# Ryan-Yanlong/DREAM-GNN

Hardware: AMD Instinct MI355X
Metric: GCMC+FGCN SpMM edges/sec and achieved HBM GB/s at 1/2/4/8 MI355X (higher is better)
Workload: dtype f32

## Files before the change

### dream_gnn_amd/_lib.py

```python
from __future__ import annotations

import ctypes
import os

import torch

_HERE = os.path.dirname(os.path.abspath(__file__))
LIB_PATH = os.path.join(_HERE, "libdgmi.so")
TORCH_LIB_PATH = os.path.join(_HERE, "libdgmi_torch.so")

ABI_VERSION = 20

_vp = ctypes.c_void_p
_i64 = ctypes.c_int64
_EPI = [ctypes.c_int32, ctypes.c_float, _vp, _i64, ctypes.c_float]


SIGNATURES = {
    "dgmi_abi_version": (ctypes.c_int, []),
    "dgmi_status_string": (ctypes.c_char_p, [ctypes.c_int]),
    "dgmi_device_ok": (ctypes.c_int, []),
    "dgmi_csr_from_coo_i32": (ctypes.c_int, [_vp, _vp, _i64, _i64, _i64, _vp, _vp, _vp, _vp,
                                             ctypes.POINTER(ctypes.c_size_t), _vp]),
    "dgmi_spmm_csr_f32": (ctypes.c_int, [_vp, _vp, _vp, _vp, _vp, ctypes.c_int32, _vp, _i64, _vp, _vp, _vp, _i64, _i64,
                                         _i64, _i64] + _EPI + [_vp]),
    "dgmi_gather_f32": (ctypes.c_int, [_vp, _vp, _i64, _vp, _vp]),
    "dgmi_gather_concat_f32": (ctypes.c_int, [_vp, _vp, _i64, _vp, _i64, _i64, _vp, _i64, _i64, _vp, _i64, _vp]),
    "dgmi_csr_sliced_from_coo_i32": (ctypes.c_int, [_vp, _vp, _i64, _i64, _i64, ctypes.c_int32, _vp, _vp, _vp, _vp,
                                                    ctypes.POINTER(ctypes.c_size_t), _vp]),
    "dgmi_csr_sliced_from_csr_i32": (ctypes.c_int, [_vp, _vp, _vp, _i64, _i64, _i64, ctypes.c_int32, _vp, _vp, _vp, _vp,
                                                    ctypes.POINTER(ctypes.c_size_t), _vp]),
    "dgmi_spmm_sliced_planes_bytes": (ctypes.c_size_t, [_i64, ctypes.c_int32, _i64]),
    "dgmi_spmm_sliced_f32": (ctypes.c_int, [_vp, _vp, _vp, _vp, _vp, ctypes.c_int32, _vp, _i64, _vp, _vp, _vp, _i64, _i64,
                                            _i64, _i64, ctypes.c_int32, ctypes.c_int32, ctypes.c_int32, _vp, ctypes.c_size_t] + _EPI
                             + [_vp]),
    "dgmi_knn_cosine_supported": (ctypes.c_int, [_i64, _i64, _i64]),
    "dgmi_knn_cosine_workspace_bytes": (ctypes.c_size_t, [_i64, _i64, ctypes.c_int32]),
    "dgmi_knn_cosine_topk_f32": (ctypes.c_int, [_vp, _i64, _i64, _i64, ctypes.c_int32, _vp, _vp, ctypes.c_size_t, _vp]),
    "dgmi_probe_row_gather_f32": (ctypes.c_int, [_vp, _i64, _i64, _i64, _i64, _i64, ctypes.c_int32, _vp, _vp]),
    "dgmi_epilogue_backward_f32": (ctypes.c_int, [_vp, _vp, _vp, _i64, ctypes.c_int32, ctypes.c_float, ctypes.c_float, _vp, _vp]),
    "dgmi_gather_add_f32": (ctypes.c_int, [_vp, _vp, _i64, _vp, _i64, _vp, _i64, _vp, _i64, _vp, _i64, ctypes.c_int32, _vp]),
    "dgmi_random_subset_workspace_bytes": (ctypes.c_size_t, []),
    "dgmi_random_subset_mask_f32": (ctypes.c_int, [_i64, _i64, ctypes.c_uint64, _vp, _vp, ctypes.c_size_t, _vp]),
    "dgmi_spmm_default_chunk": (ctypes.c_int32, [_i64, _i64]),
    "dgmi_spmm_plan_bytes": (ctypes.c_size_t, [_i64, _i64, ctypes.c_int32]),
    "dgmi_spmm_partials_bytes": (ctypes.c_size_t, [_i64, ctypes.c_int32, _i64]),
    "dgmi_spmm_plan_build": (ctypes.c_int, [_vp, _i64, _i64, ctypes.c_int32, _vp, ctypes.c_size_t, _vp,
                                            ctypes.POINTER(ctypes.c_size_t), _vp]),
    "dgmi_spmm_csr_planned_f32": (ctypes.c_int, [_vp, _vp, _vp, _vp, _vp, ctypes.c_int32, _vp, _i64, _vp, _vp, _vp, _i64,
                                                 _i64, _i64, _i64, _i64, ctypes.c_int32, _vp, _vp, ctypes.c_size_t] + _EPI
                                  + [_vp]),
    "dgmi_random_subset_select": (ctypes.c_int, [_i64, _i64, ctypes.c_uint64, ctypes.c_uint32, _vp, _vp, ctypes.c_size_t,
                                                 _vp]),
    "dgmi_random_subset_select_batch": (ctypes.c_int, [ctypes.c_int32, _vp, _vp, _vp, _vp, _vp, _vp, ctypes.c_size_t, _vp]),
    "dgmi_random_subset_select_batch_dseed": (ctypes.c_int, [ctypes.c_int32, _vp, _vp, _vp, _vp, _vp, _vp, ctypes.c_size_t, _vp]),
    "dgmi_keep_mask_f32": (ctypes.c_int, [_vp, ctypes.c_int32, _i64, _vp, _vp]),
    "dgmi_scale_rows_f32": (ctypes.c_int, [_vp, _i64, _vp, _i64, _i64, _vp, _i64, _vp]),
    "dgmi_weighted_colsum_f32": (ctypes.c_int, [_vp, _i64, _vp, _i64, _i64, _i64, ctypes.c_int32, _vp, _i64, _vp]),
    "dgmi_rank_add_f32": (ctypes.c_int, [_vp, _i64, _vp, _i64, _vp, _i64, _i64, _i64, ctypes.c_int32, _vp]),
    "dgmi_compact_layout_workspace_bytes": (ctypes.c_size_t, [_i64]),
    "dgmi_compact_layout_i32": (ctypes.c_int, [_vp, _i64, _vp, _vp, _vp, _i64, _vp, ctypes.c_int32, _vp, _vp, _vp, _vp,
                                               ctypes.c_size_t, _vp]),
    "dgmi_set_tuning": (ctypes.c_int, [ctypes.c_char_p, _i64]),
    "dgmi_row_multiplicity_f32": (ctypes.c_int, [_vp, _vp, _i64, _i64, ctypes.c_float, _vp, _vp, _vp, _vp]),
}


PAIR_SIGNATURES = {
    "dgmi_pair_topk_workspace_bytes": (ctypes.c_size_t, [_i64, _i64, ctypes.c_int32]),
    "dgmi_pair_mlp_topk_f32": (ctypes.c_int, [_vp, _i64, _i64, _vp, _i64, _i64, ctypes.c_int32, ctypes.c_int32, _vp, _vp, _vp,
                                              _vp, _vp, _vp, _i64, ctypes.c_int32, _vp, _vp, _vp, _vp, _vp, ctypes.c_size_t,
                                              _vp]),
}
PAIR_TOPK_MAX_K = 1024

RANK_SIGNATURES = {
    "dgmi_row_topk_workspace_bytes": (ctypes.c_size_t, [_i64, _i64, ctypes.c_int32]),
    "dgmi_pair_mlp_row_topk_f32": (ctypes.c_int, [_vp, _i64, _i64, _vp, _i64, _i64, ctypes.c_int32, ctypes.c_int32, _vp, _vp,
                                                  _vp, _vp, _vp, _vp, _i64, ctypes.c_int32, _vp, _vp, _vp, _vp, _vp,
                                                  ctypes.c_size_t, _vp]),
}
ROW_TOPK_MAX_K = 128

ABOVE_SIGNATURES = {
    "dgmi_pair_emit_workspace_bytes": (ctypes.c_size_t, [_i64, _i64]),
    "dgmi_pair_mlp_emit_f32": (ctypes.c_int, [_vp, _i64, _i64, _vp, _i64, _i64, ctypes.c_int32, ctypes.c_int32, _vp, _vp, _vp,
                                              _vp, _vp, _vp, _i64, ctypes.c_float, _i64, _vp, _vp, _vp, _vp, _vp, _vp,
                                              ctypes.c_size_t, _vp]),
    "dgmi_pair_records_sort_workspace_bytes": (ctypes.c_size_t, [_i64]),
    "dgmi_pair_records_sort_f32": (ctypes.c_int, [_vp, _vp, _vp, _i64, _vp, ctypes.c_size_t, _vp]),
}
PAIR_EMIT_MAX_RECORDS = 1 << 24

BF16_SIGNATURES = {
    "dgmi_rows_to_bf16": (ctypes.c_int, [_vp, _i64, _vp, _i64, _i64, _vp, _i64, _vp]),
    "dgmi_spmm_sliced_bf16": (ctypes.c_int, [_vp, _vp, _vp, _vp, _vp, ctypes.c_int32, _vp, _i64, _vp, _vp, _i64, _i64, _i64, _i64,
                                             ctypes.c_int32, ctypes.c_int32, ctypes.c_int32, _vp, ctypes.c_size_t] + _EPI + [_vp]),
}


GIVEN_SIGNATURES = {
    "dgmi_pair_rank_workspace_bytes": (ctypes.c_size_t, [_i64, _i64, _i64]),
    "dgmi_pair_mlp_score_list_f32": (ctypes.c_int, [_vp, _i64, _i64, _vp, _i64, _i64, ctypes.c_int32, ctypes.c_int32, _vp, _vp,
                                                    _vp, _vp, _vp, _vp, _i64, _vp, _vp, _vp]),
    "dgmi_pair_mlp_rank_list_f32": (ctypes.c_int, [_vp, _i64, _i64, _vp, _i64, _i64, ctypes.c_int32, ctypes.c_int32, _vp, _vp,
                                                   _vp, _vp, _vp, _vp, _i64, _vp, _vp, _i64, _vp, _vp, _vp, _vp, _vp,
                                                   ctypes.c_size_t, _vp]),
}

CURVE_SIGNATURES = {
    "dgmi_curve_areas_workspace_bytes": (ctypes.c_size_t, [_i64, _i64]),
    "dgmi_curve_areas_f32": (ctypes.c_int, [_vp, _vp, _vp, _i64, _i64, ctypes.c_float, _vp, _vp, _vp, _vp, ctypes.c_size_t,
                                            _vp]),
}
CURVE_MAX_SEGMENTS = 1 << 24

LAYOUT_SIGNATURES = {
    "dgmi_sliced_layout_slices": (ctypes.c_int32, [_i64, _i64, _i64, ctypes.c_int32]),
}

_TRAIN_OPERANDS = [_vp, _i64, _i64, _vp, _i64, _i64, ctypes.c_int32, ctypes.c_int32, _vp, _vp, _vp, _vp, _vp, _vp, _i64,
                   ctypes.c_float, _vp]
TRAIN_SIGNATURES = {
    "dgmi_pair_mlp_train_workspace_bytes": (ctypes.c_size_t, [_i64]),
    "dgmi_pair_mlp_train_forward_f32": (ctypes.c_int, _TRAIN_OPERANDS + [_vp, _vp, _vp]),
    "dgmi_pair_mlp_train_backward_f32": (ctypes.c_int, _TRAIN_OPERANDS + [_vp, _vp, _i64, _vp, _vp, _vp, _vp, _vp, _vp,
                                                                          ctypes.c_size_t, _vp]),
}

_ATTN_OPERANDS = [_vp, _i64, _vp, _i64, _i64, ctypes.c_int32, ctypes.c_int32, _vp, _vp, _vp, _vp]
ATTN_SIGNATURES = {
    "dgmi_attn_fuse_workspace_bytes": (ctypes.c_size_t, [_i64, ctypes.c_int32]),
    "dgmi_attn_fuse_forward_f32": (ctypes.c_int, _ATTN_OPERANDS + [_vp, _i64, _vp, _vp]),
    "dgmi_attn_fuse_backward_f32": (ctypes.c_int, _ATTN_OPERANDS + [_vp, _i64, _vp, _i64, _vp, _i64, _vp, _vp, _vp, _vp,
                                                                     ctypes.c_size_t, _vp]),
}


class DgmiError(RuntimeError):
    """A non-zero dgmi_status came back from the C ABI."""


def _load() -> ctypes.CDLL:
    if not os.path.exists(LIB_PATH):
        raise ImportError(
            "dream_gnn_amd: %s is missing. Build it with `python -c 'import __graft_entry__ as g; g.build()'` "
            "or `make -C dream_gnn_amd/csrc` (hipcc --offload-arch=gfx950). There is no CPU fallback." % LIB_PATH)
    lib = ctypes.CDLL(LIB_PATH)
    for name, (res, args) in (list(SIGNATURES.items()) + list(PAIR_SIGNATURES.items()) + list(RANK_SIGNATURES.items())
                              + list(ABOVE_SIGNATURES.items()) + list(BF16_SIGNATURES.items())
                              + list(GIVEN_SIGNATURES.items()) + list(CURVE_SIGNATURES.items())
                              + list(LAYOUT_SIGNATURES.items()) + list(TRAIN_SIGNATURES.items())
                              + list(ATTN_SIGNATURES.items())):
        fn = getattr(lib, name)
        fn.restype = res
        fn.argtypes = args
    got = lib.dgmi_abi_version()
    if got != ABI_VERSION:
        raise ImportError("libdgmi.so ABI version %d != expected %d; rebuild" % (got, ABI_VERSION))
    return lib


lib = _load()


def _load_torch_ops():
    if not os.path.exists(TORCH_LIB_PATH):
        raise ImportError(
            "dream_gnn_amd: %s is missing. Build it with `python -c 'import __graft_entry__ as g; g.build()'` or "
            "`make -C dream_gnn_amd/csrc`. There is no CPU fallback." % TORCH_LIB_PATH)
    torch.ops.load_library(TORCH_LIB_PATH)
    return torch.ops.dreamgnn_mi


torch_ops = _load_torch_ops()


def set_tuning(name: str, value: int) -> None:
    check(lib.dgmi_set_tuning(name.encode(), int(value)), "dgmi_set_tuning(%s)" % name)


def sliced_layout_slices(n_dst: int, n_src: int, F: int, id_mult: bool = False) -> int:
    return int(lib.dgmi_sliced_layout_slices(int(n_dst), int(n_src), int(F), 1 if id_mult else 0))


def check(status: int, what: str) -> None:
    if status != 0:
        raise DgmiError("%s failed: %s (status %d)" % (what, lib.dgmi_status_string(status).decode(), status))
```

### dream_gnn_amd/csrc/dgmi_api.hip

```cpp
#include <hip/hip_runtime.h>
#include <limits.h>
#include <stdlib.h>
#include <string.h>

#include "dgmi.h"
#include "dgmi_bf16.h"
#include "dgmi_keep.h"
#include "dgmi_layout.h"
#include "dgmi_kernels.h"
#include "dgmi_tuning.h"

namespace {

inline hipStream_t as_stream(dgmi_stream_t s) { return static_cast<hipStream_t>(s); }

inline int from_hip(hipError_t e) { return e == hipSuccess ? DGMI_OK : DGMI_ERR_LAUNCH; }

long long env_ll(const char* name, long long dflt) {
  const char* e = getenv(name);
  return e != nullptr && e[0] != '\0' ? atoll(e) : dflt;
}

}

namespace dgmi {

Tuning& tuning() {
  static Tuning t = [] {
    Tuning v;
    v.sliced_rows = (int)env_ll("DGMI_SLICED_ROWS", 0);
    v.sliced_touch_lead = (int)env_ll("DGMI_SLICED_PF", -1);
    v.sliced_lpr = (int)env_ll("DGMI_SLICED_LPR", 0);
    v.sliced_no_off32 = getenv("DGMI_NO_OFF32") != nullptr ? 1 : 0;
    v.sliced_chunk_rows = env_ll("DGMI_SLICED_CHUNK_ROWS", 0);
    v.sliced_taper_rows = env_ll("DGMI_SLICED_TAPER_ROWS", 0);
    v.sliced_owned = (int)env_ll("DGMI_SLICED_OWNED", -1);
    v.sliced_owned_grid = (int)env_ll("DGMI_SLICED_OWNED_GRID", 0);
    v.sliced_owned_wgs = (int)env_ll("DGMI_SLICED_OWNED_WGS", 0);
    v.sliced_owned_rows = (int)env_ll("DGMI_SLICED_OWNED_ROWS", 0);
    v.sliced_owned_lds_rows = env_ll("DGMI_SLICED_OWNED_LDS_ROWS", 0);
    v.sliced_owned_workers = (int)env_ll("DGMI_SLICED_OWNED_WORKERS", 0);
    v.sliced_owned_slices = (int)env_ll("DGMI_SLICED_OWNED_SLICES", 0);
    v.sliced_owned_lag = (int)env_ll("DGMI_SLICED_OWNED_LAG", -2);
    v.sliced_owned_spin_ticks = env_ll("DGMI_SLICED_OWNED_SPIN_TICKS", 0);
    v.select_window_min = env_ll("DGMI_SELECT_WINDOW_MIN", 0);
    v.select_narrow_window = env_ll("DGMI_SELECT_NARROW_WINDOW", 0) != 0 ? 1 : 0;
    v.sort_plain_tiles = env_ll("DGMI_SORT_PLAIN_TILES", 0) != 0 ? 1 : 0;
    v.knn_screen_first = env_ll("DGMI_KNN_SCREEN_V1", 0) != 0 ? 1 : 0;
    v.knn_pool_chunks = env_ll("DGMI_KNN_POOL_CHUNKS", 0);
    return v;
  }();
  return t;
}

}

extern "C" {

DGMI_API int dgmi_set_tuning(const char* name, int64_t value) {
  if (name == nullptr) return DGMI_ERR_INVALID_ARG;
  dgmi::Tuning& t = dgmi::tuning();
  if (strcmp(name, "sliced_rows") == 0) t.sliced_rows = (int)value;
  else if (strcmp(name, "sliced_touch_lead") == 0) t.sliced_touch_lead = (int)value;
  else if (strcmp(name, "sliced_lpr") == 0) t.sliced_lpr = (int)value;
  else if (strcmp(name, "sliced_no_off32") == 0) t.sliced_no_off32 = value != 0;
  else if (strcmp(name, "sliced_chunk_rows") == 0) t.sliced_chunk_rows = value;
  else if (strcmp(name, "sliced_taper_rows") == 0) t.sliced_taper_rows = value;
  else if (strcmp(name, "sliced_owned") == 0) t.sliced_owned = (int)value;
  else if (strcmp(name, "sliced_owned_grid") == 0) t.sliced_owned_grid = (int)value;
  else if (strcmp(name, "sliced_owned_wgs") == 0) t.sliced_owned_wgs = (int)value;
  else if (strcmp(name, "sliced_owned_rows") == 0) t.sliced_owned_rows = (int)value;
  else if (strcmp(name, "sliced_owned_lds_rows") == 0) t.sliced_owned_lds_rows = value;
  else if (strcmp(name, "sliced_owned_workers") == 0) t.sliced_owned_workers = (int)value;
  else if (strcmp(name, "sliced_owned_slices") == 0) t.sliced_owned_slices = (int)value;
  else if (strcmp(name, "sliced_owned_lag") == 0) t.sliced_owned_lag = (int)value;
  else if (strcmp(name, "sliced_owned_spin_ticks") == 0) t.sliced_owned_spin_ticks = value;
  else if (strcmp(name, "select_window_min") == 0) t.select_window_min = value;
  else if (strcmp(name, "select_narrow_window") == 0) t.select_narrow_window = value != 0;
  else if (strcmp(name, "sort_plain_tiles") == 0) t.sort_plain_tiles = value != 0;
  else if (strcmp(name, "knn_screen_first") == 0) t.knn_screen_first = value != 0;
  else if (strcmp(name, "knn_pool_chunks") == 0) t.knn_pool_chunks = value;
  else return DGMI_ERR_INVALID_ARG;
  return DGMI_OK;
}

DGMI_API int dgmi_abi_version(void) { return DGMI_ABI_VERSION; }

DGMI_API const char* dgmi_status_string(int status) {
  switch (status) {
    case DGMI_OK: return "ok";
    case DGMI_ERR_INVALID_ARG: return "invalid argument (null pointer, negative size or ld < F)";
    case DGMI_ERR_TOO_LARGE: return "size does not fit the int32 id space";
    case DGMI_ERR_WORKSPACE: return "workspace missing or too small";
    case DGMI_ERR_LAUNCH: return "HIP launch failed";
    case DGMI_ERR_NO_DEVICE: return "no gfx950 device visible";
    default: return "unknown dgmi status";
  }
}

DGMI_API int dgmi_device_ok(void) {
  int n = 0;
  if (hipGetDeviceCount(&n) != hipSuccess || n <= 0) return 0;
  int dev = 0;
  if (hipGetDevice(&dev) != hipSuccess) return 0;
  hipDeviceProp_t prop;
  if (hipGetDeviceProperties(&prop, dev) != hipSuccess) return 0;
  return strncmp(prop.gcnArchName, "gfx950", 6) == 0 ? 1 : 0;
}

DGMI_API int dgmi_csr_from_coo_i32(const int32_t* row, const int32_t* col, int64_t E, int64_t n_rows,
                          int64_t n_cols, int32_t* indptr, int32_t* indices, int32_t* eid, void* workspace,
                          size_t* workspace_bytes, dgmi_stream_t stream) {
  if (E < 0 || n_rows < 0 || workspace_bytes == nullptr) return DGMI_ERR_INVALID_ARG;
  if (E > INT32_MAX || n_rows >= INT32_MAX || n_cols >= INT32_MAX) return DGMI_ERR_TOO_LARGE;
  if (workspace != nullptr) {
    if (indptr == nullptr) return DGMI_ERR_INVALID_ARG;
    if (E > 0 && (row == nullptr || col == nullptr || indices == nullptr || eid == nullptr))
      return DGMI_ERR_INVALID_ARG;
  }
  size_t need = 0;
  hipError_t err = dgmi::csr_from_coo_i32(row, col, E, n_rows, n_cols, indptr, indices, eid, nullptr,
                                          &need, as_stream(stream));
  if (err != hipSuccess) return DGMI_ERR_LAUNCH;
  if (workspace == nullptr) {
    *workspace_bytes = need;
    return DGMI_OK;
  }
  if (*workspace_bytes < need) return DGMI_ERR_WORKSPACE;
  return from_hip(dgmi::csr_from_coo_i32(row, col, E, n_rows, n_cols, indptr, indices, eid, workspace,
                                         workspace_bytes, as_stream(stream)));
}

static bool epilogue_ok(int32_t act, const float* out_mask, int64_t ld_mask, int64_t F) {
  return (act == 0 || act == 1) && (out_mask == nullptr || ld_mask >= F);
}

static bool keep_args_ok(const int32_t* eid, const uint32_t* keep, int32_t n_keep) {
  if (n_keep < 0 || n_keep > dgmi::kMaxKeepSegs) return false;
  return n_keep == 0 || (eid != nullptr && keep != nullptr);
}

DGMI_API int dgmi_spmm_csr_f32(const int32_t* indptr, const int32_t* indices, const float* vals,
                      const int32_t* eid, const uint32_t* keep, int32_t n_keep,
                      const float* X, int64_t ldx, const float* src_scale,
                      const float* dst_scale, float* Y, int64_t ldy, int64_t n_dst,
                      int64_t n_src, int64_t F, int32_t act, float act_slope, const float* out_mask,
                      int64_t ld_mask, float out_mask_scale, dgmi_stream_t stream) {
  if (n_dst < 0 || n_src < 0 || F < 0 || !keep_args_ok(eid, keep, n_keep) || !epilogue_ok(act, out_mask, ld_mask, F))
    return DGMI_ERR_INVALID_ARG;
  if (n_dst >= INT32_MAX || n_src >= INT32_MAX || F > INT32_MAX) return DGMI_ERR_TOO_LARGE;
  if (n_dst == 0 || F == 0) return DGMI_OK;
  if (indptr == nullptr || Y == nullptr) return DGMI_ERR_INVALID_ARG;
  if (ldx < F || ldy < F) return DGMI_ERR_INVALID_ARG;
  if (X == nullptr && n_src > 0) return DGMI_ERR_INVALID_ARG;
  if (static_cast<const void*>(X) == static_cast<const void*>(Y)) return DGMI_ERR_INVALID_ARG;
  dgmi::SpmmArgs a{indptr, indices, vals, X, ldx, src_scale, dst_scale, Y, ldy, n_dst, n_src, F,
                   nullptr, 0, 0, nullptr, 0, eid, keep, n_keep, {act, act_slope, out_mask, ld_mask, out_mask_scale}};
  return from_hip(dgmi::spmm_csr_f32(a, as_stream(stream)));
}

DGMI_API int32_t dgmi_spmm_default_chunk(int64_t n_rows, int64_t nnz) {
  (void)n_rows;
  int64_t c = (nnz / 4096 + 63) / 64 * 64;
  if (c < 64) c = 64;
  if (c > 512) c = 512;
  return (int32_t)c;
}

static bool chunk_ok(int32_t chunk) { return chunk >= 16 && chunk <= 65536; }

DGMI_API size_t dgmi_spmm_plan_bytes(int64_t n_rows, int64_t nnz, int32_t chunk) {
  if (n_rows < 0 || nnz < 0 || !chunk_ok(chunk)) return 0;
  return dgmi::plan_bytes(n_rows, nnz, chunk);
}

DGMI_API size_t dgmi_spmm_partials_bytes(int64_t nnz, int32_t chunk, int64_t F) {
  if (nnz < 0 || F < 0 || !chunk_ok(chunk)) return 0;
  const size_t ldp = (size_t)((F + 3) / 4 * 4);
  const size_t b = (size_t)dgmi::plan_slots_cap(nnz, chunk) * ldp * sizeof(float);
  return b < 16 ? 16 : b;
}

DGMI_API int dgmi_spmm_plan_build(const int32_t* indptr, int64_t n_rows, int64_t nnz, int32_t chunk,
                                  void* plan, size_t plan_bytes, void* workspace,
                                  size_t* workspace_bytes, dgmi_stream_t stream) {
  if (n_rows < 0 || nnz < 0 || !chunk_ok(chunk) || workspace_bytes == nullptr)
    return DGMI_ERR_INVALID_ARG;
  if (n_rows >= INT32_MAX || nnz > INT32_MAX) return DGMI_ERR_TOO_LARGE;
  size_t need = 0;
  if (dgmi::spmm_plan_build(indptr, n_rows, nnz, chunk, nullptr, nullptr, &need, as_stream(stream)) !=
      hipSuccess)
    return DGMI_ERR_LAUNCH;
  if (workspace == nullptr) {
    *workspace_bytes = need;
    return DGMI_OK;
  }
  if (plan == nullptr || (indptr == nullptr && n_rows > 0)) return DGMI_ERR_INVALID_ARG;
  if (*workspace_bytes < need || plan_bytes < dgmi::plan_bytes(n_rows, nnz, chunk))
    return DGMI_ERR_WORKSPACE;
  return from_hip(dgmi::spmm_plan_build(indptr, n_rows, nnz, chunk, static_cast<int32_t*>(plan),
                                        workspace, workspace_bytes, as_stream(stream)));
}

DGMI_API int dgmi_spmm_csr_planned_f32(const int32_t* indptr, const int32_t* indices,
                                       const float* vals, const int32_t* eid, const uint32_t* keep,
                                       int32_t n_keep, const float* X, int64_t ldx,
                                       const float* src_scale, const float* dst_scale, float* Y,
                                       int64_t ldy, int64_t n_dst, int64_t n_src, int64_t F,
                                       int64_t nnz, int32_t chunk, const void* plan, void* partials,
                                       size_t partials_bytes, int32_t act, float act_slope,
                                       const float* out_mask, int64_t ld_mask, float out_mask_scale,
                                       dgmi_stream_t stream) {
  if (n_dst < 0 || n_src < 0 || F < 0 || nnz < 0 || !chunk_ok(chunk) || !keep_args_ok(eid, keep, n_keep) ||
      !epilogue_ok(act, out_mask, ld_mask, F))
    return DGMI_ERR_INVALID_ARG;
  if (n_dst >= INT32_MAX || n_src >= INT32_MAX || F > INT32_MAX || nnz > INT32_MAX)
    return DGMI_ERR_TOO_LARGE;
  if (n_dst == 0 || F == 0) return DGMI_OK;
  if (indptr == nullptr || Y == nullptr || plan == nullptr || partials == nullptr)
    return DGMI_ERR_INVALID_ARG;
  if (ldx < F || ldy < F) return DGMI_ERR_INVALID_ARG;
  if (X == nullptr && n_src > 0) return DGMI_ERR_INVALID_ARG;
  if (static_cast<const void*>(X) == static_cast<const void*>(Y)) return DGMI_ERR_INVALID_ARG;
  if (partials_bytes < dgmi_spmm_partials_bytes(nnz, chunk, F)) return DGMI_ERR_WORKSPACE;
  dgmi::SpmmArgs a{indptr, indices, vals, X, ldx, src_scale, dst_scale, Y, ldy, n_dst, n_src, F,
                   static_cast<const int32_t*>(plan), nnz, chunk, static_cast<float*>(partials),
                   (F + 3) / 4 * 4, eid, keep, n_keep, {act, act_slope, out_mask, ld_mask, out_mask_scale}};
  return from_hip(dgmi::spmm_csr_f32(a, as_stream(stream)));
}

static int64_t slice_width_for(int64_t n_cols, int32_t n_slices) {
  const int64_t w = (n_cols + n_slices - 1) / n_slices;
  return w > 0 ? w : 1;
}

static int id_bits(int64_t n) {
  int b = 1;
  while (b < 32 && ((int64_t)1 << b) < n) ++b;
  return b;
}

DGMI_API int dgmi_csr_sliced_from_coo_i32(const int32_t* row, const int32_t* col, int64_t E, int64_t n_rows,
                                          int64_t n_cols, int32_t n_slices, int32_t* segptr,
                                          int32_t* indices, int32_t* eid, void* workspace,
                                          size_t* workspace_bytes, dgmi_stream_t stream) {
  if (E < 0 || n_rows < 0 || n_cols < 0 || n_slices < 1 || n_slices > 64 || workspace_bytes == nullptr)
    return DGMI_ERR_INVALID_ARG;
  if (E > INT32_MAX || n_cols >= INT32_MAX || n_rows * (int64_t)n_slices >= INT32_MAX) return DGMI_ERR_TOO_LARGE;
  if (workspace != nullptr) {
    if (segptr == nullptr) return DGMI_ERR_INVALID_ARG;
    if (E > 0 && (row == nullptr || col == nullptr || indices == nullptr || eid == nullptr))
      return DGMI_ERR_INVALID_ARG;
  }
  const int64_t width = slice_width_for(n_cols, n_slices);
  size_t need = 0;
  if (dgmi::csr_sliced_from_coo_i32(row, col, E, n_rows, n_cols, n_slices, width, segptr, indices, eid, nullptr,
                                    &need, as_stream(stream)) != hipSuccess)
    return DGMI_ERR_LAUNCH;
  if (workspace == nullptr) {
    *workspace_bytes = need;
    return DGMI_OK;
  }
  if (*workspace_bytes < need) return DGMI_ERR_WORKSPACE;
  return from_hip(dgmi::csr_sliced_from_coo_i32(row, col, E, n_rows, n_cols, n_slices, width, segptr, indices,
                                                eid, workspace, workspace_bytes, as_stream(stream)));
}

DGMI_API int dgmi_csr_sliced_from_csr_i32(const int32_t* indptr, const int32_t* indices, const int32_t* eid, int64_t E,
                                          int64_t n_rows, int64_t n_cols, int32_t n_slices, int32_t* segptr,
                                          int32_t* s_indices, int32_t* s_eid, void* workspace, size_t* workspace_bytes,
                                          dgmi_stream_t stream) {
  if (E < 0 || n_rows < 0 || n_cols < 0 || n_slices < 1 || n_slices > 64 || workspace_bytes == nullptr)
    return DGMI_ERR_INVALID_ARG;
  if (E > INT32_MAX || n_cols >= INT32_MAX || n_rows * (int64_t)n_slices >= INT32_MAX) return DGMI_ERR_TOO_LARGE;
  if (id_bits(n_rows) + id_bits(n_slices) > 31) return DGMI_ERR_TOO_LARGE;
  if (workspace != nullptr) {
    if (segptr == nullptr) return DGMI_ERR_INVALID_ARG;
    if (E > 0 && (indptr == nullptr || indices == nullptr || eid == nullptr || s_indices == nullptr || s_eid == nullptr))
      return DGMI_ERR_INVALID_ARG;
  }
  const int64_t width = slice_width_for(n_cols, n_slices);
  size_t need = 0;
  if (dgmi::csr_sliced_from_csr_i32(indptr, indices, eid, E, n_rows, n_cols, n_slices, width, segptr, s_indices, s_eid,
                                    nullptr, &need, as_stream(stream)) != hipSuccess)
    return DGMI_ERR_LAUNCH;
  if (workspace == nullptr) {
    *workspace_bytes = need;
    return DGMI_OK;
  }
  if (*workspace_bytes < need) return DGMI_ERR_WORKSPACE;
  return from_hip(dgmi::csr_sliced_from_csr_i32(indptr, indices, eid, E, n_rows, n_cols, n_slices, width, segptr, s_indices,
                                                s_eid, workspace, workspace_bytes, as_stream(stream)));
}

static int64_t sliced_chunk_rows(int64_t n_dst, int32_t n_slices, int64_t F) {
  const int64_t row_bytes = (int64_t)n_slices * ((F + 3) / 4 * 4) * (int64_t)sizeof(float);
  int64_t rows = ((int64_t)4096 << 20) / (row_bytes > 0 ? row_bytes : 1);
  rows = rows / 1024 * 1024;
  if (rows < 1024) rows = 1024;
  if (dgmi::tuning().sliced_chunk_rows > 0) rows = dgmi::tuning().sliced_chunk_rows;
  return rows < n_dst ? rows : n_dst;
}

DGMI_API size_t dgmi_spmm_sliced_planes_bytes(int64_t n_dst, int32_t n_slices, int64_t F) {
  if (n_dst < 0 || n_slices < 1 || F < 0) return 0;
  const size_t b = (size_t)sliced_chunk_rows(n_dst, n_slices, F) * (size_t)n_slices *
                   (size_t)((F + 3) / 4 * 4) * sizeof(float);
  return b < 16 ? 16 : b;
}

static int spmm_sliced(const int32_t* segptr, const int32_t* indices, const float* vals, const int32_t* eid, const uint32_t* keep,
                       int32_t n_keep, const void* X, int x_bytes, int64_t ldx, const float* src_scale, const float* dst_scale,
                       float* Y, int64_t ldy, int64_t n_dst, int64_t n_src, int64_t F, int32_t n_slices, int32_t column_passes,
                       int32_t id_multiplicity, void* planes, size_t planes_bytes, int32_t act, float act_slope,
                       const float* out_mask, int64_t ld_mask, float out_mask_scale, dgmi_stream_t stream) {
  const int cols = 16 / x_bytes;
  if (n_dst < 0 || n_src < 0 || F < 0 || n_slices < 1 || n_slices > 64 || !keep_args_ok(eid, keep, n_keep) ||
      !epilogue_ok(act, out_mask, ld_mask, F) || column_passes < 0 || column_passes > 1 || id_multiplicity < 0 ||
      id_multiplicity > 1)
    return DGMI_ERR_INVALID_ARG;
  if (id_multiplicity == 1 && (vals != nullptr || n_src > (int64_t)dgmi::kMultIdMask + 1)) return DGMI_ERR_INVALID_ARG;
  if (out_mask != nullptr && (ld_mask % 4 != 0 || (reinterpret_cast<uintptr_t>(out_mask) & 15))) return DGMI_ERR_INVALID_ARG;
  if (n_dst >= INT32_MAX || n_src >= INT32_MAX || F > INT32_MAX) return DGMI_ERR_TOO_LARGE;
  if (n_dst == 0 || F == 0) return DGMI_OK;
  if (segptr == nullptr || Y == nullptr || planes == nullptr) return DGMI_ERR_INVALID_ARG;
  if (X == nullptr && n_src > 0) return DGMI_ERR_INVALID_ARG;
  if (ldx < F || ldy < F || F % cols != 0 || ldx % cols != 0 || ldy % 4 != 0) return DGMI_ERR_INVALID_ARG;
  if ((reinterpret_cast<uintptr_t>(X) & 15) || (reinterpret_cast<uintptr_t>(Y) & 15) ||
      (reinterpret_cast<uintptr_t>(planes) & 15))
    return DGMI_ERR_INVALID_ARG;
  if (X == static_cast<const void*>(Y)) return DGMI_ERR_INVALID_ARG;
  if (planes_bytes < dgmi_spmm_sliced_planes_bytes(n_dst, n_slices, F)) return DGMI_ERR_WORKSPACE;
  dgmi::SlicedArgs a{segptr, indices, vals, X, x_bytes, ldx, src_scale, dst_scale, Y, ldy, n_dst, n_src, F, n_slices,
                     static_cast<float*>(planes), F, sliced_chunk_rows(n_dst, n_slices, F), eid, keep, n_keep,
                     {act, act_slope, out_mask, ld_mask, out_mask_scale}, column_passes == 1, id_multiplicity == 1};
  return from_hip(dgmi::spmm_sliced(a, as_stream(stream)));
}

DGMI_API int dgmi_spmm_sliced_f32(const int32_t* segptr, const int32_t* indices, const float* vals,
                                  const int32_t* eid, const uint32_t* keep, int32_t n_keep,
                                  const float* X, int64_t ldx, const float* src_scale,
                                  const float* dst_scale, float* Y, int64_t ldy, int64_t n_dst,
                                  int64_t n_src, int64_t F, int32_t n_slices, int32_t column_passes,
                                  int32_t id_multiplicity, void* planes,
                                  size_t planes_bytes, int32_t act, float act_slope, const float* out_mask,
                                  int64_t ld_mask, float out_mask_scale, dgmi_stream_t stream) {
  return spmm_sliced(segptr, indices, vals, eid, keep, n_keep, X, 4, ldx, src_scale, dst_scale, Y, ldy, n_dst, n_src, F,
                     n_slices, column_passes, id_multiplicity, planes, planes_bytes, act, act_slope, out_mask, ld_mask,
                     out_mask_scale, stream);
}

DGMI_API int dgmi_rows_to_bf16(const float* X, int64_t ldx, const float* scale, int64_t n, int64_t F, uint16_t* out, int64_t ldo,
                               dgmi_stream_t stream) {
  if (n < 0 || F < 0 || F % 8 != 0 || ldx < F || ldo < F || ldx % 4 != 0 || ldo % 8 != 0) return DGMI_ERR_INVALID_ARG;
  if (F > INT32_MAX) return DGMI_ERR_TOO_LARGE;
  if (n == 0 || F == 0) return DGMI_OK;
  if (X == nullptr || out == nullptr) return DGMI_ERR_INVALID_ARG;
  if ((reinterpret_cast<uintptr_t>(X) & 15) || (reinterpret_cast<uintptr_t>(out) & 15)) return DGMI_ERR_INVALID_ARG;
  if (static_cast<const void*>(X) == static_cast<const void*>(out)) return DGMI_ERR_INVALID_ARG;
  return from_hip(dgmi::rows_to_bf16(X, ldx, scale, n, F, out, ldo, as_stream(stream)));
}

DGMI_API int dgmi_spmm_sliced_bf16(const int32_t* segptr, const int32_t* indices, const float* vals, const int32_t* eid,
                                   const uint32_t* keep, int32_t n_keep, const uint16_t* X, int64_t ldx,
                                   const float* dst_scale, float* Y, int64_t ldy, int64_t n_dst, int64_t n_src, int64_t F,
                                   int32_t n_slices, int32_t column_passes, int32_t id_multiplicity, void* planes,
                                   size_t planes_bytes, int32_t act, float act_slope, const float* out_mask,
                                   int64_t ld_mask, float out_mask_scale, dgmi_stream_t stream) {
  return spmm_sliced(segptr, indices, vals, eid, keep, n_keep, X, 2, ldx, nullptr, dst_scale, Y, ldy, n_dst, n_src, F,
                     n_slices, column_passes, id_multiplicity, planes, planes_bytes, act, act_slope, out_mask, ld_mask,
                     out_mask_scale, stream);
}

DGMI_API int32_t dgmi_sliced_layout_slices(int64_t n_dst, int64_t n_src, int64_t F, int32_t id_multiplicity) {
  return dgmi::sliced_layout_slices(n_dst, n_src, F, id_multiplicity == 1);
}

DGMI_API int dgmi_gather_concat_f32(const int32_t* src, const int32_t* dst, int64_t E, const float* A,
                                    int64_t lda, int64_t Fa, const float* B, int64_t ldb, int64_t Fb,
                                    float* out, int64_t ldo, dgmi_stream_t stream) {
  if (E < 0 || Fa < 0 || Fb < 0) return DGMI_ERR_INVALID_ARG;
  if (E > INT32_MAX || Fa + Fb > INT32_MAX) return DGMI_ERR_TOO_LARGE;
  if (E == 0 || Fa + Fb == 0) return DGMI_OK;
  if (src == nullptr || dst == nullptr || out == nullptr) return DGMI_ERR_INVALID_ARG;
  if ((Fa > 0 && A == nullptr) || (Fb > 0 && B == nullptr)) return DGMI_ERR_INVALID_ARG;
  if (lda < Fa || ldb < Fb || ldo < Fa + Fb) return DGMI_ERR_INVALID_ARG;
  return from_hip(dgmi::gather_concat_f32(src, dst, E, A, lda, Fa, B, ldb, Fb, out, ldo, as_stream(stream)));
}

DGMI_API int dgmi_gather_add_f32(const int32_t* src, const int32_t* dst, int64_t E, const float* A,
                                 int64_t lda, const float* B, int64_t ldb, const float* bias, int64_t F,
                                 float* out, int64_t ldo, int32_t act, dgmi_stream_t stream) {
  if (E < 0 || F < 0 || (act != 0 && act != 1)) return DGMI_ERR_INVALID_ARG;
  if (E > INT32_MAX || F > INT32_MAX) return DGMI_ERR_TOO_LARGE;
  if (E == 0 || F == 0) return DGMI_OK;
  if (src == nullptr || dst == nullptr || A == nullptr || B == nullptr || out == nullptr)
    return DGMI_ERR_INVALID_ARG;
  if (lda < F || ldb < F || ldo < F) return DGMI_ERR_INVALID_ARG;
  return from_hip(dgmi::gather_add_f32(src, dst, E, A, lda, B, ldb, bias, F, out, ldo, act, as_stream(stream)));
}

DGMI_API int dgmi_epilogue_backward_f32(const float* dY, const float* Y, const float* mask, int64_t n, int32_t act,
                                        float act_slope, float mask_scale, float* out, dgmi_stream_t stream) {
  if (n < 0 || act < 0 || act > 2 || (act == 2 && mask != nullptr)) return DGMI_ERR_INVALID_ARG;
  if (n == 0) return DGMI_OK;
  if (dY == nullptr || out == nullptr || (act != 0 && Y == nullptr)) return DGMI_ERR_INVALID_ARG;
  return from_hip(dgmi::epilogue_backward_f32(dY, Y, mask, n, act, act_slope, mask_scale, out, as_stream(stream)));
}

DGMI_API int dgmi_scale_rows_f32(const float* X, int64_t ldx, const float* scale, int64_t n, int64_t F, float* out, int64_t ldo,
                                 dgmi_stream_t stream) {
  if (n < 0 || F < 0 || ldx < F || ldo < F) return DGMI_ERR_INVALID_ARG;
  if (F > INT32_MAX) return DGMI_ERR_TOO_LARGE;
  if (n == 0 || F == 0) return DGMI_OK;
  if (X == nullptr || scale == nullptr || out == nullptr) return DGMI_ERR_INVALID_ARG;
  return from_hip(dgmi::scale_rows_f32(X, ldx, scale, n, F, out, ldo, as_stream(stream)));
}

DGMI_API int dgmi_weighted_colsum_f32(const float* A, int64_t lda, const float* coef, int64_t ldc, int64_t n, int64_t W,
                                      int32_t B, float* out, int64_t ldo, dgmi_stream_t stream) {
  if (n < 0 || W < 0 || B < 0 || B > 64 || lda < W || ldo < W || ldc < n) return DGMI_ERR_INVALID_ARG;
  if (W > INT32_MAX) return DGMI_ERR_TOO_LARGE;
  if (W == 0 || B == 0) return DGMI_OK;
  if (out == nullptr || coef == nullptr || (A == nullptr && n > 0)) return DGMI_ERR_INVALID_ARG;
  return from_hip(dgmi::weighted_colsum_f32(A, lda, coef, ldc, n, W, B, out, ldo, as_stream(stream)));
}

DGMI_API int dgmi_rank_add_f32(float* G, int64_t ldg, const float* coef, int64_t ldc, const float* gs, int64_t lds, int64_t n,
                               int64_t W, int32_t B, dgmi_stream_t stream) {
  if (n < 0 || W < 0 || B < 0 || B > 64 || ldg < W || lds < W || ldc < n) return DGMI_ERR_INVALID_ARG;
  if (W > INT32_MAX) return DGMI_ERR_TOO_LARGE;
  if (n == 0 || W == 0 || B == 0) return DGMI_OK;
  if (G == nullptr || coef == nullptr || gs == nullptr) return DGMI_ERR_INVALID_ARG;
  return from_hip(dgmi::rank_add_f32(G, ldg, coef, ldc, gs, lds, n, W, B, as_stream(stream)));
}

DGMI_API size_t dgmi_random_subset_workspace_bytes(void) { return dgmi::random_subset_workspace_bytes(); }

DGMI_API int dgmi_random_subset_mask_f32(int64_t E, int64_t keep, uint64_t seed, float* mask, void* workspace,
                                         size_t workspace_bytes, dgmi_stream_t stream) {
  if (E < 0 || keep < 0 || keep > E) return DGMI_ERR_INVALID_ARG;
  if (E > INT32_MAX) return DGMI_ERR_TOO_LARGE;
  if (E == 0) return DGMI_OK;
  if (mask == nullptr || workspace == nullptr) return DGMI_ERR_INVALID_ARG;
  if (workspace_bytes < dgmi::random_subset_workspace_bytes()) return DGMI_ERR_WORKSPACE;
  return from_hip(dgmi::random_subset_mask_f32(E, keep, seed, mask, workspace, as_stream(stream)));
}

DGMI_API int dgmi_random_subset_select(int64_t E, int64_t keep, uint64_t seed, uint32_t e_offset, uint32_t* desc,
                                      void* workspace, size_t workspace_bytes, dgmi_stream_t stream) {
  if (E < 0 || keep < 0 || keep > E || desc == nullptr) return DGMI_ERR_INVALID_ARG;
  if (E > INT32_MAX || (uint64_t)e_offset + (uint64_t)E > (uint64_t)INT32_MAX) return DGMI_ERR_TOO_LARGE;
  if (workspace == nullptr) return DGMI_ERR_INVALID_ARG;
  if (workspace_bytes < dgmi::random_subset_workspace_bytes()) return DGMI_ERR_WORKSPACE;
  return from_hip(dgmi::random_subset_select(E, keep, seed, e_offset, desc, workspace, as_stream(stream)));
}

DGMI_API int dgmi_random_subset_select_batch(int32_t n, const int64_t* E, const int64_t* keep, const uint64_t* seed,
                                            const uint32_t* e_offset, uint32_t* descs, void* workspace,
                                            size_t workspace_bytes, dgmi_stream_t stream) {
  if (n < 0 || n > dgmi::kMaxKeepSegs) return DGMI_ERR_INVALID_ARG;
  if (n == 0) return DGMI_OK;
  if (E == nullptr || keep == nullptr || seed == nullptr || descs == nullptr || workspace == nullptr)
    return DGMI_ERR_INVALID_ARG;
  for (int i = 0; i < n; ++i) {
    if (E[i] < 0 || keep[i] < 0 || keep[i] > E[i]) return DGMI_ERR_INVALID_ARG;
    if (E[i] > INT32_MAX || (uint64_t)(e_offset ? e_offset[i] : 0u) + (uint64_t)E[i] > (uint64_t)INT32_MAX)
      return DGMI_ERR_TOO_LARGE;
  }
  if (workspace_bytes < dgmi::random_subset_workspace_bytes()) return DGMI_ERR_WORKSPACE;
  return from_hip(dgmi::random_subset_select_batch(n, E, keep, seed, e_offset, descs, workspace, as_stream(stream)));
}

DGMI_API int dgmi_random_subset_select_batch_dseed(int32_t n, const int64_t* E, const int64_t* keep, const uint64_t* seed_dev,
                                                  const uint32_t* e_offset, uint32_t* descs, void* workspace,
                                                  size_t workspace_bytes, dgmi_stream_t stream) {
  if (n < 0 || n > dgmi::kMaxKeepSegs) return DGMI_ERR_INVALID_ARG;
  if (n == 0) return DGMI_OK;
  if (E == nullptr || keep == nullptr || seed_dev == nullptr || descs == nullptr || workspace == nullptr)
    return DGMI_ERR_INVALID_ARG;
  if (reinterpret_cast<uintptr_t>(seed_dev) & 7) return DGMI_ERR_INVALID_ARG;
  for (int i = 0; i < n; ++i) {
    if (E[i] < 0 || keep[i] < 0 || keep[i] > E[i]) return DGMI_ERR_INVALID_ARG;
    if (E[i] > INT32_MAX || (uint64_t)(e_offset ? e_offset[i] : 0u) + (uint64_t)E[i] > (uint64_t)INT32_MAX)
      return DGMI_ERR_TOO_LARGE;
  }
  if (workspace_bytes < dgmi::random_subset_workspace_bytes()) return DGMI_ERR_WORKSPACE;
  return from_hip(dgmi::random_subset_select_batch(n, E, keep, nullptr, e_offset, descs, workspace, as_stream(stream), seed_dev));
}

DGMI_API int dgmi_keep_mask_f32(const uint32_t* keep, int32_t n_keep, int64_t E, float* mask, dgmi_stream_t stream) {
  if (E < 0 || n_keep < 0 || n_keep > dgmi::kMaxKeepSegs || (n_keep > 0 && keep == nullptr)) return DGMI_ERR_INVALID_ARG;
  if (E > INT32_MAX) return DGMI_ERR_TOO_LARGE;
  if (E == 0) return DGMI_OK;
  if (mask == nullptr) return DGMI_ERR_INVALID_ARG;
  return from_hip(dgmi::keep_mask_f32(keep, n_keep, E, mask, as_stream(stream)));
}

DGMI_API int dgmi_row_multiplicity_f32(const int32_t* indptr, const float* vals, int64_t n_rows, int64_t nnz, float rel_tol,
                                       float* row_scale, int32_t* mult, int32_t* fail, dgmi_stream_t stream) {
  if (n_rows < 0 || nnz < 0 || !(rel_tol >= 0.f) || fail == nullptr) return DGMI_ERR_INVALID_ARG;
  if (n_rows >= INT32_MAX || nnz > INT32_MAX) return DGMI_ERR_TOO_LARGE;
  if (n_rows > 0 && (indptr == nullptr || row_scale == nullptr)) return DGMI_ERR_INVALID_ARG;
  if (nnz > 0 && (vals == nullptr || mult == nullptr)) return DGMI_ERR_INVALID_ARG;
  return from_hip(dgmi::row_multiplicity_f32(indptr, vals, n_rows, rel_tol, row_scale, mult, fail, as_stream(stream)));
}

DGMI_API size_t dgmi_compact_layout_workspace_bytes(int64_t nnz) {
  return nnz < 0 ? 0 : dgmi::compact_workspace_bytes(nnz);
}

DGMI_API int dgmi_compact_layout_i32(const int32_t* ptr, int64_t n_ptr, const int32_t* indices, const float* vals,
                                     const int32_t* eid, int64_t nnz, const uint32_t* keep, int32_t n_keep, int32_t* ptr_out,
                                     int32_t* indices_out, float* vals_out, void* workspace, size_t workspace_bytes,
                                     dgmi_stream_t stream) {
  if (n_ptr < 0 || nnz < 0 || n_keep < 1 || n_keep > dgmi::kMaxKeepSegs || keep == nullptr)
    return DGMI_ERR_INVALID_ARG;
  if (nnz > INT32_MAX || n_ptr > INT32_MAX) return DGMI_ERR_TOO_LARGE;
  if (n_ptr == 0) return DGMI_OK;
  if (ptr == nullptr || ptr_out == nullptr) return DGMI_ERR_INVALID_ARG;
  if (nnz > 0 && (indices == nullptr || eid == nullptr || indices_out == nullptr || workspace == nullptr)) return DGMI_ERR_INVALID_ARG;
  if ((vals == nullptr) != (vals_out == nullptr)) return DGMI_ERR_INVALID_ARG;
  if (nnz > 0 && workspace_bytes < dgmi::compact_workspace_bytes(nnz)) return DGMI_ERR_WORKSPACE;
  if (nnz > 0 && (reinterpret_cast<uintptr_t>(workspace) & 7)) return DGMI_ERR_INVALID_ARG;
  return from_hip(dgmi::compact_layout_i32(ptr, n_ptr, indices, vals, eid, nnz, keep, n_keep, ptr_out, indices_out, vals_out,
                                           workspace, as_stream(stream)));
}

DGMI_API int dgmi_gather_f32(const float* in, const int32_t* perm, int64_t n, float* out,
                    dgmi_stream_t stream) {
  if (n < 0) return DGMI_ERR_INVALID_ARG;
  if (n == 0) return DGMI_OK;
  if (in == nullptr || perm == nullptr || out == nullptr) return DGMI_ERR_INVALID_ARG;
  return from_hip(dgmi::gather_f32(in, perm, n, out, as_stream(stream)));
}

DGMI_API int dgmi_knn_cosine_supported(int64_t N, int64_t D, int64_t k) { return dgmi::knn_supported(N, D, k) ? 1 : 0; }

DGMI_API size_t dgmi_knn_cosine_workspace_bytes(int64_t N, int64_t D, int32_t k) {
  return dgmi::knn_supported(N, D, k) ? dgmi::knn_workspace_bytes(N, D, k) : 0;
}

DGMI_API int dgmi_knn_cosine_topk_f32(const float* Xn, int64_t ld, int64_t N, int64_t D, int32_t k, int32_t* nbr,
                                      void* workspace, size_t workspace_bytes, dgmi_stream_t stream) {
  if (N < 0 || D < 0 || k < 0 || ld < D) return DGMI_ERR_INVALID_ARG;
  if (N > INT32_MAX) return DGMI_ERR_TOO_LARGE;
  if (N == 0 || k == 0) return DGMI_OK;
  if (Xn == nullptr || nbr == nullptr || ld % 4 != 0 || (reinterpret_cast<uintptr_t>(Xn) & 15)) return DGMI_ERR_INVALID_ARG;
  if (!dgmi::knn_supported(N, D, k)) return DGMI_ERR_INVALID_ARG;
  const size_t need = dgmi::knn_workspace_bytes(N, D, k);
  if (need > 0 && (workspace == nullptr || workspace_bytes < need)) return DGMI_ERR_WORKSPACE;
  return from_hip(dgmi::knn_cosine_topk_f32(Xn, ld, N, D, k, nbr, workspace, as_stream(stream)));
}

DGMI_API int dgmi_probe_row_gather_f32(const float* table, int64_t n_rows, int64_t F, int64_t groups,
                                       int64_t per_group, int64_t window, int32_t per_xcd, float* out,
                                       dgmi_stream_t stream) {
  if (table == nullptr || out == nullptr || n_rows < 1 || groups < 1 || per_group < 1) return DGMI_ERR_INVALID_ARG;
  if (F < 4 || F % 4 != 0 || F > 256 || window < 1 || window > n_rows) return DGMI_ERR_INVALID_ARG;
  if (window > UINT32_MAX || groups > INT32_MAX) return DGMI_ERR_TOO_LARGE;
  if (per_xcd && window * 8 > n_rows) return DGMI_ERR_INVALID_ARG;
  if ((reinterpret_cast<uintptr_t>(table) & 15) || (reinterpret_cast<uintptr_t>(out) & 15)) return DGMI_ERR_INVALID_ARG;
  return from_hip(dgmi::probe_row_gather(table, n_rows, F, groups, per_group, window, per_xcd, out, as_stream(stream)));
}

}
```

### dream_gnn_amd/csrc/dgmi_kernels.h

```cpp
#pragma once
#include <hip/hip_runtime.h>
#include <stddef.h>
#include <stdint.h>

namespace dgmi {

constexpr int kPlanHeaderWords = 16;
constexpr int kPlanNumItems = 0;
constexpr int kPlanNumLong = 1;
constexpr int kPlanNumSlots = 2;
constexpr int kPlanChunk = 3;

inline int64_t plan_items_cap(int64_t n_rows, int64_t nnz, int64_t chunk) {
  return n_rows + nnz / chunk;
}
inline int64_t plan_long_cap(int64_t nnz, int64_t chunk) { return nnz / (chunk + 1); }
inline int64_t plan_slots_cap(int64_t nnz, int64_t chunk) {
  return nnz / chunk + plan_long_cap(nnz, chunk);
}
inline size_t plan_bytes(int64_t n_rows, int64_t nnz, int64_t chunk) {
  return sizeof(int32_t) *
         (size_t)(kPlanHeaderWords + 4 * (plan_items_cap(n_rows, nnz, chunk) + plan_long_cap(nnz, chunk)));
}

inline int pick_lpr(int64_t F, int cols = 4, int widest = 64) {
  const int64_t fc = (F + cols - 1) / cols;
  int best = 8;
  double best_util = 0.0;
  for (int lpr = widest; lpr >= 8; lpr /= 2) {
    const int64_t tiles = (fc + lpr - 1) / lpr;
    const double util = (double)fc / (double)(tiles * lpr);
    if (util >= 0.85) return lpr;
    if (util > best_util + 1e-9) {
      best_util = util;
      best = lpr;
    }
  }
  return best;
}

struct Epilogue {
  int act;
  float slope;
  const float* mask;
  int64_t ldm;
  float mask_scale;
};

struct SpmmArgs {
  const int32_t* indptr;
  const int32_t* indices;
  const float* vals;
  const float* X;
  int64_t ldx;
  const float* src_scale;
  const float* dst_scale;
  float* Y;
  int64_t ldy;
  int64_t n_dst;
  int64_t n_src;
  int64_t F;
  const int32_t* plan;
  int64_t nnz;
  int64_t chunk;
  float* partials;
  int64_t ldp;
  const int32_t* eid;
  const void* keep;
  int n_keep;
  Epilogue ep;
};

hipError_t spmm_csr_f32(const SpmmArgs& a, hipStream_t s);

hipError_t spmm_plan_build(const int32_t* indptr, int64_t n_rows, int64_t nnz, int64_t chunk,
                           int32_t* plan, void* workspace, size_t* workspace_bytes, hipStream_t s);

hipError_t csr_from_coo_i32(const int32_t* row, const int32_t* col, int64_t E,
                            int64_t n_rows, int64_t n_cols, int32_t* indptr, int32_t* indices,
                            int32_t* eid, void* workspace, size_t* workspace_bytes,
                            hipStream_t s);

struct SortPassPlan {
  int shift[8], bits[8];
};
int radix_sort_passes(int shift0, int bits, SortPassPlan* plan);
size_t radix_sort_workspace_bytes(int64_t E, int bits);
hipError_t radix_sort_records(const int32_t* key, const int32_t* eid_in, const int32_t* col, int64_t E, int shift0, int bits,
                              int32_t n_rows, int32_t n_cols, int32_t* keys_out, int32_t* eid_out, int32_t* col_out, int32_t* flag,
                              void* workspace, hipStream_t s);

hipError_t csr_sliced_from_coo_i32(const int32_t* row, const int32_t* col, int64_t E, int64_t n_rows,
                                   int64_t n_cols, int64_t n_slices, int64_t slice_width,
                                   int32_t* segptr, int32_t* indices, int32_t* eid, void* workspace,
                                   size_t* workspace_bytes, hipStream_t s);

hipError_t csr_sliced_from_csr_i32(const int32_t* indptr, const int32_t* indices, const int32_t* eid, int64_t E,
                                   int64_t n_rows, int64_t n_cols, int64_t n_slices, int64_t slice_width, int32_t* segptr,
                                   int32_t* s_indices, int32_t* s_eid, void* workspace, size_t* workspace_bytes,
                                   hipStream_t s);

constexpr int kMultShift = 28;
constexpr int kMultMax = 7;
constexpr uint32_t kMultIdMask = 0x0fffffffu;

struct SlicedArgs {
  const int32_t* segptr;
  const int32_t* indices;
  const float* vals;
  const void* X;
  int x_bytes;
  int64_t ldx;
  const float* src_scale;
  const float* dst_scale;
  float* Y;
  int64_t ldy;
  int64_t n_dst, n_src, F;
  int64_t n_slices;
  float* planes;
  int64_t ldp;
  int64_t chunk_rows;
  const int32_t* eid;
  const void* keep;
  int n_keep;
  Epilogue ep;
  bool full_width;
  bool id_mult;
};

hipError_t row_multiplicity_f32(const int32_t* indptr, const float* vals, int64_t n_rows, float rel_tol, float* row_scale,
                                int32_t* mult, int32_t* fail, hipStream_t s);
hipError_t spmm_sliced(const SlicedArgs& a, hipStream_t s);
int sliced_layout_slices(int64_t n_dst, int64_t n_src, int64_t F, bool id_mult);

hipError_t rows_to_bf16(const float* X, int64_t ldx, const float* scale, int64_t n, int64_t F, uint16_t* out, int64_t ldo,
                        hipStream_t s);

hipError_t gather_concat_f32(const int32_t* src, const int32_t* dst, int64_t E, const float* A,
                             int64_t lda, int64_t Fa, const float* B, int64_t ldb, int64_t Fb,
                             float* out, int64_t ldo, hipStream_t s);

hipError_t gather_add_f32(const int32_t* src, const int32_t* dst, int64_t E, const float* A, int64_t lda,
                          const float* B, int64_t ldb, const float* bias, int64_t F, float* out,
                          int64_t ldo, int act, hipStream_t s);

hipError_t epilogue_backward_f32(const float* dY, const float* Y, const float* mask, int64_t n, int act, float slope,
                                 float mask_scale, float* out, hipStream_t s);

hipError_t weighted_colsum_f32(const float* A, int64_t lda, const float* coef, int64_t ldc, int64_t n, int64_t W, int B,
                               float* out, int64_t ldo, hipStream_t s);
hipError_t rank_add_f32(float* G, int64_t ldg, const float* coef, int64_t ldc, const float* gs, int64_t lds, int64_t n,
                        int64_t W, int B, hipStream_t s);

hipError_t scale_rows_f32(const float* X, int64_t ldx, const float* scale, int64_t n, int64_t F, float* out, int64_t ldo,
                          hipStream_t s);

size_t random_subset_workspace_bytes();
hipError_t random_subset_select(int64_t E, int64_t keep, uint64_t seed, uint32_t e_offset, void* seg_out,
                                void* workspace, hipStream_t s);
hipError_t random_subset_select_batch(int n, const int64_t* E, const int64_t* keep, const uint64_t* seed,
                                      const uint32_t* e_offset, void* descs, void* workspace, hipStream_t s,
                                      const uint64_t* seed_dev = nullptr);
hipError_t keep_mask_f32(const void* table, int n_seg, int64_t E, float* mask, hipStream_t s);
hipError_t random_subset_mask_f32(int64_t E, int64_t keep, uint64_t seed, float* mask, void* workspace,
                                  hipStream_t s);

hipError_t gather_f32(const float* in, const int32_t* perm, int64_t n, float* out,
                      hipStream_t s);

size_t compact_workspace_bytes(int64_t nnz);
hipError_t compact_layout_i32(const int32_t* ptr, int64_t n_ptr, const int32_t* indices, const float* vals, const int32_t* eid,
                              int64_t nnz, const void* keep, int n_keep, int32_t* ptr_out, int32_t* indices_out, float* vals_out,
                              void* workspace, hipStream_t s);

bool knn_supported(int64_t N, int64_t D, int64_t k);
size_t knn_workspace_bytes(int64_t N, int64_t D, int k);
constexpr int kKnnTileMaxK = 16;
constexpr int kKnnScreenMaxK = 64;
int64_t knn_screen_min_rows();
bool knn_screen_supported(int64_t N, int64_t D, int64_t k);
size_t knn_screen_workspace_bytes(int64_t N, int64_t D, int k);
hipError_t knn_cosine_topk_screened(const float* Xn, int64_t ld, int64_t N, int64_t D, int k, int32_t* nbr, void* workspace,
                                    hipStream_t s);
hipError_t knn_cosine_topk_exact_tiles(const float* Xn, int64_t ld, int64_t N, int64_t D, int k, int32_t* nbr,
                                       const int32_t* flags, hipStream_t s);
hipError_t knn_cosine_topk_f32(const float* Xn, int64_t ld, int64_t N, int64_t D, int k, int32_t* nbr, void* workspace,
                               hipStream_t s);

hipError_t probe_row_gather(const float* table, int64_t n_rows, int64_t F, int64_t groups, int64_t per_group,
                            int64_t window, int per_xcd, float* out, hipStream_t s);

}
```

### dream_gnn_amd/csrc/dgmi_owned.hip

```cpp
#include <hip/hip_runtime.h>
#include <limits.h>
#include <stdint.h>

#include <map>
#include <mutex>
#include <type_traits>
#include <utility>

#include "dgmi_owned_common.h"
#include "dgmi_owned_kernel.h"
#include "dgmi_sliced_common.h"

namespace dgmi {
namespace {

constexpr int64_t kOwnedSpinTicks = 3000;
constexpr int64_t kOwnedMinRows = 32768;
constexpr int kOwnedLag = -1;
constexpr int kOwnedWideSlices = 16;
constexpr int kOwnedAssumedCus = 256;

template <int LPR, int VALS, bool OFF32, int WAVES>
__global__ __launch_bounds__(kWave* WAVES, WAVES == kOwnedWaves ? 4 : 6) void spmm_owned_kernel(
    const int32_t* __restrict__ segptr, const int32_t* __restrict__ indices, const float* __restrict__ X, int64_t ldx,
    const float* __restrict__ dst_scale, float* __restrict__ Y, int64_t ldy, int64_t n_dst, int F, OwnedPlan pl,
    unsigned* __restrict__ arrive, int lag, int64_t spin_ticks, int workers, Epilogue ep) {
  owned_body<OwnedRowF32, LPR, VALS, OFF32, WAVES, true>(segptr, indices, X, ldx, dst_scale, Y, ldy, n_dst, F, pl, arrive, lag,
                                                         spin_ticks, workers, ep);
}

template <int LPR, int VALS, bool OFF32>
__global__ __launch_bounds__(kWave* kOwnedWaves, 4) void spmm_owned_bf16_kernel(
    const int32_t* __restrict__ segptr, const int32_t* __restrict__ indices, const uint16_t* __restrict__ X, int64_t ldx,
    const float* __restrict__ dst_scale, float* __restrict__ Y, int64_t ldy, int64_t n_dst, int F, OwnedPlan pl,
    unsigned* __restrict__ arrive, int lag, int64_t spin_ticks, int workers, Epilogue ep) {
  owned_body<OwnedRowBf16, LPR, VALS, OFF32, kOwnedWaves, false>(segptr, indices, X, ldx, dst_scale, Y, ldy, n_dst, F, pl, arrive,
                                                                 lag, spin_ticks, workers, ep);
}

template <typename Row, int LPR, int VALS, bool OFF32, int WAVES>
constexpr auto owned_kernel() {
  if constexpr (std::is_same<Row, OwnedRowBf16>::value)
    return &spmm_owned_bf16_kernel<LPR, VALS, OFF32>;
  else
    return &spmm_owned_kernel<LPR, VALS, OFF32, WAVES>;
}

int device_cus() {
  static const int cus = [] {
    int dev = 0, n = 0;
    if (hipGetDevice(&dev) != hipSuccess || hipDeviceGetAttribute(&n, hipDeviceAttributeMultiprocessorCount, dev) != hipSuccess)
      return 0;
    return n;
  }();
  return cus;
}

int owned_class_form(const OwnedPlan& pl, bool id_mult, int64_t table_bytes, int x_bytes) {
  const auto mib = [&](int64_t lo, int64_t hi) { return table_bytes >= (lo << 20) && table_bytes <= (hi << 20); };
  if (x_bytes == 2) {
    if (pl.slices != kOwnedSlices || pl.col_rounds != 1) return 0;
    if (pl.row_rounds == 1 && !id_mult && mib(16, 32)) return 1;
    if (pl.row_rounds == 2 && !id_mult && mib(8, 16)) return 1;
    if (pl.row_rounds == 2 && id_mult && mib(16, 32)) return 1;
    if (pl.row_rounds == 1 && id_mult && mib(8, 16)) return 1;
    return 0;
  }
  if (x_bytes != 4) return 0;
  if (pl.slices == kOwnedSlices) {
    if (pl.col_rounds == 1 && pl.row_rounds == 2 && !id_mult && mib(16, 32)) return 1;
    if (pl.col_rounds == 2 && pl.row_rounds == 1 && id_mult && mib(48, 64)) return 1;
    if (pl.col_rounds == 1 && pl.row_rounds == 1 && id_mult && mib(16, 32)) return 1;
  }
  if (pl.slices == kOwnedWideSlices && pl.col_rounds == 1 && pl.row_rounds == 1 && !id_mult && mib(48, 64)) return 1;
  return 0;
}

int owned_class_phase_tasks(const OwnedPlan& pl, bool id_mult, int64_t table_bytes, int x_bytes) {
  if (x_bytes != 4) return kOwnedPhaseTasks;
  const auto mib = [&](int64_t lo, int64_t hi) { return table_bytes >= (lo << 20) && table_bytes <= (hi << 20); };
  if (pl.slices != kOwnedSlices) return kOwnedPhaseTasks;
  if (pl.col_rounds == 2 && pl.row_rounds == 1 && id_mult && mib(48, 64)) return kOwnedPhaseTasksMult;
  if (pl.col_rounds == 1 && pl.row_rounds == 1 && id_mult && mib(16, 32)) return kOwnedPhaseTasksMult;
  return kOwnedPhaseTasks;
}

bool owned_coresident(const void* kern, int threads, size_t lds, int wgs) {
  static std::mutex mu;
  static std::map<std::pair<const void*, size_t>, int> known;
  std::lock_guard<std::mutex> lock(mu);
  auto it = known.find({kern, lds});
  if (it == known.end()) {
    int n = 0;
    if (hipOccupancyMaxActiveBlocksPerMultiprocessor(&n, kern, threads, lds) != hipSuccess) {
      (void)hipGetLastError();
      n = 0;
    }
    it = known.emplace(std::make_pair(kern, lds), n).first;
  }
  return it->second >= wgs;
}

template <typename Row, int LPR, int WAVES>
hipError_t launch_owned(const SlicedArgs& a, const OwnedPlan& pl, int64_t grid, bool off32, int lag, int64_t spin_ticks,
                        hipStream_t s, bool* resident) {
  constexpr int kWgsPerCu = WAVES == kOwnedWaves ? 1 : 2;
  unsigned* arrive = reinterpret_cast<unsigned*>(a.planes);
  const int workers = tuning().sliced_owned_workers > 0 && tuning().sliced_owned_workers < WAVES - 1 ? tuning().sliced_owned_workers : 0;
  *resident = true;
#define DGMI_OWNED(V, O)                                                                                                  \
  do {                                                                                                                    \
    if constexpr (kWgsPerCu > 1 && LPR == 8 && V == 2) {                                                                  \
      *resident = false;                                                                                                  \
      return hipSuccess;                                                                                                  \
    } else {                                                                                                              \
    auto kern = owned_kernel<Row, LPR, V, O, WAVES>();                                                                    \
    static const hipError_t attr = hipFuncSetAttribute(reinterpret_cast<const void*>(kern),                               \
                                                       hipFuncAttributeMaxDynamicSharedMemorySize, (160 << 10) / kWgsPerCu); \
    if (attr != hipSuccess) return attr;                                                                                  \
    if (kWgsPerCu > 1 && !owned_coresident(reinterpret_cast<const void*>(kern), kWave * WAVES, pl.lds_bytes, kWgsPerCu)) { \
      *resident = false;                                                                                                  \
      return hipSuccess;                                                                                                  \
    }                                                                                                                     \
    if (lag >= 0) {                                                            \
      const hipError_t err = hipMemsetAsync(arrive, 0, sizeof(unsigned) * 8 * (size_t)pl.phases, s);                      \
      if (err != hipSuccess) return err;                                                                                  \
    }                                                                                                                     \
    hipLaunchKernelGGL(kern, dim3((unsigned)grid), dim3(kWave* WAVES), pl.lds_bytes, s, a.segptr, a.indices,              \
                       static_cast<const typename Row::Elem*>(a.X), a.ldx, a.dst_scale, a.Y, a.ldy, a.n_dst, (int)a.F, pl, \
                       arrive, lag, spin_ticks, workers, a.ep);                                                           \
    }                                                                                                                     \
  } while (0)
  if (a.id_mult) {
    if (off32) DGMI_OWNED(2, true); else DGMI_OWNED(2, false);
  } else {
    if (off32) DGMI_OWNED(0, true); else DGMI_OWNED(0, false);
  }
#undef DGMI_OWNED
  return hipGetLastError();
}

template <typename Row, int WAVES>
hipError_t launch_owned_width(const SlicedArgs& a, const OwnedPlan& pl, int lpr, int64_t grid, bool off32, int lag,
                              int64_t spin_ticks, hipStream_t s, bool* resident) {
  switch (lpr) {
    case 8: return launch_owned<Row, 8, WAVES>(a, pl, grid, off32, lag, spin_ticks, s, resident);
    case 16: return launch_owned<Row, 16, WAVES>(a, pl, grid, off32, lag, spin_ticks, s, resident);
    case 32: return launch_owned<Row, 32, WAVES>(a, pl, grid, off32, lag, spin_ticks, s, resident);
    case 64:
      if constexpr (Row::kMaxLpr >= 64)
        return launch_owned<Row, 64, WAVES>(a, pl, grid, off32, lag, spin_ticks, s, resident);
      else
        return hipErrorInvalidValue;
    default: return hipErrorInvalidValue;
  }
}

}

hipError_t spmm_owned_try(const SlicedArgs& a, hipStream_t s, bool* taken) {
  *taken = false;
  const Tuning& tune = tuning();
  if (tune.sliced_owned == 0) return hipSuccess;
  if ((a.x_bytes != 4 && a.x_bytes != 2) || a.vals != nullptr || a.src_scale != nullptr || a.n_keep != 0 || a.n_slices < 1 || a.n_slices > kOwnedMaxSlices ||
      tune.sliced_chunk_rows > 0 || a.chunk_rows < a.n_dst || a.n_dst == 0 || a.F == 0)
    return hipSuccess;
  if (a.x_bytes == 2 && tune.sliced_owned_slices > 0) return hipSuccess;
  const int64_t grid = tune.sliced_owned_grid > 0 ? tune.sliced_owned_grid : device_cus();
  if (grid < 1) return hipSuccess;
  const int lpr = sliced_lpr(a.F, a.n_src, a.n_slices, a.n_dst, a.full_width, a.n_keep, a.x_bytes, tune.sliced_lpr);
  const int slices = (int)a.n_slices;
  const int cols = 16 / a.x_bytes;
  const int64_t table_bytes = a.n_src * a.ldx * (int64_t)a.x_bytes;
  OwnedPlan pl = owned_plan(a.n_dst, a.F, lpr, grid, tune.sliced_owned_rows, tune.sliced_owned_lds_rows, 1, kOwnedPhaseTasks, slices, cols);
  const int phase_tasks = a.n_dst < kOwnedMinRows ? kOwnedPhaseTasks : owned_class_phase_tasks(pl, a.id_mult, table_bytes, a.x_bytes);
  if (pl.ok && phase_tasks != kOwnedPhaseTasks)
    pl = owned_plan(a.n_dst, a.F, lpr, grid, tune.sliced_owned_rows, tune.sliced_owned_lds_rows, 1, phase_tasks, slices, cols);
  if (!pl.ok || pl.lds_bytes > (size_t)(160 << 10)) return hipSuccess;
  const int rule = a.n_dst < kOwnedMinRows ? 0 : owned_class_form(pl, a.id_mult, table_bytes, a.x_bytes);
  if (tune.sliced_owned != 1 && rule == 0) return hipSuccess;
  const bool off32 = !tune.sliced_no_off32 && (a.n_src * a.ldx + a.F) * a.x_bytes < ((int64_t)1 << 32);
  bool resident = true;
  if (a.x_bytes == 2) {
    *taken = true;
    return launch_owned_width<OwnedRowBf16, kOwnedWaves>(a, pl, lpr, grid, off32, -1, 0, s, &resident);
  }
  const auto arrive_fits = [&](const OwnedPlan& p) {
    return sizeof(unsigned) * 8 * (size_t)p.phases <= sizeof(float) * (size_t)a.n_slices * (size_t)a.n_dst * (size_t)a.ldp;
  };
  if (!arrive_fits(pl)) return hipSuccess;
  const int form = tune.sliced_owned_wgs == 1 || tune.sliced_owned_wgs == 2 ? tune.sliced_owned_wgs : (rule == 2 ? 2 : 1);
  const int64_t spin = tune.sliced_owned_spin_ticks > 0 ? tune.sliced_owned_spin_ticks : kOwnedSpinTicks;
  const int lag = tune.sliced_owned_lag >= -1 ? tune.sliced_owned_lag : kOwnedLag;
  *taken = true;
  if (form == 2) {
    const int64_t grid2 = tune.sliced_owned_grid > 0 ? grid : 2 * grid;
    const OwnedPlan pl2 = owned_plan(a.n_dst, a.F, lpr, grid2, tune.sliced_owned_rows, tune.sliced_owned_lds_rows, 2, kOwnedPhaseTasks, slices);
    if (pl2.ok && pl2.lds_bytes <= (size_t)(80 << 10) && arrive_fits(pl2)) {
      const hipError_t err = launch_owned_width<OwnedRowF32, kOwnedPairWaves>(a, pl2, lpr, grid2, off32, lag, spin, s, &resident);
      if (err != hipSuccess || resident) return err;
    }
  }
  return launch_owned_width<OwnedRowF32, kOwnedWaves>(a, pl, lpr, grid, off32, lag, spin, s, &resident);
}

int sliced_layout_slices(int64_t n_dst, int64_t n_src, int64_t F, bool id_mult) {
  const Tuning& tune = tuning();
  if (n_dst < 1 || n_src < 1 || F < 1 || F % 4 != 0 || tune.sliced_owned == 0 || tune.sliced_chunk_rows > 0) return kOwnedSlices;
  const int forced = tune.sliced_owned_slices;
  const int slices = forced > 0 ? (forced < kOwnedMaxSlices ? forced : kOwnedMaxSlices) : kOwnedWideSlices;
  if (slices == kOwnedSlices) return kOwnedSlices;
  if (n_dst * slices >= INT32_MAX || n_dst * slices * F * (int64_t)sizeof(float) > ((int64_t)4096 << 20)) return kOwnedSlices;
  const int64_t grid = tune.sliced_owned_grid > 0 ? tune.sliced_owned_grid : (device_cus() > 0 ? device_cus() : kOwnedAssumedCus);
  const int lpr = sliced_lpr(F, n_src, slices, n_dst, false, 0, 4, tune.sliced_lpr);
  const OwnedPlan pl = owned_plan(n_dst, F, lpr, grid, tune.sliced_owned_rows, tune.sliced_owned_lds_rows, 1, kOwnedPhaseTasks, slices);
  if (!pl.ok || pl.lds_bytes > (size_t)(160 << 10)) return kOwnedSlices;
  if (forced > 0) return slices;
  if (n_dst < kOwnedMinRows) return kOwnedSlices;
  return owned_class_form(pl, id_mult, n_src * F * (int64_t)sizeof(float), 4) == 1 ? slices : kOwnedSlices;
}

}
```

### dream_gnn_amd/csrc/dgmi_owned_kernel.h

```cpp
#pragma once
#include <hip/hip_runtime.h>
#include <stdint.h>

#include "dgmi_owned_common.h"
#include "dgmi_sliced_common.h"

namespace dgmi {
namespace {

constexpr int kOwnedTouchChunk = 4;
constexpr int kOwnedTouchLead = 8;

struct OwnedRowF32 : RowF32 {
  static constexpr int kLaneSlots = 1;
  static constexpr bool kCarry = true;
  static constexpr bool kPeel = true;

  template <int LPR>
  static __device__ __forceinline__ void commit(float4* slot, bool first, const Acc& acc) {
    if (first) {
      *slot = acc;
      return;
    }
    float4 t = *slot;
    t.x += acc.x;
    t.y += acc.y;
    t.z += acc.z;
    t.w += acc.w;
    *slot = t;
  }

  template <int LPR>
  static __device__ __forceinline__ Acc sum(const float4* slot) {
    return *slot;
  }

  static __device__ __forceinline__ void scale(Acc& t, float d) {
    t.x *= d;
    t.y *= d;
    t.z *= d;
    t.w *= d;
  }

  static __device__ __forceinline__ void write(const Acc& t, float* y, const Epilogue& ep, int64_t row, int col) {
    *reinterpret_cast<float4*>(y) = epilogue4(ep, t, row, col);
  }
};

struct OwnedRowBf16 : RowBf16 {
  static constexpr int kLaneSlots = 2;
  static constexpr bool kCarry = false;
  static constexpr bool kPeel = false;

  template <int LPR>
  static __device__ __forceinline__ Acc sum(const float4* slot) {
    return pairs(slot[0], slot[LPR]);
  }

  template <int LPR>
  static __device__ __forceinline__ void commit(float4* slot, bool first, const Acc& acc) {
    Acc t = acc;
    if (!first) {
      const Acc s = sum<LPR>(slot);
#pragma unroll
      for (int k = 0; k < 4; ++k) t.p[k] = s.p[k] + acc.p[k];
    }
    slot[0] = half(t, 0);
    slot[LPR] = half(t, 1);
  }

  static __device__ __forceinline__ void scale(Acc& t, float d) {
#pragma unroll
    for (int k = 0; k < 4; ++k) t.p[k] *= d;
  }

  static __device__ __forceinline__ void write(const Acc& t, float* y, const Epilogue& ep, int64_t row, int col) {
    OwnedRowF32::write(half(t, 0), y, ep, row, col);
    OwnedRowF32::write(half(t, 1), y + 4, ep, row, col + 4);
  }
};

template <typename Row, int LPR, int VALS, bool OFF32, int WAVES, bool GATE>
__device__ __forceinline__ void owned_body(const int32_t* __restrict__ segptr, const int32_t* __restrict__ indices,
                                           const typename Row::Elem* __restrict__ X, int64_t ldx,
                                           const float* __restrict__ dst_scale, float* __restrict__ Y, int64_t ldy,
                                           int64_t n_dst, int F, OwnedPlan pl, unsigned* __restrict__ arrive, int lag,
                                           int64_t spin_ticks, int workers, Epilogue ep) {
  typedef typename Row::Elem Elem;
  typedef typename Row::Acc Acc;
  constexpr bool MULT = VALS == 2;
  constexpr int kIdMask = MULT ? (int)kMultIdMask : 0x7fffffff;
  constexpr int kRowSlots = Row::kLaneSlots * LPR;
  constexpr bool CARRY = WAVES == kOwnedWaves && MULT && Row::kCarry;
  extern __shared__ float4 lds_rows[];
  const int lane = threadIdx.x & (kWave - 1);
  const int wave = threadIdx.x >> 6;
  const int grp = lane / LPR, glane = lane % LPR, gbase = grp * LPR;
  const int64_t wg = blockIdx.x;
  const int T = owned_wg_tasks(pl, wg);
  if (T == 0) return;
  int* done = reinterpret_cast<int*>(lds_rows + (size_t)pl.round_rows * kRowSlots);
  int* phase_cnt = done + pl.tasks;
  int* counter = phase_cnt + pl.phases;
  int* open = counter + 1;
  for (int i = threadIdx.x; i < pl.tasks + pl.phases + 2; i += blockDim.x) done[i] = 0;
  __syncthreads();
  const int total = pl.phases * T;
  const int label = (int)(blockIdx.x & 7u);

  if (wave == WAVES - 1) {
    const unsigned n_label = (unsigned)((pl.active - label + 7) >> 3);
    const unsigned* my_arrive = GATE ? arrive + (size_t)label * pl.phases : nullptr;
    const int chunks_per_phase = (T + kOwnedTouchChunk - 1) / kOwnedTouchChunk, chunks = pl.phases * chunks_per_phase;
    const int last_gate = GATE && lag >= 0 ? pl.phases - 1 : 0;
    int keepalive = 0, touched = 0, opened = 0;
    bool waiting = false;
    uint64_t wait_start = 0;
    while (touched < chunks || opened < last_gate) {
      bool idle = true;
      const int next = __hip_atomic_load(counter, __ATOMIC_RELAXED, __HIP_MEMORY_SCOPE_WORKGROUP);
      if (touched < chunks) {
        const int P = touched / chunks_per_phase, t0 = (touched - P * chunks_per_phase) * kOwnedTouchChunk;
        if (P * T + t0 <= next + kOwnedTouchLead) {
          ++touched;
          idle = false;
          const OwnedPhase ph = owned_phase(pl, P);
          const int64_t in_round = owned_round_rows(pl, wg, ph.row_round);
          const int64_t lds_first = (int64_t)t0 * pl.G * pl.R;
          int64_t lds_last = lds_first + (int64_t)kOwnedTouchChunk * pl.G * pl.R;
          if (lds_last > in_round) lds_last = in_round;
          if (lds_first < lds_last) {
            const int32_t* sp_s = segptr + (int64_t)ph.slice * n_dst;
            const int64_t r_first = owned_task(pl, wg, ph.row_round, t0, 0).row0, r_last = r_first + (lds_last - lds_first);
            const int64_t rp = lane == 0 ? r_first : (lane == 1 ? r_last : r_first + (int64_t)(lane - 1) * 32);
            int v = 0;
            if (rp <= r_last) v = sp_s[rp];
            keepalive ^= v;
            const int e0 = __builtin_amdgcn_readlane(v, 0), e1 = __builtin_amdgcn_readlane(v, 1);
            for (int64_t p = (int64_t)e0 + (int64_t)lane * 32; p < e1; p += (int64_t)kWave * 32) keepalive ^= indices[p];
            asm volatile("" ::"v"(keepalive));
          }
        }
      }
      if (GATE && opened < last_gate) {
        const int P = opened + 1, need = P - 1 - lag;
        bool ok = need < 0 || __hip_atomic_load(&my_arrive[need], __ATOMIC_RELAXED, __HIP_MEMORY_SCOPE_AGENT) >= n_label;
        if (!ok && next >= P * T) {
          const uint64_t now = __builtin_amdgcn_s_memrealtime();
          if (!waiting) {
            waiting = true;
            wait_start = now;
          } else if (now - wait_start >= (uint64_t)spin_ticks) {
            ok = true;
          }
        }
        if (ok) {
          opened = P;
          waiting = false;
          idle = false;
          __hip_atomic_store(open, P, __ATOMIC_RELAXED, __HIP_MEMORY_SCOPE_WORKGROUP);
        }
      }
      if (idle) __builtin_amdgcn_s_sleep(2);
    }
    return;
  }

  if (workers > 0 && wave >= workers) return;
  auto grab = [&]() {
    int k = 0;
    if (lane == 0) k = __hip_atomic_fetch_add(counter, 1, __ATOMIC_RELAXED, __HIP_MEMORY_SCOPE_WORKGROUP);
    return __builtin_amdgcn_readfirstlane(k);
  };
  auto boundaries = [&](const OwnedWork& t) {
    return segptr[t.rows == 0 ? 0 : (int64_t)t.slice * n_dst + t.row_base + (t.lds_row + (glane < t.rows ? glane : t.rows))];
  };
  auto scales = [&](const OwnedWork& t) {
    if (!CARRY || dst_scale == nullptr || t.slice != pl.slices - 1 || t.rows == 0) return 0.f;
    return dst_scale[t.row_base + (t.lds_row + (glane < t.rows ? glane : t.rows - 1))];
  };
  int nxt_idx = 0, nxt_idx1 = 0, rel_b = 0;
  float my_ds = 0.f, nxt_ds = 0.f;
  static_assert(kOwnedWindowFirstBatches == 2, "nxt_idx and nxt_idx1");
  auto hand_over = [&](int b, const OwnedWork& nxt, int& beg, int& end) {
    beg = __shfl(b, gbase, kWave);
    rel_b = b - beg;
    end = beg + __shfl(rel_b, gbase + nxt.rows, kWave);
    if (beg < end) {
      nxt_idx = indices[beg + owned_carry_slot_edge(glane % kOwnedWindow, end - beg)];
      nxt_idx1 = indices[beg + owned_window_id_edge(owned_carry_start_batch(), glane, end - beg)];
    }
    my_ds = nxt_ds;
    nxt_ds = scales(nxt);
  };

  constexpr int W = kOwnedWindow;
  static_assert(W <= 8 && kMultShift == 28 && LPR % W == 0, "at most eight 4-bit multiplicity fields, shifted down from bit 28");
  typename Row::Reg v[W];
  int idx[W];
  int nidx[W];
  uint32_t mults = 0, mults_in = 0, nmults = 0;
  bool carried = false;
  auto read_batch = [&](int batch_idx, int (&out)[W], uint32_t& fields) {
#pragma unroll
    for (int u = 0; u < W; ++u) {
      int id = __shfl(batch_idx, gbase + u, kWave);
      if (MULT) {
        fields = (fields >> 4) | ((uint32_t)id & ((uint32_t)kMultMax << kMultShift));
        id &= kIdMask;
      }
      out[u] = id;
    }
    if (MULT) asm volatile("" : "+v"(fields));
  };
  auto read_ids = [&](int batch_idx) { read_batch(batch_idx, idx, mults_in); };

  const uint32_t row_bytes = (uint32_t)ldx * (uint32_t)sizeof(Elem);
  int k = grab();
  OwnedWork w = owned_decode(pl, wg, T, k, grp);
  int e_begin = 0, e_end = 0;
  hand_over(boundaries(w), w, e_begin, e_end);
  int my_rel = rel_b;
  while (k < total) {
    const int L = e_end - e_begin;
    int col = (w.col_round * LPR + glane) * Row::kCols;
    const bool col_ok = col < F;
    if (!col_ok) col = 0;
    const Elem* Xc = X + col;
    const uint32_t col_bytes = (uint32_t)col * (uint32_t)sizeof(Elem);
    if (L > 0 && !carried) {
      read_ids(nxt_idx);
#pragma unroll
      for (int u = 0; u < W; ++u) v[u] = Row::template load<OFF32>(X, Xc, idx[u], ldx, row_bytes, col_bytes);
      mults = mults_in;
    }
    const int k_next = grab();
    const OwnedWork w_next = owned_decode(pl, wg, T, k_next, grp);
    const int next_b = boundaries(w_next);
    int n_begin = 0, n_end = 0;
    if (GATE && lag >= 0)
      while (__hip_atomic_load(open, __ATOMIC_RELAXED, __HIP_MEMORY_SCOPE_WORKGROUP) < w.phase) __builtin_amdgcn_s_sleep(1);
    while (__hip_atomic_load(&done[w.task], __ATOMIC_ACQUIRE, __HIP_MEMORY_SCOPE_WORKGROUP) < w.phase) __builtin_amdgcn_s_sleep(1);
    const int first_ids = nxt_idx1;
    static_assert(owned_carry_start_batch() == 1, "nxt_idx1");
    if (CARRY) hand_over(next_b, w_next, n_begin, n_end);

    const int nr = w.rows;
    float4* slot = lds_rows + (size_t)w.lds_row * kRowSlots + glane;
    auto commit = [&](int r, const Acc& acc) { Row::template commit<LPR>(slot + r * kRowSlots, w.slice == 0, acc); };
    auto write_rows = [&]() {
      if (w.slice != pl.slices - 1) return;
      for (int r = 0; r < nr; ++r) {
        float d = 0.f;
        if (CARRY) d = __shfl(my_ds, gbase + r, kWave);
        if (!col_ok) continue;
        Acc t = Row::template sum<LPR>(slot + r * kRowSlots);
        const int64_t row = w.row_base + (w.lds_row + r);
        if (dst_scale != nullptr) {
          if (!CARRY) d = dst_scale[row];
          Row::scale(t, d);
        }
        Row::write(t, Y + row * ldy + col, ep, row, col);
      }
    };

    bool carry = false;
    int r = 0;
    Acc acc = Row::zero();
    if (L > 0) {
      int row_end = e_begin + __shfl(my_rel, gbase + 1, kWave);
      auto add = [&](int u) {
        float m = 1.f;
        if (MULT) {
          m = (float)(((mults >> (32 - 4 * W)) & (uint32_t)kMultMax) + 1u);
          mults >>= 4;
        }
        Row::template add<MULT>(acc, m, v[u]);
      };
      auto rows_before = [&](int p) {
        while (p >= row_end) {
          commit(r, acc);
          acc = Row::zero();
          ++r;
          row_end = e_begin + __shfl(my_rel, gbase + r + 1, kWave);
        }
      };
      int ids = first_ids;
      __builtin_amdgcn_sched_barrier(0);
      int p0 = e_begin;
      carry = CARRY && owned_carry(L, n_end - n_begin);
      auto group = [&](int g) {
        read_ids(ids);
        ids = indices[e_begin + owned_window_id_edge(owned_window_request_batch(g), glane, L)];
        __builtin_amdgcn_sched_barrier(0);
#pragma unroll
        for (int u = 0; u < W; ++u) {
          rows_before(p0 + u);
          add(u);
          v[u] = Row::template load<OFF32>(X, Xc, idx[u], ldx, row_bytes, col_bytes);
          __builtin_amdgcn_sched_barrier(0);
        }
        mults = mults_in;
      };
      static_assert(Row::kPeel || !CARRY, "the hand-over reads the next task's batch between the peeled groups");
      static_assert(owned_carry_read_group(2 * W + 1) == 0 && owned_carry_read_group(2 * W) == -1, "behind group 0 of three or more");
      int g = 0;
      if (!Row::kPeel) {
      } else if (owned_carry_read_group(L) == 0) {
        group(0);
        p0 += W;
        if (carry) read_batch(nxt_idx, nidx, nmults);
        group(1);
        p0 += W;
        g = 2;
      } else {
        if (p0 + W < e_end) {
          group(0);
          p0 += W;
          g = 1;
        }
        if (carry) read_batch(nxt_idx, nidx, nmults);
      }
      for (; p0 + W < e_end; ++g, p0 += W) group(g);
      const Elem* Xn = X;
      uint32_t ncol_bytes = 0;
      if (carry) {
        int ncol = (w_next.col_round * LPR + glane) * Row::kCols;
        if (ncol >= F) ncol = 0;
        Xn = X + ncol;
        ncol_bytes = (uint32_t)ncol * (uint32_t)sizeof(Elem);
      }
      __builtin_amdgcn_sched_barrier(0);
      if (carry) {
#pragma unroll
        for (int u = 0; u < W; ++u) {
          if (p0 + u < e_end) {
            rows_before(p0 + u);
            add(u);
          }
          v[u] = Row::template load<OFF32>(X, Xn, nidx[u], ldx, row_bytes, ncol_bytes);
          __builtin_amdgcn_sched_barrier(0);
        }
        mults = nmults;
      } else {
#pragma unroll
        for (int u = 0; u < W; ++u) {
          if (p0 + u < e_end) {
            rows_before(p0 + u);
            add(u);
          }
        }
      }
    }
    if (nr > 0) {
      for (; r < nr; ++r) {
        commit(r, acc);
        acc = Row::zero();
      }
      write_rows();
    }
    const OwnedWork w_then = CARRY ? w_next : owned_decode(pl, wg, T, k_next, grp);
    if (!CARRY) hand_over(next_b, w_then, n_begin, n_end);
    __builtin_amdgcn_wave_barrier();
    if (lane == 0) {
      __hip_atomic_store(&done[w.task], w.phase + 1, __ATOMIC_RELEASE, __HIP_MEMORY_SCOPE_WORKGROUP);
      if (GATE && lag >= 0) {
        const int finished = __hip_atomic_fetch_add(&phase_cnt[w.phase], 1, __ATOMIC_RELAXED, __HIP_MEMORY_SCOPE_WORKGROUP);
        if (finished == T - 1)
          __hip_atomic_fetch_add(&arrive[(size_t)label * pl.phases + w.phase], 1u, __ATOMIC_RELAXED, __HIP_MEMORY_SCOPE_AGENT);
      }
    }
    k = k_next;
    w = w_then;
    my_rel = rel_b;
    e_begin = n_begin;
    e_end = n_end;
    carried = carry;
  }
}

}
}
```

### dream_gnn_amd/csrc/dgmi_sliced.hip

```cpp
#include <hip/hip_runtime.h>
#include <stdint.h>

#include "dgmi_sliced_kernel.h"

namespace dgmi {
namespace {

template <int LPR, int VALS, bool HAS_SS, bool KEEP, bool OFF32>
__global__ __launch_bounds__(kWave* kWavesPerBlock) void spmm_sliced_vec4_kernel(
    const int32_t* __restrict__ segptr, const int32_t* __restrict__ indices,
    const float* __restrict__ vals, const float* __restrict__ X, int64_t ldx,
    const float* __restrict__ src_scale, float* __restrict__ planes, int64_t ldp, int64_t n_dst,
    int64_t row_begin, int64_t row_end, int F, int n_slices, const int32_t* __restrict__ eid,
    const KeepSeg* __restrict__ keep, int n_keep, int touch_lead, SlicedRuns runs, int touch_group) {
  sliced_body<SlicedRowF32, LPR, VALS, HAS_SS, KEEP, OFF32>(segptr, indices, vals, X, ldx, src_scale, planes, ldp, n_dst, row_begin,
                                                            row_end, F, n_slices, eid, keep, n_keep, touch_lead, runs, touch_group);
}

template <int LPR, int VALS, bool KEEP, bool OFF32>
__global__ __launch_bounds__(kWave* kWavesPerBlock, (VALS != 0 && (KEEP || LPR == 8)) ? 4 : 5) void spmm_sliced_bf16_kernel(
    const int32_t* __restrict__ segptr, const int32_t* __restrict__ indices, const float* __restrict__ vals,
    const uint16_t* __restrict__ X, int64_t ldx, float* __restrict__ planes, int64_t ldp, int64_t n_dst, int64_t row_begin,
    int64_t row_end, int F, int n_slices, const int32_t* __restrict__ eid, const KeepSeg* __restrict__ keep, int n_keep,
    int touch_lead, SlicedRuns runs, int touch_group) {
  sliced_body<SlicedRowBf16, LPR, VALS, false, KEEP, OFF32>(segptr, indices, vals, X, ldx, nullptr, planes, ldp, n_dst, row_begin,
                                                            row_end, F, n_slices, eid, keep, n_keep, touch_lead, runs, touch_group);
}

template <bool HAS_DS, int S>
__global__ __launch_bounds__(256) void reduce_planes_kernel(const float* __restrict__ planes, int64_t ldp,
                                                            int64_t rows, int F4, int n_slices,
                                                            const float* __restrict__ dst_scale,
                                                            float* __restrict__ Y, int64_t ldy, Epilogue ep) {
  const int64_t total = rows * F4;
  const int64_t stride = (int64_t)gridDim.x * 256;
  const int64_t plane_stride = rows * ldp;
  const bool dense = (ldp == 4 * (int64_t)F4) && (ldy == ldp);
  for (int64_t t = (int64_t)blockIdx.x * 256 + threadIdx.x; t < total; t += stride) {
    int64_t row, poff, yoff;
    if (dense) {
      row = t / F4;
      poff = yoff = 4 * t;
    } else {
      row = t / F4;
      const int c = (int)(t - row * F4) * 4;
      poff = row * ldp + c;
      yoff = row * ldy + c;
    }
    const float* p = planes + poff;
    float4 acc;
    if (S > 0) {
      float4 v[S > 0 ? S : 1];
#pragma unroll
      for (int s = 0; s < S; ++s) {
        const v4f t = __builtin_nontemporal_load(reinterpret_cast<const v4f*>(p + s * plane_stride));
        v[s] = make_float4(t.x, t.y, t.z, t.w);
      }
      acc = v[0];
#pragma unroll
      for (int s = 1; s < S; ++s) {
        acc.x += v[s].x;
        acc.y += v[s].y;
        acc.z += v[s].z;
        acc.w += v[s].w;
      }
    } else {
      acc = *reinterpret_cast<const float4*>(p);
      for (int s = 1; s < n_slices; ++s) {
        const float4 v = *reinterpret_cast<const float4*>(p + s * plane_stride);
        acc.x += v.x;
        acc.y += v.y;
        acc.z += v.z;
        acc.w += v.w;
      }
    }
    if (HAS_DS) {
      const float d = dst_scale[row];
      acc.x *= d;
      acc.y *= d;
      acc.z *= d;
      acc.w *= d;
    }
    *reinterpret_cast<float4*>(Y + yoff) = epilogue4(ep, acc, row, (int)(yoff - row * ldy));
  }
}

hipError_t reduce_planes(const float* planes, int64_t ldp, int64_t rows, int64_t F, int64_t n_slices, const float* ds, float* y,
                         int64_t ldy, const Epilogue& ep, hipStream_t s) {
  const int F4 = (int)(F / 4);
  int64_t blocks = (rows * F4 + 255) / 256;
  if (blocks > 8192) blocks = 8192;
#define DGMI_REDUCE(D, S)                                                                                        \
  hipLaunchKernelGGL((reduce_planes_kernel<D, S>), dim3((unsigned)blocks), dim3(256), 0, s, planes, ldp, rows, F4, \
                     (int)n_slices, ds, y, ldy, ep)
  if (n_slices == 8) {
    if (ds) DGMI_REDUCE(true, 8); else DGMI_REDUCE(false, 8);
  } else {
    if (ds) DGMI_REDUCE(true, 0); else DGMI_REDUCE(false, 0);
  }
#undef DGMI_REDUCE
  return hipGetLastError();
}

template <typename Row, int LPR, int VALS, bool HAS_SS, bool KEEP, bool OFF32>
void launch_form(const SlicedArgs& a, const SlicedGeometry& g, int64_t row_begin, int64_t row_end, hipStream_t s) {
  const dim3 block(kWave * kWavesPerBlock);
  const auto* X = static_cast<const typename Row::Elem*>(a.X);
  const auto* keep = static_cast<const KeepSeg*>(a.keep);
  if constexpr (!Row::kSrcScale) {
    if constexpr (!HAS_SS)
      hipLaunchKernelGGL((spmm_sliced_bf16_kernel<LPR, VALS, KEEP, OFF32>), g.grid, block, 0, s, a.segptr, a.indices, a.vals, X,
                         a.ldx, a.planes, a.ldp, a.n_dst, row_begin, row_end, (int)a.F, (int)a.n_slices, a.eid, keep, a.n_keep,
                         g.touch_lead, g.runs, g.touch_group);
  } else {
    hipLaunchKernelGGL((spmm_sliced_vec4_kernel<LPR, VALS, HAS_SS, KEEP, OFF32>), g.grid, block, 0, s, a.segptr, a.indices,
                       a.vals, X, a.ldx, a.src_scale, a.planes, a.ldp, a.n_dst, row_begin, row_end, (int)a.F, (int)a.n_slices,
                       a.eid, keep, a.n_keep, g.touch_lead, g.runs, g.touch_group);
  }
}

template <typename Row, int LPR>
hipError_t launch_sliced(const SlicedArgs& a, int64_t row_begin, int64_t row_end, hipStream_t s) {
  typedef void (*Form)(const SlicedArgs&, const SlicedGeometry&, int64_t, int64_t, hipStream_t);
#define DGMI_FORMS(V, S) \
  {{launch_form<Row, LPR, V, S, false, false>, launch_form<Row, LPR, V, S, false, true>}, \
   {launch_form<Row, LPR, V, S, true, false>, launch_form<Row, LPR, V, S, true, true>}}
  static constexpr Form table[3][2][2][2] = {{DGMI_FORMS(0, false), DGMI_FORMS(0, true)},
                                             {DGMI_FORMS(1, false), DGMI_FORMS(1, true)},
                                             {DGMI_FORMS(2, false), DGMI_FORMS(2, true)}};
#undef DGMI_FORMS
  const SlicedGeometry g = sliced_geometry(row_begin, row_end, a.F, a.n_src, a.ldx, a.n_slices, LPR, a.x_bytes);
  table[a.vals ? 1 : (a.id_mult ? 2 : 0)][a.src_scale != nullptr][a.n_keep > 0][g.off32](a, g, row_begin, row_end, s);
  return hipGetLastError();
}

template <typename Row>
hipError_t launch_gather(const SlicedArgs& a, int lpr, int64_t r0, int64_t r1, hipStream_t s) {
  switch (lpr) {
    case 8: return launch_sliced<Row, 8>(a, r0, r1, s);
    case 16: return launch_sliced<Row, 16>(a, r0, r1, s);
    case 32: return launch_sliced<Row, 32>(a, r0, r1, s);
    default:
      if constexpr (Row::kMaxLpr >= 64)
        return launch_sliced<Row, 64>(a, r0, r1, s);
      else
        return launch_sliced<Row, 32>(a, r0, r1, s);
  }
}

template <typename Row>
hipError_t spmm_sliced_chunks(const SlicedArgs& a, hipStream_t s) {
  if (a.n_dst == 0 || a.F == 0) return hipSuccess;
  const int64_t chunk = a.chunk_rows > 0 ? a.chunk_rows : a.n_dst;
  for (int64_t r0 = 0; r0 < a.n_dst; r0 += chunk) {
    const int64_t r1 = r0 + chunk < a.n_dst ? r0 + chunk : a.n_dst;
    const int lpr = sliced_lpr(a.F, a.n_src, a.n_slices, a.n_dst, a.full_width, a.n_keep, a.x_bytes, tuning().sliced_lpr);
    hipError_t err = launch_gather<Row>(a, lpr, r0, r1, s);
    if (err != hipSuccess) return err;
    Epilogue ep = a.ep;
    if (ep.mask != nullptr) ep.mask += r0 * ep.ldm;
    err = reduce_planes(a.planes, a.ldp, r1 - r0, a.F, a.n_slices, a.dst_scale ? a.dst_scale + r0 : nullptr, a.Y + r0 * a.ldy,
                        a.ldy, ep, s);
    if (err != hipSuccess) return err;
  }
  return hipSuccess;
}

}

hipError_t spmm_sliced(const SlicedArgs& a, hipStream_t s) {
  if (a.x_bytes != 4 && a.x_bytes != 2) return hipErrorInvalidValue;
  if (a.x_bytes == 2 && a.src_scale != nullptr) return hipErrorInvalidValue;
  bool owned = false;
  const hipError_t err = spmm_owned_try(a, s, &owned);
  if (err != hipSuccess || owned) return err;
  return a.x_bytes == 4 ? spmm_sliced_chunks<SlicedRowF32>(a, s) : spmm_sliced_chunks<SlicedRowBf16>(a, s);
}

}
```

### dream_gnn_amd/csrc/dgmi_tuning.h

```cpp
#pragma once
#include <stdint.h>

namespace dgmi {

struct Tuning {
  int sliced_rows = 0;
  int sliced_touch_lead = -1;
  int sliced_lpr = 0;
  int sliced_no_off32 = 0;
  int64_t sliced_chunk_rows = 0;
  int64_t sliced_taper_rows = 0;
  int sliced_owned = -1;
  int sliced_owned_grid = 0;
  int sliced_owned_wgs = 0;
  int sliced_owned_rows = 0;
  int64_t sliced_owned_lds_rows = 0;
  int sliced_owned_workers = 0;
  int sliced_owned_slices = 0;
  int sliced_owned_lag = -2;
  int64_t sliced_owned_spin_ticks = 0;
  int64_t select_window_min = 0;
  int select_narrow_window = 0;
  int sort_plain_tiles = 0;
  int knn_screen_first = 0;
  int64_t knn_pool_chunks = 0;
};

Tuning& tuning();

}
```

### dream_gnn_amd/ops.py

```python
from __future__ import annotations

import contextlib
import ctypes
import operator
import os
import threading
from typing import Optional, Tuple

import torch

from . import _lib

_L = _lib.lib
_T = _lib.torch_ops
_NULLCTX = contextlib.nullcontext()
_NO_EPI = (0, 0.0, None, 1.0)

_GATHER_DTYPES = (torch.float32, torch.bfloat16)
_gather_default = threading.local()


def _check_gather_dtype(dtype):
    if dtype is not None and dtype not in _GATHER_DTYPES:
        raise ValueError("gather_dtype must be None, torch.float32 or torch.bfloat16, got %r" % (dtype,))
    return dtype


def _resolve_gather_dtype(dtype):
    if _check_gather_dtype(dtype) is not None:
        return dtype
    return getattr(_gather_default, "dtype", None) or torch.float32


@contextlib.contextmanager
def gather_precision(dtype):
    _check_gather_dtype(dtype)
    prev = getattr(_gather_default, "dtype", None)
    _gather_default.dtype = dtype
    try:
        yield
    finally:
        _gather_default.dtype = prev


def rows_to_bf16(X: torch.Tensor, scale: Optional[torch.Tensor] = None) -> torch.Tensor:
    _require_device(X, scale)
    return _T.rows_to_bf16(X, None if scale is None else scale.reshape(-1).contiguous())


def _ptr(t: Optional[torch.Tensor]):
    return None if t is None else t.data_ptr()


def _stream(device) -> int:
    return torch._C._cuda_getCurrentRawStream(device.index)


def _guard(device):
    if torch.cuda.current_device() == device.index:
        return _NULLCTX
    return torch.cuda.device(device)


def _require_device(*tensors):
    dev = None
    for t in tensors:
        if t is None:
            continue
        if not t.is_cuda:
            raise RuntimeError(
                "dream_gnn_amd ops run on the MI355X only: got a %s tensor. There is no CPU path "
                "(the CPU restatement under oracle/ is test infrastructure)." % t.device)
        if dev is None:
            dev = t.device
        elif t.device != dev:
            raise RuntimeError("tensors on different devices: %s vs %s" % (dev, t.device))
    return dev


def csr_from_coo(row: torch.Tensor, col: torch.Tensor, n_rows: int, n_cols: int = 0,
                 check_range: bool = False, return_flag: bool = False):
    _require_device(row, col)
    indptr, indices, eid, flag = _T.csr_from_coo(row, col, n_rows, n_cols)
    if check_range and int(flag.item()) != 0:
        raise RuntimeError("csr_from_coo: an id is outside [0, %d) x [0, %s)"
                           % (n_rows, n_cols if n_cols > 0 else "unchecked"))
    if return_flag:
        return indptr, indices, eid, flag
    return indptr, indices, eid


def gather_f32(values: torch.Tensor, perm: torch.Tensor) -> torch.Tensor:
    _require_device(values, perm)
    return _T.gather_f32(values, perm)


class SpmmPlan:

    def __init__(self, indptr: torch.Tensor, nnz: int, chunk: Optional[int] = None):
        dev = _require_device(indptr)
        self.n_rows = int(indptr.shape[0] - 1)
        self.nnz = int(nnz)
        self.chunk = int(chunk) if chunk else int(_L.dgmi_spmm_default_chunk(self.n_rows, self.nnz))
        if int(_L.dgmi_spmm_plan_bytes(self.n_rows, self.nnz, self.chunk)) == 0:
            raise RuntimeError("invalid plan parameters (chunk=%d)" % self.chunk)
        self.buf = _T.plan_build(indptr, self.nnz, self.chunk)
        self._pbytes = {}

    def partials_bytes(self, F: int) -> int:
        b = self._pbytes.get(F)
        if b is None:
            b = self._pbytes[F] = int(_L.dgmi_spmm_partials_bytes(self.nnz, self.chunk, int(F)))
        return b

    def header(self):
        return tuple(int(v) for v in self.buf[:64].view(torch.int32).tolist())


def build_plan(indptr: torch.Tensor, nnz: int, chunk: Optional[int] = None) -> SpmmPlan:
    return SpmmPlan(indptr, nnz, chunk)


def _launch_spmm(dev, indptr, indices, vals, X, src_scale, dst_scale, out, plan, n_dst, n_src, F, ldx,
                 eid=None, keep=None, epi=None):
    args = (indptr, indices, vals, eid if keep is not None else None, keep, X, src_scale, dst_scale,
            None if plan is None else plan.buf, 0 if plan is None else plan.chunk)
    epi = epi or _NO_EPI
    if out is None:
        return _T.spmm_csr_raw(*args, *epi)
    _T.spmm_csr_out(*args, out, *epi)
    return out


def _prep_scale(s, n, name):
    if s is None:
        return None
    if s.dim() != 1:
        s = s.reshape(-1)
    if s.dtype != torch.float32 or s.shape[0] != n or not s.is_contiguous():
        if s.dtype != torch.float32:
            raise RuntimeError("%s must be float32" % name)
        if s.shape[0] != n:
            raise RuntimeError("%s has %d entries, expected %d" % (name, s.shape[0], n))
        s = s.contiguous()
    return s


def spmm_csr_raw(indptr, indices, vals, X, src_scale=None, dst_scale=None, out=None,
                 plan: Optional[SpmmPlan] = None, eid=None, keep=None) -> torch.Tensor:
    dev = _require_device(indptr, indices, vals, X, src_scale, dst_scale, out, eid, keep)
    if keep is not None:
        keep = _prep_keep(keep)
    n_dst = indptr.shape[0] - 1
    if plan is not None and (plan.n_rows != n_dst or plan.nnz != indices.shape[0]):
        raise RuntimeError("plan was built for another CSR")
    src_scale = None if src_scale is None else src_scale.reshape(-1)
    dst_scale = None if dst_scale is None else dst_scale.reshape(-1)
    return _launch_spmm(dev, indptr, indices, vals, X, src_scale, dst_scale, out, plan, n_dst, X.shape[0],
                        X.shape[1] if X.dim() == 2 else 0, 0, eid, keep)


def _prep_keep(keep):
    if keep.dtype != torch.int32 or keep.dim() not in (1, 2) or keep.shape[-1] != 8:
        raise RuntimeError("keep must be int32 with 8 words per description, got %s %s" % (keep.dtype, tuple(keep.shape)))
    keep = keep.reshape(-1, 8)
    if keep.shape[0] > 8:
        raise RuntimeError("at most 8 subset descriptions per product")
    return keep if keep.is_contiguous() else keep.contiguous()


def _sliced_ok(X, out) -> bool:
    if X.dtype != torch.float32 or X.stride(1) != 1 or X.stride(0) % 4 != 0 or X.data_ptr() % 16 != 0:
        return False
    return out is None or (out.is_contiguous() and out.data_ptr() % 16 == 0)


def _sliced_bf16_ok(X, out) -> bool:
    if X.dtype == torch.float32:
        return _sliced_ok(X, out)
    if X.dtype != torch.bfloat16 or X.stride(1) != 1 or X.stride(0) % 8 != 0 or X.data_ptr() % 16 != 0:
        return False
    return out is None or (out.is_contiguous() and out.data_ptr() % 16 == 0)


class SlicedCSR:

    N_SLICES = 8

    def __init__(self, dst, src, n_dst, n_src, vals=None, n_slices: int = N_SLICES):
        _require_device(dst, src, vals)
        self.n_dst, self.n_src, self.n_slices = int(n_dst), int(n_src), int(n_slices)
        self.segptr, self.indices, self.eid, self.range_flag = _T.csr_sliced_from_coo(dst, src, self.n_dst, self.n_src,
                                                                                    self.n_slices)
        self.vals = None if vals is None else gather_f32(vals, self.eid)
        self.id_mult = False

    @classmethod
    def from_csr(cls, indptr, indices, eid, n_dst, n_src, n_slices: int = N_SLICES):
        self = cls.__new__(cls)
        self.n_dst, self.n_src, self.n_slices = int(n_dst), int(n_src), int(n_slices)
        self.segptr, self.indices, self.eid, self.range_flag = _T.csr_sliced_from_csr(indptr, indices, eid, self.n_src,
                                                                                    self.n_slices)
        self.vals = None
        self.id_mult = False
        return self

    def compacted(self, keep, vals=None, indices=None, id_mult=False) -> "SlicedCSR":
        c = SlicedCSR.__new__(SlicedCSR)
        c.n_dst, c.n_src, c.n_slices = self.n_dst, self.n_src, self.n_slices
        c.segptr, c.indices, v = _T.compact_layout(self.segptr, self.indices if indices is None else indices, vals, self.eid,
                                                   _prep_keep(keep))
        c.vals = None if vals is None else v
        c.id_mult = bool(id_mult)
        c.eid, c.range_flag = None, self.range_flag
        return c

    _DEFAULT = object()

    def _prescale_pays(self, table_bytes: int, one_pass: bool) -> bool:
        return self._prescale_rule(table_bytes, one_pass, self.n_dst, self.n_slices, int(self.indices.shape[0]))

    @staticmethod
    def _prescale_rule(table_bytes: int, one_pass: bool, n_dst: int, n_slices: int, nnz: int) -> bool:
        if table_bytes < PRESCALE_MIN_TABLE_BYTES:
            return False
        passes = 1 if one_pass or n_dst < 32768 or table_bytes // n_slices <= (4 << 20) else 2
        return table_bytes <= 6 * nnz * passes

    def spmm(self, X, src_scale=None, dst_scale=None, out=None, vals=_DEFAULT, keep=None, epi=None, full_width=False,
             indices=None, id_mult=None, gather_dtype=None):
        vals = self.vals if vals is SlicedCSR._DEFAULT else vals
        _check_gather_dtype(gather_dtype)
        if X.dtype == torch.bfloat16 and src_scale is not None:
            raise RuntimeError("a bfloat16 X cannot take a src_scale: the scale is applied in float32 BEFORE the one rounding "
                               "to bf16 — pass the float32 table (with gather_dtype=torch.bfloat16) or rows_to_bf16(X, src_scale)")
        if not X.is_cuda or X.device != self.segptr.device:
            _require_device(self.segptr, X)
        if X.dim() == 2 and X.shape[0] != self.n_src:
            raise RuntimeError("X has %d rows, the graph has %d source nodes" % (X.shape[0], self.n_src))
        if X.dtype == torch.bfloat16 or gather_dtype == torch.bfloat16:
            if X.dim() != 2 or X.shape[1] % 8 != 0:
                raise RuntimeError("the bf16 gather needs a 2-D table with a multiple of 8 columns, got %s" % (tuple(X.shape),))
            if X.dtype != torch.bfloat16:
                if X.dtype != torch.float32:
                    raise RuntimeError("X must be float32 or bfloat16, got %s" % X.dtype)
                X = _T.rows_to_bf16(X, None if src_scale is None else src_scale.reshape(-1).contiguous())
            id_mult = self.id_mult if id_mult is None else bool(id_mult)
            args = (self.segptr, self.indices if indices is None else indices, vals, self.eid if keep is not None else None,
                    None if keep is None else _prep_keep(keep), X, None if dst_scale is None else dst_scale.reshape(-1),
                    self.n_dst, self.n_slices)
            epi = epi or _NO_EPI
            if out is None:
                return _T.spmm_sliced_bf16_raw(*args, *epi, 1 if full_width else 0, int(id_mult))
            _T.spmm_sliced_bf16_out(*args, out, *epi, 1 if full_width else 0, int(id_mult))
            return out
        if src_scale is not None and X.dim() == 2 and self._prescale_pays(X.shape[0] * X.shape[1] * 4, keep is not None or full_width):
            X = _T.scale_rows(X, src_scale.reshape(-1).contiguous())
            src_scale = None
        id_mult = self.id_mult if id_mult is None else bool(id_mult)
        args = (self.segptr, self.indices if indices is None else indices, vals, self.eid if keep is not None else None,
                None if keep is None else _prep_keep(keep), X, None if src_scale is None else src_scale.reshape(-1),
                None if dst_scale is None else dst_scale.reshape(-1), self.n_dst, self.n_slices)
        epi = epi or _NO_EPI
        passes = 1 if full_width else 0
        if out is None:
            return _T.spmm_sliced_raw(*args, *epi, passes, int(id_mult))
        _T.spmm_sliced_out(*args, out, *epi, passes, int(id_mult))
        return out


FORCE_KERNEL = {"planned": "planned", "sliced": "sliced"}.get(os.environ.get("DGMI_FORCE_KERNEL", ""))
SLICED_MIN_TABLE_BYTES = 6_000_000
SLICED_TIERS = ((48, 420_000_000), (96, 800_000_000), (192, 1_500_000_000))
SLICED_LOW_DEGREE = (32, 20_000_000, 80_000_000)
SPLIT_MIN_TABLE_BYTES = 4_000_000
PRESCALE_MIN_TABLE_BYTES = 8_000_000
COMPACT_DROPPED = os.environ.get("DGMI_COMPACT_DROPPED", "1") != "0"
MULT_FORM = os.environ.get("DGMI_MULT_FORM", "1") != "0"
MULT_REL_TOL = 2.4e-7
MULT_SHIFT, MULT_MAX_IDS = 28, 1 << 28
COLUMN_PASS_MIN_ROWS, LONG_ROW_MIN_DEGREE = 32768, 384
SPLIT_MIN_DEGREE, SPLIT_DENSE_DEGREE = 8, 300
SPLIT_MAX_TABLE_BYTES, SPLIT_MAX_TABLE_BYTES_DENSE = 350_000_000, 900_000_000


def _table_cap(tiers, degree: float) -> int:
    cap = 0
    for d, c in tiers:
        if degree >= d:
            cap = c
    return cap


class _Direction:

    __slots__ = ("transposed", "suffix", "csr_key", "sliced_key", "split_key", "gathered_name", "out_name",
                 "n_rows", "n_cols", "cols_coo", "indptr", "indices", "eid", "plan", "max_deg", "regular", "sliced", "split")

    def __init__(self, suffix, n_rows, n_cols, cols_coo, regular, gathered_name, out_name):
        self.transposed, self.suffix = bool(suffix), suffix
        self.csr_key, self.sliced_key, self.split_key = "csr" + suffix, "sliced" + suffix, "split" + suffix
        self.gathered_name, self.out_name = gathered_name, out_name
        self.n_rows, self.n_cols, self.cols_coo = n_rows, n_cols, cols_coo
        self.indptr = self.indices = self.eid = self.plan = None
        self.max_deg = None
        self.regular = regular
        self.sliced = self.split = None


class _Structure:

    __slots__ = ("n_dst", "n_src", "dst", "src", "nnz", "planned", "validated", "wide", "fwd", "bwd")


for _side, _sfx, _fields in (("fwd", "", ("indptr", "indices", "eid", "plan", "max_deg", "regular", "sliced", "split")),
                             ("bwd", "_t", ("max_deg", "regular", "sliced", "split"))):
    for _f in _fields:
        setattr(_Structure, _f + _sfx, property(operator.attrgetter(_side + "." + _f)))


SPLIT_ROW_EDGES = 256


SPLIT_LIGHT_ROW_EDGES = 24


class _SplitSliced:

    def __init__(self, indptr, eid, cols_coo, n_rows, n_cols):
        dev = indptr.device
        nnz = int(eid.shape[0])
        deg = (indptr[1:] - indptr[:-1]).long()
        light = deg < SPLIT_LIGHT_ROW_EDGES
        n_light = int(light.sum())
        self.has_light = 4 * n_light >= n_rows and n_light < n_rows
        if not self.has_light:
            light = torch.zeros_like(light)
        nv = torch.where(light, torch.zeros_like(deg), torch.clamp((deg + SPLIT_ROW_EDGES - 1) // SPLIT_ROW_EDGES, min=1))
        vptr = torch.zeros(n_rows + 1, dtype=torch.int64, device=dev)
        vptr[1:] = torch.cumsum(nv, 0)
        self.n_virtual = int(vptr[-1])
        rows_p = torch.repeat_interleave(torch.arange(n_rows, device=dev), deg, output_size=nnz)
        rank = torch.arange(nnz, device=dev) - indptr.long()[rows_p]
        vrow_p = (vptr[rows_p] + rank // SPLIT_ROW_EDGES).to(torch.int32)
        cols_p = cols_coo[eid.long()]
        self.n_rows, self.n_cols = n_rows, n_cols
        if not self.has_light:
            vrow_coo = torch.empty(nnz, dtype=torch.int32, device=dev)
            vrow_coo[eid.long()] = vrow_p
            self.sliced = SlicedCSR(vrow_coo, cols_coo, self.n_virtual, n_cols)
            self.c_indptr = vptr.to(torch.int32)
            self.c_indices = torch.arange(self.n_virtual, dtype=torch.int32, device=dev)
            self.c_eid = self.c_light_eid = self.c_order = None
        else:
            heavy_p = ~light[rows_p]
            self.sliced = SlicedCSR(vrow_p[heavy_p].contiguous(), cols_p[heavy_p].contiguous(), self.n_virtual, n_cols)
            self.sliced.eid = eid[heavy_p][self.sliced.eid.long()].contiguous()
            light_p = ~heavy_p
            ent_row = torch.cat([torch.repeat_interleave(torch.arange(n_rows, device=dev), nv, output_size=self.n_virtual), rows_p[light_p]])
            ent_idx = torch.cat([torch.arange(self.n_virtual, dtype=torch.int32, device=dev), cols_p[light_p] + self.n_virtual])
            order = torch.sort(ent_row, stable=True).indices
            self.c_order = order
            self.c_indices = ent_idx[order].contiguous()
            cptr = torch.zeros(n_rows + 1, dtype=torch.int64, device=dev)
            cptr[1:] = torch.cumsum(torch.where(light, deg, nv), 0)
            self.c_indptr = cptr.to(torch.int32)
            self.c_light_eid = eid[light_p]
            never = torch.full((self.n_virtual,), 0x7FFFFFFF, dtype=torch.int32, device=dev)
            self.c_eid = torch.cat([never, self.c_light_eid])[order].contiguous()
        self.c_plan = build_plan(self.c_indptr, int(self.c_indices.shape[0]))

    def combine_values(self, coo_vals):
        if coo_vals is None or not self.has_light:
            return None
        ones = torch.ones(self.n_virtual, dtype=torch.float32, device=coo_vals.device)
        return torch.cat([ones, coo_vals[self.c_light_eid.long()]])[self.c_order].contiguous()

    def spmm(self, X, src_scale, dst_scale, out, vals, keep=None, epi=None, compacted=None, c_vals=None):
        F = X.shape[1]
        if self.has_light:
            buf = torch.empty((self.n_virtual + self.n_cols, F), dtype=torch.float32, device=X.device)
            xs, yv = buf[self.n_virtual:], buf[:self.n_virtual]
            if src_scale is not None:
                torch.mul(X, src_scale.reshape(-1, 1), out=xs)
            else:
                xs.copy_(X)
            if compacted is not None:
                compacted.spmm(xs, None, None, yv)
            else:
                self.sliced.spmm(xs, None, None, yv, vals=vals, keep=keep)
            table, n_table, c_keep = buf, self.n_virtual + self.n_cols, keep
        else:
            if compacted is not None:
                yv = compacted.spmm(X, src_scale, None, None)
            else:
                yv = self.sliced.spmm(X, src_scale, None, None, vals=vals, keep=keep)
            table, n_table, c_keep = yv, self.n_virtual, None
        if out is None:
            out = torch.empty((self.n_rows, F), dtype=torch.float32, device=X.device)
        return _launch_spmm(X.device, self.c_indptr, self.c_indices, c_vals, table, None, dst_scale, out, self.c_plan,
                            self.n_rows, n_table, F, F, eid=self.c_eid, keep=c_keep, epi=epi)


class CSRGraph:

    def __init__(self, dst: torch.Tensor, src: torch.Tensor, n_dst: int, n_src: int,
                 vals: Optional[torch.Tensor] = None, check_range: bool = True, planned: bool = True,
                 regular: Optional[bool] = None, regular_t: Optional[bool] = None):
        _require_device(dst, src, vals)
        S = self._S = _Structure()
        S.n_dst, S.n_src = int(n_dst), int(n_src)
        S.dst = dst.to(torch.int32).contiguous()
        S.src = src.to(torch.int32).contiguous()
        if vals is not None and vals.shape[0] != S.dst.shape[0]:
            raise RuntimeError("vals/edge-list length mismatch")
        S.planned = planned
        S.wide = {}
        S.validated = bool(check_range)
        D = S.fwd = _Direction("", S.n_dst, S.n_src, S.src, bool(regular) if regular is not None else None, "src_scale", "dst_scale")
        S.bwd = _Direction("_t", S.n_src, S.n_dst, S.dst, regular_t, "dst_scale", "src_scale")
        D.indptr, D.indices, D.eid, flag = csr_from_coo(S.dst, S.src, S.n_dst, S.n_src, return_flag=True)
        S.nnz = int(D.indices.shape[0])
        self._set_values(None if vals is None else vals.to(torch.float32).contiguous())
        if check_range:
            self._validate(flag)
        D.plan = build_plan(D.indptr, S.nnz) if planned else None

    def _set_values(self, coo_vals, keep=None):
        self._coo_vals = coo_vals
        self._v = {}
        self._c = {}
        self._keep = keep
        self._mask = None
        self._vals_before_mask = None

    def with_values(self, coo_vals: Optional[torch.Tensor]) -> "CSRGraph":
        if coo_vals is not None and coo_vals.shape[0] != self.nnz:
            raise RuntimeError("expected %d edge values, got %d" % (self.nnz, coo_vals.shape[0]))
        view = object.__new__(CSRGraph)
        view._S = self._S
        view._set_values(None if coo_vals is None else coo_vals.to(torch.float32).contiguous(), self._keep)
        return view

    def masked(self, keep: torch.Tensor) -> "CSRGraph":
        keep = keep.to(torch.float32)
        view = self.with_values(keep if self._coo_vals is None else self._coo_vals * keep)
        view._keep = self._keep
        view._mask = keep if self._mask is None else self._mask * keep
        view._vals_before_mask = self._vals_before_mask if self._mask is not None else self._coo_vals
        view._v["mult"] = False
        return view

    def dropped(self, desc: torch.Tensor) -> "CSRGraph":
        desc = _prep_keep(desc)
        view = object.__new__(CSRGraph)
        view._S = self._S
        view._coo_vals, view._v = self._coo_vals, self._v
        view._c = {}
        view._mask, view._vals_before_mask = self._mask, self._vals_before_mask
        view._keep = desc if self._keep is None else torch.cat([self._keep, desc])
        if view._keep.shape[0] > 8:
            raise RuntimeError("at most 8 subset descriptions per graph view")
        return view

    def keep_mask(self) -> Optional[torch.Tensor]:
        return None if self._keep is None else keep_mask(self._keep, self.nnz)

    def survivors(self) -> Optional[torch.Tensor]:
        m = self.keep_mask()
        if self._mask is not None:
            m = self._mask if m is None else m * self._mask
        return m

    def undropped(self) -> "CSRGraph":
        view = object.__new__(CSRGraph)
        view._S = self._S
        vals = self._coo_vals
        if self._mask is not None:
            vals = self._vals_before_mask
        view._set_values(vals)
        return view

    def _compacted(self, name: str, sliced: "SlicedCSR", mult=None) -> Optional["SlicedCSR"]:
        if self._keep is None or not COMPACT_DROPPED:
            return None
        c = self._c.get(name)
        if c is None:
            if mult is not None:
                c = sliced.compacted(self._keep, None, indices=mult[2], id_mult=True)
            else:
                c = sliced.compacted(self._keep, self._vals_for(name, sliced.eid))
            self._c[name] = c
        return c

    def _mult_form(self):
        if self._coo_vals is None or not MULT_FORM or self._S.n_src > MULT_MAX_IDS or self._S.n_dst > MULT_MAX_IDS:
            return None
        m = self._v.get("mult")
        if m is None:
            if self._capturing():
                return None
            m = False
            for kind, D in (("row", self._S.fwd), ("col", self._S.bwd)):
                D = self._built(D)
                scale, code, fail = _T.row_multiplicity(D.indptr, self._vals_for(D.csr_key, D.eid), MULT_REL_TOL)
                if int(fail.item()) == 0:
                    code_coo = torch.empty_like(code)
                    code_coo[D.eid.long()] = code
                    m = (kind, scale, code_coo)
                    break
            self._v["mult"] = m
        return m or None

    def _mult_ids(self, name: str, sliced: "SlicedCSR"):
        mf = self._mult_form()
        if mf is None:
            return None
        ids = self._v.get(name + "/ids")
        if ids is None:
            ids = self._v[name + "/ids"] = sliced.indices | (mf[2][sliced.eid.long()] << MULT_SHIFT)
        return mf[0], mf[1], ids

    @staticmethod
    def _fold(scale, other):
        return scale if other is None else scale * other.reshape(-1)

    def _combine_vals(self, name: str, split: "_SplitSliced"):
        if self._coo_vals is None or not split.has_light:
            return None
        v = self._v.get(name + "/combine")
        if v is None:
            v = self._v[name + "/combine"] = split.combine_values(self._coo_vals)
        return v

    def _vals_for(self, layout: str, eid: torch.Tensor):
        if self._coo_vals is None:
            return None
        v = self._v.get(layout)
        if v is None:
            v = self._v[layout] = gather_f32(self._coo_vals, eid)
        return v

    n_dst = property(lambda self: self._S.n_dst)
    n_src = property(lambda self: self._S.n_src)
    indptr = property(lambda self: self._S.indptr)
    indices = property(lambda self: self._S.indices)
    eid = property(lambda self: self._S.eid)
    plan = property(lambda self: self._S.plan)
    regular = property(lambda self: self._S.regular)
    regular_t = property(lambda self: self._S.regular_t)
    _sliced = property(lambda self: self._S.sliced)
    _sliced_t = property(lambda self: self._S.sliced_t)

    @property
    def vals(self):
        return self._vals_for("csr", self._S.fwd.eid)

    @property
    def nnz(self) -> int:
        return self._S.nnz

    @property
    def device(self):
        return self._S.fwd.indptr.device

    @staticmethod
    def _is_regular(max_deg: int, nnz: int, n_rows: int) -> bool:
        return max_deg <= max(1024, 32 * (nnz // max(n_rows, 1)))

    def _validate(self, flag: torch.Tensor):
        S, D = self._S, self._S.fwd
        if self.nnz == 0:
            D.regular = True
            return
        bad, max_deg = torch.stack([flag.reshape(()), (D.indptr[1:] - D.indptr[:-1]).max()]).tolist()
        if bad:
            dlo, dhi, slo, shi = (int(v) for v in torch.stack([S.dst.min(), S.dst.max(), S.src.min(), S.src.max()]).tolist())
            if dlo < 0 or dhi >= S.n_dst:
                raise RuntimeError("destination id out of range [0, %d): min %d max %d" % (S.n_dst, dlo, dhi))
            raise RuntimeError("source id out of range [0, %d): min %d max %d" % (S.n_src, slo, shi))
        D.max_deg = int(max_deg)
        D.regular = self._is_regular(int(max_deg), self.nnz, S.n_dst)

    @staticmethod
    def _capturing() -> bool:
        return torch.cuda.is_available() and torch.cuda.is_current_stream_capturing()

    def _decide_regular(self, X, D: _Direction):
        small = X.dim() != 2 or D.n_cols * X.shape[1] * 4 < min(SLICED_MIN_TABLE_BYTES, SPLIT_MIN_TABLE_BYTES)
        if (small and not self._S.validated) or not X.is_cuda or self._capturing():
            return
        indptr = self._built(D).indptr
        D.max_deg = int((indptr[1:] - indptr[:-1]).max()) if self.nnz else 0
        D.regular = self._is_regular(D.max_deg, self.nnz, D.n_rows)

    def _use_sliced(self, F: int, n_rows: int, n_cols: int, regular: bool) -> bool:
        if FORCE_KERNEL is not None:
            return FORCE_KERNEL == "sliced" and F % 4 == 0 and n_rows * SlicedCSR.N_SLICES < 2 ** 31 - 1
        table = n_cols * F * 4
        if not (bool(regular) and F % 4 == 0 and n_rows * SlicedCSR.N_SLICES < 2 ** 31 - 1) or table < SLICED_MIN_TABLE_BYTES:
            return False
        degree = self.nnz / max(n_rows, 1)
        if table <= _table_cap(SLICED_TIERS, degree):
            return True
        lo_deg, lo, hi = SLICED_LOW_DEGREE
        return degree >= lo_deg and lo <= table <= hi

    def _use_split(self, F: int, n_rows: int, n_cols: int, regular) -> bool:
        if FORCE_KERNEL is not None or regular is not False or not self._S.validated:
            return False
        table = n_cols * F * 4
        n_virtual_bound = n_rows + self.nnz // SPLIT_ROW_EDGES
        if F % 4 != 0 or n_virtual_bound * SlicedCSR.N_SLICES >= 2 ** 31 - 1 or table < SPLIT_MIN_TABLE_BYTES:
            return False
        degree = self.nnz / max(n_rows, 1)
        if degree < SPLIT_MIN_DEGREE:
            return False
        return table <= (SPLIT_MAX_TABLE_BYTES_DENSE if degree >= SPLIT_DENSE_DEGREE else SPLIT_MAX_TABLE_BYTES)

    def _few_long_rows(self, F: int, n_rows: int, n_cols: int) -> bool:
        if FORCE_KERNEL is not None or not self._S.validated or n_rows >= COLUMN_PASS_MIN_ROWS:
            return False
        slice_bytes = (n_cols + SlicedCSR.N_SLICES - 1) // SlicedCSR.N_SLICES * F * 4
        return self.nnz >= LONG_ROW_MIN_DEGREE * max(n_rows, 1) and slice_bytes > (4 << 20)

    @staticmethod
    def _plan_if_needed(plan, max_deg):
        if plan is not None and max_deg is not None and max_deg <= plan.chunk:
            return None
        return plan

    def _built(self, D: _Direction) -> _Direction:
        if D.indptr is None:
            S = self._S
            D.indptr, D.indices, D.eid = csr_from_coo(S.src, S.dst, S.n_src)
            D.plan = build_plan(D.indptr, S.nnz) if S.planned else None
        return D

    def _t_struct(self):
        T = self._built(self._S.bwd)
        return T.indptr, T.indices, T.eid, T.plan

    def transposed(self):
        T = self._built(self._S.bwd)
        return T.indptr, T.indices, self._vals_for(T.csr_key, T.eid), T.plan

    def _run(self, D: _Direction, X, col_scale, row_scale, out, epi):
        dev = D.indptr.device
        if not X.is_cuda or X.device != dev:
            _require_device(D.indptr, X)
        if X.dim() == 2 and X.shape[0] != D.n_cols:
            raise RuntimeError("X has %d rows, the graph has %d source nodes" % (X.shape[0], D.n_cols))
        return _launch_spmm(dev, D.indptr, D.indices, self._vals_for(D.csr_key, D.eid), X,
                            None if col_scale is None else col_scale.reshape(-1),
                            None if row_scale is None else row_scale.reshape(-1), out, self._plan_if_needed(D.plan, D.max_deg),
                            D.n_rows, D.n_cols, 0, 0, D.eid if self._keep is not None else None, self._keep, epi)

    def _bf16_gather_reason(self, F: int, D: _Direction) -> Optional[str]:
        if F % 8 != 0:
            return "F = %d is not a multiple of 8 (a lane loads 8 bf16 columns)" % F
        if (bool(D.regular) and self._few_long_rows(F, D.n_rows, D.n_cols)) or not self._use_sliced(F, D.n_rows, D.n_cols, D.regular):
            return ("a %d x %d product at F = %d does not take the plain XCD-local form (it runs the planned, wave-per-row "
                    "or split kernels, which gather float32 only)" % (D.n_rows, D.n_cols, F))
        return None

    def takes_bf16_gather(self, F: int, transposed: bool = False) -> bool:
        D = self._S.bwd if transposed else self._S.fwd
        if D.regular is None:
            self._decide_regular(torch.empty((0, int(F)), dtype=torch.float32, device=self.device), D)
        return self._bf16_gather_reason(int(F), D) is None

    def _bf16_request(self, X, out, gather_dtype, D: _Direction) -> bool:
        if X.dtype != torch.bfloat16 and _resolve_gather_dtype(gather_dtype) != torch.bfloat16:
            return False
        if X.dim() != 2:
            reason = "X is not 2-D"
        else:
            reason = self._bf16_gather_reason(X.shape[1], D)
            if reason is None and not _sliced_bf16_ok(X, out):
                reason = "the rows of X (or out) are not contiguous and 16-byte aligned"
        if reason is not None and X.dtype == torch.bfloat16:
            raise RuntimeError("a bfloat16 X is only taken by the XCD-local bf16 gather, and %s: pass the float32 table" % reason)
        return reason is None

    def _plain_layout(self, D: _Direction, F: int, gathered_scale):
        n = SlicedCSR.N_SLICES
        mf = self._mult_form()
        if (self._coo_vals is None or mf is not None) and (self._keep is None or COMPACT_DROPPED):
            n = _lib.sliced_layout_slices(D.n_rows, D.n_cols, F, mf is not None)
            scaled = gathered_scale is not None or (mf is not None and (mf[0] == "row") == D.transposed)
            if n != SlicedCSR.N_SLICES and scaled and not SlicedCSR._prescale_rule(D.n_cols * F * 4, False, D.n_rows, n, self.nnz):
                n = SlicedCSR.N_SLICES
        return self._layout_of(D, n)

    def _layout_of(self, D, n_slices: int = SlicedCSR.N_SLICES):
        if D.__class__ is not _Direction:
            D = self._S.bwd if D else self._S.fwd
        first = D.sliced
        if first is not None and first.n_slices == n_slices:
            return D.sliced_key, first
        layout = None if first is None else self._S.wide.get((D.transposed, n_slices))
        if layout is None:
            self._built(D)
            layout = SlicedCSR.from_csr(D.indptr, D.indices, D.eid, D.n_rows, D.n_cols, n_slices)
            if first is not None:
                self._S.wide[(D.transposed, n_slices)] = layout
            else:
                D.sliced = layout
        return (D.sliced_key if first is None else "%s/%d" % (D.sliced_key, n_slices)), layout

    def _product(self, D: _Direction, X, gathered_scale, out_scale, out, epi, gather_dtype):
        if D.regular is None:
            self._decide_regular(X, D)
        two_d = X.dim() == 2
        F = X.shape[1] if two_d else 0
        bf16 = self._bf16_request(X, out, gather_dtype, D)
        long_rows = not bf16 and two_d and bool(D.regular) and self._few_long_rows(F, D.n_rows, D.n_cols)
        if bf16 or (two_d and not long_rows and self._use_sliced(F, D.n_rows, D.n_cols, D.regular) and _sliced_ok(X, out)):
            name, layout = self._layout_of(D) if bf16 else self._plain_layout(D, F, gathered_scale)
            mult = self._mult_ids(name, layout)
            if mult is not None:
                if (mult[0] == "row") != D.transposed:
                    out_scale = self._fold(mult[1], out_scale)
                else:
                    gathered_scale = self._fold(mult[1], gathered_scale)
            gd = None
            if bf16:
                if X.dtype != torch.bfloat16:
                    gd = torch.bfloat16
                elif gathered_scale is not None:
                    raise RuntimeError("a bfloat16 X cannot take a scale on the gathered rows (src_scale, or the row scale of this "
                                       "graph's `scale x multiplicity` values): it is applied in float32 before the one rounding — "
                                       "pass the float32 table")
            c = self._compacted(name, layout, mult)
            if c is not None:
                return c.spmm(X, gathered_scale, out_scale, out, epi=epi, gather_dtype=gd)
            if mult is not None:
                return layout.spmm(X, gathered_scale, out_scale, out, vals=None, keep=self._keep, epi=epi, indices=mult[2],
                                   id_mult=True, gather_dtype=gd)
            return layout.spmm(X, gathered_scale, out_scale, out, vals=self._vals_for(name, layout.eid), keep=self._keep, epi=epi,
                               gather_dtype=gd)
        if two_d and _sliced_ok(X, out) and (self._use_split(F, D.n_rows, D.n_cols, D.regular) or (
                long_rows and self._use_sliced(F, D.n_rows, D.n_cols, D.regular))):
            split = D.split
            if split is None:
                split = D.split = _SplitSliced(D.indptr, D.eid, D.cols_coo, D.n_rows, D.n_cols)
            c = self._compacted(D.split_key, split.sliced)
            return split.spmm(X, _prep_scale(gathered_scale, D.n_cols, D.gathered_name), _prep_scale(out_scale, D.n_rows, D.out_name),
                              out, None if c is not None else self._vals_for(D.split_key, split.sliced.eid), keep=self._keep,
                              epi=epi, compacted=c, c_vals=self._combine_vals(D.split_key, split))
        return self._run(D, X, gathered_scale, out_scale, out, epi)

    def spmm(self, X, src_scale=None, dst_scale=None, out=None, epi=None, gather_dtype=None):
        return self._product(self._S.fwd, X, src_scale, dst_scale, out, epi, gather_dtype)

    def spmm_t(self, dY, src_scale=None, dst_scale=None, out=None, gather_dtype=None):
        return self._product(self._built(self._S.bwd), dY, dst_scale, src_scale, out, None, gather_dtype)


class _SpMM(torch.autograd.Function):
    @staticmethod
    def forward(ctx, X, g: CSRGraph, src_scale, dst_scale, gather_dtype=torch.float32):
        ctx.g, ctx.gather_dtype = g, gather_dtype
        ctx.save_for_backward(src_scale, dst_scale)
        return g.spmm(X, src_scale, dst_scale, gather_dtype=gather_dtype)

    @staticmethod
    def backward(ctx, dY):
        src_scale, dst_scale = ctx.saved_tensors
        dX = None
        if ctx.needs_input_grad[0]:
            if not dY.is_contiguous():
                dY = dY.contiguous()
            dX = ctx.g.spmm_t(dY, src_scale, dst_scale, gather_dtype=ctx.gather_dtype)
        return dX, None, None, None, None


class _SpMMEpilogue(torch.autograd.Function):

    @staticmethod
    def forward(ctx, X, g: CSRGraph, src_scale, dst_scale, act, slope, mask, mask_scale, gather_dtype=torch.float32):
        y = g.spmm(X, src_scale, dst_scale, epi=(act, slope, mask, mask_scale), gather_dtype=gather_dtype)
        ctx.g, ctx.epi, ctx.gather_dtype = g, (act, slope, mask_scale), gather_dtype
        ctx.save_for_backward(src_scale, dst_scale, y, mask)
        return y

    @staticmethod
    def backward(ctx, dY):
        src_scale, dst_scale, y, mask = ctx.saved_tensors
        act, slope, mask_scale = ctx.epi
        dX = None
        if ctx.needs_input_grad[0]:
            g_pre = epilogue_backward(dY.contiguous(), y, mask, act, slope, mask_scale)
            dX = ctx.g.spmm_t(g_pre, src_scale, dst_scale, gather_dtype=ctx.gather_dtype)
        return dX, None, None, None, None, None, None, None, None


def colsum_rows_(feat_ext, coef, n: int, R: int, i0: int):
    _require_device(feat_ext, coef)
    _T.colsum_rows_(feat_ext, coef, n, R, i0)
    return feat_ext


def colsum_rows_backward_(gf, coef, gs, n: int, R: int, i0: int):
    _require_device(gf, coef, gs)
    _T.colsum_rows_backward_(gf, coef, gs, n, R, i0)
    return gf


def epilogue_backward(dY, Y, mask, act, slope, mask_scale):
    _require_device(dY, Y, mask)
    return _T.epilogue_backward(dY, Y, mask, act, slope, mask_scale)


def spmm_csr_act_dropout(g: CSRGraph, X, src_scale=None, dst_scale=None, act: int = 0, slope: float = 0.0,
                         mask: Optional[torch.Tensor] = None, mask_scale: float = 1.0, gather_dtype=None) -> torch.Tensor:
    if src_scale is not None and src_scale.requires_grad or dst_scale is not None and dst_scale.requires_grad:
        raise RuntimeError("spmm_csr: gradients w.r.t. the diagonal scales are not part of the path")
    return _SpMMEpilogue.apply(X, g, src_scale, dst_scale, act, slope, mask, mask_scale, _resolve_gather_dtype(gather_dtype))


def spmm_csr(g: CSRGraph, X: torch.Tensor, src_scale: Optional[torch.Tensor] = None,
             dst_scale: Optional[torch.Tensor] = None, gather_dtype=None) -> torch.Tensor:
    if src_scale is not None and src_scale.requires_grad or dst_scale is not None and dst_scale.requires_grad:
        raise RuntimeError("spmm_csr: gradients w.r.t. the diagonal scales are not part of the path")
    return _SpMM.apply(X, g, src_scale, dst_scale, _resolve_gather_dtype(gather_dtype))


def _check_tables(A, B, n_src, n_dst):
    if n_src is not None and A.shape[0] < n_src:
        raise RuntimeError("source feature table has %d rows, the edge list addresses %d source nodes" % (A.shape[0], n_src))
    if n_dst is not None and B.shape[0] < n_dst:
        raise RuntimeError("destination feature table has %d rows, the edge list addresses %d destination nodes"
                           % (B.shape[0], n_dst))


def gather_concat_raw(src, dst, A, B, out=None, n_src=None, n_dst=None) -> torch.Tensor:
    _require_device(src, dst, A, B, out)
    _check_tables(A, B, n_src, n_dst)
    y = _T.gather_concat_raw(src, dst, A, B)
    if out is not None:
        out.copy_(y)
        return out
    return y


class EdgePairs:

    def __init__(self, src: torch.Tensor, dst: torch.Tensor, n_src: int, n_dst: int, check_range: bool = True):
        _require_device(src, dst)
        self.src = src.to(torch.int32).contiguous()
        self.dst = dst.to(torch.int32).contiguous()
        self.n_src, self.n_dst = int(n_src), int(n_dst)
        self.E = int(self.src.shape[0])
        if check_range and self.E:
            lo = torch.stack([self.src.min(), self.dst.min()]).min()
            hi_s, hi_d = self.src.max(), self.dst.max()
            lo, hi_s, hi_d = (int(v) for v in torch.stack([lo, hi_s, hi_d]).tolist())
            if lo < 0 or hi_s >= self.n_src or hi_d >= self.n_dst:
                raise RuntimeError("decoder edge id out of range")
        self._by_src = self._by_dst = None

    def _group(self, key, n):
        iota = torch.arange(self.E, dtype=torch.int32, device=key.device)
        g = CSRGraph(key, iota, n, self.E, check_range=False, regular=False, regular_t=False)
        return g

    def by_src(self) -> "CSRGraph":
        if self._by_src is None:
            self._by_src = self._group(self.src, self.n_src)
        return self._by_src

    def by_dst(self) -> "CSRGraph":
        if self._by_dst is None:
            self._by_dst = self._group(self.dst, self.n_dst)
        return self._by_dst


class _GatherConcat(torch.autograd.Function):
    @staticmethod
    def forward(ctx, A, B, pairs: EdgePairs):
        ctx.pairs = pairs
        ctx.Fa, ctx.Fb = A.shape[1], B.shape[1]
        return gather_concat_raw(pairs.src, pairs.dst, A, B, n_src=pairs.n_src, n_dst=pairs.n_dst)

    @staticmethod
    def backward(ctx, dOut):
        pairs, Fa, Fb = ctx.pairs, ctx.Fa, ctx.Fb
        dOut = dOut.contiguous()
        dA = dB = None
        if ctx.needs_input_grad[0]:
            dA = pairs.by_src().spmm(dOut[:, :Fa])
        if ctx.needs_input_grad[1]:
            dB = pairs.by_dst().spmm(dOut[:, Fa:])
        return dA, dB, None


def gather_concat(pairs: EdgePairs, A: torch.Tensor, B: torch.Tensor) -> torch.Tensor:
    return _GatherConcat.apply(A, B, pairs)


def gather_add_raw(src, dst, A, B, bias=None, out=None, n_src=None, n_dst=None, act: int = 0) -> torch.Tensor:
    _require_device(src, dst, A, B, bias, out)
    _check_tables(A, B, n_src, n_dst)
    y = _T.gather_add_raw(src, dst, A, B, bias, int(act))
    if out is not None:
        out.copy_(y)
        return out
    return y


class _GatherAdd(torch.autograd.Function):
    @staticmethod
    def forward(ctx, A, B, bias, pairs: EdgePairs):
        ctx.pairs = pairs
        return gather_add_raw(pairs.src, pairs.dst, A, B, bias, n_src=pairs.n_src, n_dst=pairs.n_dst)

    @staticmethod
    def backward(ctx, dOut):
        pairs = ctx.pairs
        dOut = dOut.contiguous()
        dA = pairs.by_src().spmm(dOut) if ctx.needs_input_grad[0] else None
        dB = pairs.by_dst().spmm(dOut) if ctx.needs_input_grad[1] else None
        dbias = dOut.sum(0) if ctx.needs_input_grad[2] else None
        return dA, dB, dbias, None


def gather_add(pairs: EdgePairs, A: torch.Tensor, B: torch.Tensor, bias: Optional[torch.Tensor] = None):
    return _GatherAdd.apply(A, B, bias, pairs)


class _GatherAddReluDropout(torch.autograd.Function):

    @staticmethod
    def forward(ctx, A, B, bias, pairs: EdgePairs, p: float):
        y = gather_add_raw(pairs.src, pairs.dst, A, B, bias, n_src=pairs.n_src, n_dst=pairs.n_dst, act=1)
        y = torch.nn.functional.dropout(y, p, True)
        ctx.pairs, ctx.scale = pairs, 1.0 / (1.0 - p)
        ctx.save_for_backward(y)
        return y

    @staticmethod
    def backward(ctx, dY):
        (y,) = ctx.saved_tensors
        pairs = ctx.pairs
        dZ = epilogue_backward(dY.contiguous(), y, None, 2, 0.0, ctx.scale)
        dA = pairs.by_src().spmm(dZ) if ctx.needs_input_grad[0] else None
        dB = pairs.by_dst().spmm(dZ) if ctx.needs_input_grad[1] else None
        dbias = dZ.sum(0) if ctx.needs_input_grad[2] else None
        return dA, dB, dbias, None, None


def gather_add_relu_dropout(pairs: EdgePairs, A, B, bias, p: float):
    return _GatherAddReluDropout.apply(A, B, bias, pairs, float(p))


def knn_cosine_supported(N: int, D: int, k: int) -> bool:
    return bool(_L.dgmi_knn_cosine_supported(int(N), int(D), int(k)))


def knn_cosine_topk(xn: torch.Tensor, k: int) -> torch.Tensor:
    _require_device(xn)
    return _T.knn_cosine_topk(xn, int(k))


PAIR_TOPK_MAX_K = _lib.PAIR_TOPK_MAX_K


def pair_mlp_topk(P: torch.Tensor, Q: torch.Tensor, W2: torch.Tensor, b2: torch.Tensor, w3: torch.Tensor,
                  b3: torch.Tensor, known_drug: Optional[torch.Tensor], known_dis: Optional[torch.Tensor],
                  k: int) -> Tuple[torch.Tensor, torch.Tensor, torch.Tensor]:
    k = int(k)
    if not 1 <= k <= PAIR_TOPK_MAX_K:
        raise ValueError("k must be in 1..%d (the on-chip top-k limit), got %d" % (PAIR_TOPK_MAX_K, k))
    _require_device(P, Q, W2, b2, w3, b3, known_drug, known_dis)
    drug, dis, logit, info = _T.pair_mlp_topk(P, Q, W2, b2.reshape(-1), w3.reshape(-1), b3.reshape(-1), known_drug,
                                              known_dis, k)
    n, bad = (int(v) for v in info.tolist())
    if bad:
        raise RuntimeError("pair_mlp_topk: a known (drug, disease) id is outside [0, %d) x [0, %d)"
                           % (P.shape[0], Q.shape[0]))
    return drug[:n].long(), dis[:n].long(), logit[:n]


ROW_TOPK_MAX_K = _lib.ROW_TOPK_MAX_K


def pair_mlp_row_topk(X: torch.Tensor, C: torch.Tensor, W2: torch.Tensor, b2: torch.Tensor, w3: torch.Tensor,
                      b3: torch.Tensor, known_query: Optional[torch.Tensor], known_cand: Optional[torch.Tensor],
                      k: int) -> Tuple[torch.Tensor, torch.Tensor, torch.Tensor]:
    k = int(k)
    if not 1 <= k <= ROW_TOPK_MAX_K:
        raise ValueError("k must be in 1..%d (the per-row on-chip top-k limit), got %d" % (ROW_TOPK_MAX_K, k))
    _require_device(X, C, W2, b2, w3, b3, known_query, known_cand)
    cand, logit, count, info = _T.pair_mlp_row_topk(X, C, W2, b2.reshape(-1), w3.reshape(-1), b3.reshape(-1), known_query,
                                                    known_cand, k)
    if int(info[1]):
        raise RuntimeError("pair_mlp_row_topk: a known (query, candidate) id is outside [0, %d) x [0, %d)"
                           % (X.shape[0], C.shape[0]))
    return cand.long(), logit, count


PAIR_EMIT_MAX_RECORDS = _lib.PAIR_EMIT_MAX_RECORDS


class TooManyPairs(RuntimeError):

    def __init__(self, count: int, max_pairs: int):
        super().__init__("%d novel pairs reach the cut, more than max_pairs = %d: raise the cut or max_pairs"
                         % (count, max_pairs))
        self.count = int(count)
        self.max_pairs = int(max_pairs)


def _check_max_pairs(max_pairs) -> int:
    max_pairs = int(max_pairs)
    if not 1 <= max_pairs <= PAIR_EMIT_MAX_RECORDS:
        raise ValueError("max_pairs must be in 1..%d (the record buffer limit), got %d" % (PAIR_EMIT_MAX_RECORDS, max_pairs))
    return max_pairs


def _pair_emit(P, Q, W2, b2, w3, b3, known_drug, known_dis, min_logit, capacity):
    _require_device(P, Q, W2, b2, w3, b3, known_drug, known_dis)
    drug = torch.empty(capacity, dtype=torch.int32, device=P.device)
    dis = torch.empty_like(drug)
    logit = torch.empty(capacity, dtype=torch.float32, device=P.device)
    count, info = _T.pair_mlp_emit(P, Q, W2, b2.reshape(-1), w3.reshape(-1), b3.reshape(-1), known_drug, known_dis,
                                   float(min_logit), drug, dis, logit)
    n, _, bad = (int(v) for v in torch.cat([count, info.long()]).tolist())
    if bad:
        raise RuntimeError("pair_mlp_emit: a known (drug, disease) id is outside [0, %d) x [0, %d)"
                           % (P.shape[0], Q.shape[0]))
    return drug, dis, logit, n


def pair_mlp_above(P: torch.Tensor, Q: torch.Tensor, W2: torch.Tensor, b2: torch.Tensor, w3: torch.Tensor,
                   b3: torch.Tensor, known_drug: Optional[torch.Tensor], known_dis: Optional[torch.Tensor],
                   min_logit: float, max_pairs: int = 1 << 20) -> Tuple[torch.Tensor, torch.Tensor, torch.Tensor, int]:
    max_pairs = _check_max_pairs(max_pairs)
    drug, dis, logit, n = _pair_emit(P, Q, W2, b2, w3, b3, known_drug, known_dis, min_logit, max_pairs)
    if n > max_pairs:
        raise TooManyPairs(n, max_pairs)
    _T.pair_records_sort(drug, dis, logit, n)
    return drug[:n].long(), dis[:n].long(), logit[:n], n


def pair_mlp_count_above(P: torch.Tensor, Q: torch.Tensor, W2: torch.Tensor, b2: torch.Tensor, w3: torch.Tensor,
                         b3: torch.Tensor, known_drug: Optional[torch.Tensor], known_dis: Optional[torch.Tensor],
                         min_logit: float) -> int:
    return _pair_emit(P, Q, W2, b2, w3, b3, known_drug, known_dis, min_logit, 0)[3]


def _pair_list(pair_query, pair_cand):
    for name, t in (("pair_query", pair_query), ("pair_cand", pair_cand)):
        if not isinstance(t, torch.Tensor) or t.dim() != 1 or t.dtype not in (torch.int32, torch.int64):
            raise ValueError("%s must be a 1-D int32 / int64 tensor of ids" % name)
    if pair_query.numel() != pair_cand.numel():
        raise ValueError("pair id lists differ in length: %d vs %d" % (pair_query.numel(), pair_cand.numel()))


def pair_mlp_score_list(X: torch.Tensor, C: torch.Tensor, W2: torch.Tensor, b2: torch.Tensor, w3: torch.Tensor,
                        b3: torch.Tensor, pair_query: torch.Tensor, pair_cand: torch.Tensor) -> torch.Tensor:
    _pair_list(pair_query, pair_cand)
    _require_device(X, C, W2, b2, w3, b3, pair_query, pair_cand)
    logit, info = _T.pair_mlp_score_list(X, C, W2, b2.reshape(-1), w3.reshape(-1), b3.reshape(-1), pair_query, pair_cand)
    if int(info[0]):
        raise RuntimeError("pair_mlp_score_list: a listed (query, candidate) id is outside [0, %d) x [0, %d)"
                           % (X.shape[0], C.shape[0]))
    return logit


class _PairMlpTrain(torch.autograd.Function):

    @staticmethod
    def forward(ctx, P, Q, W2, b2, w3, b3, pairs: EdgePairs, p: float, seed):
        _check_tables(P, Q, pairs.n_src, pairs.n_dst)
        logit, _ = _T.pair_mlp_train_forward(P, Q, W2, b2.reshape(-1), w3.reshape(-1), b3.reshape(-1), pairs.src, pairs.dst,
                                             p, seed)
        ctx.pairs, ctx.p = pairs, p
        ctx.save_for_backward(P, Q, W2, b2, w3, b3, seed)
        return logit

    @staticmethod
    @torch.autograd.function.once_differentiable
    def backward(ctx, dlogit):
        P, Q, W2, b2, w3, b3, seed = ctx.saved_tensors
        pairs = ctx.pairs
        dZ1, dW2, db2, dw3, db3, _ = _T.pair_mlp_train_backward(P, Q, W2, b2.reshape(-1), w3.reshape(-1), b3.reshape(-1),
                                                                pairs.src, pairs.dst, ctx.p, seed, dlogit.contiguous())
        need = ctx.needs_input_grad
        if pairs.E == 0:
            dP, dQ = (torch.zeros_like(P) if need[0] else None), (torch.zeros_like(Q) if need[1] else None)
        else:
            dP = pairs.by_src().spmm(dZ1) if need[0] else None
            dQ = pairs.by_dst().spmm(dZ1) if need[1] else None
        return (dP, dQ, dW2 if need[2] else None, db2.reshape(b2.shape) if need[3] else None,
                dw3.reshape(w3.shape) if need[4] else None, db3.reshape(b3.shape) if need[5] else None, None, None, None)


def pair_mlp_train(P: torch.Tensor, Q: torch.Tensor, W2: torch.Tensor, b2: torch.Tensor, w3: torch.Tensor, b3: torch.Tensor,
                   pairs: EdgePairs, p: float, seed: Optional[torch.Tensor] = None) -> torch.Tensor:
    if not isinstance(pairs, EdgePairs):
        raise TypeError("pairs must be an ops.EdgePairs, got %s" % type(pairs).__name__)
    p = float(p)
    if not 0.0 <= p < 1.0:
        raise ValueError("dropout p must be in [0, 1), got %r" % (p,))
    _require_device(P, Q, W2, b2, w3, b3, seed)
    if seed is None:
        seed = torch.randint(0, 2 ** 62, (1,), dtype=torch.int64, device=P.device)
    elif seed.dtype != torch.int64 or seed.numel() != 1:
        raise ValueError("seed must be a 1-element int64 device tensor")
    seed = seed.reshape(1)
    pair_mlp_train.last_seed = seed
    return _PairMlpTrain.apply(P, Q, W2, b2, w3, b3, pairs, p, seed)


pair_mlp_train.last_seed = None


ATTN_FUSE_BLOCK_ROWS = 64
ATTN_FUSE_MAX_WORKGROUPS = 1024
_ATTN_HIDDEN = 16


class _AttentionFuse(torch.autograd.Function):

    @staticmethod
    def forward(ctx, a, b, W1, b1, w2, mult):
        A, B = (a[:, 0], a[:, 1]) if b is None else (a, b)
        out, beta = _T.attn_fuse_forward(A, B, mult, W1, b1.reshape(-1), w2.reshape(-1))
        ctx.stacked = b is None
        ctx.save_for_backward(a, b, W1, b1, w2, mult)
        ctx.mark_non_differentiable(beta)
        return out, beta

    @staticmethod
    @torch.autograd.function.once_differentiable
    def backward(ctx, dout, _dbeta):
        a, b, W1, b1, w2, mult = ctx.saved_tensors
        A, B = (a[:, 0], a[:, 1]) if ctx.stacked else (a, b)
        dA, dB, dW1, db1, dw2 = _T.attn_fuse_backward(A, B, mult, W1, b1.reshape(-1), w2.reshape(-1), dout)
        need = ctx.needs_input_grad
        if ctx.stacked:
            n, F = dA.shape
            if n > 0 and dA.stride(0) == 2 * F and dB.data_ptr() == dA.data_ptr() + 4 * F:
                da = dA.as_strided((n, 2, F), (2 * F, F, 1))
            else:
                da = torch.stack([dA, dB], 1)
            db = None
        else:
            da, db = dA, dB
        return (da if need[0] else None, db if need[1] else None, dW1 if need[2] else None,
                db1.reshape(b1.shape) if need[3] else None, dw2.reshape(w2.shape) if need[4] else None, None)


def _check_attention(A, B, W1, b1, w2, mult):
    if A.dim() != 2 or B.dim() != 2 or A.shape != B.shape:
        raise ValueError("a and b must be two (n, F) tables of one shape, got %s and %s" % (tuple(A.shape), tuple(B.shape)))
    n, F = A.shape
    if F % 4 != 0 or not 4 <= F <= 512:
        raise ValueError("the width must be a multiple of 4 in [4, 512], got %d" % F)
    if W1.dim() != 2 or W1.shape[0] != _ATTN_HIDDEN or b1.numel() != _ATTN_HIDDEN or w2.numel() != _ATTN_HIDDEN:
        raise ValueError("only hidden size %d is supported: W1 %s, b1 %s, w2 %s"
                         % (_ATTN_HIDDEN, tuple(W1.shape), tuple(b1.shape), tuple(w2.shape)))
    if W1.shape[1] != F:
        raise ValueError("W1 must be (%d, %d), got %s" % (_ATTN_HIDDEN, F, tuple(W1.shape)))
    if mult is not None and tuple(mult.shape) != (n, 2):
        raise ValueError("mult must be (%d, 2), got %s" % (n, tuple(mult.shape)))
    for name, t in (("a", A), ("b", B), ("W1", W1), ("b1", b1), ("w2", w2), ("mult", mult)):
        if t is not None and t.dtype != torch.float32:
            raise ValueError("%s must be float32, got %s" % (name, t.dtype))


def attention_fuse(a: torch.Tensor, b: torch.Tensor, W1: torch.Tensor, b1: torch.Tensor, w2: torch.Tensor,
                   mult: Optional[torch.Tensor] = None):
    _require_device(a, b, W1, b1, w2, mult)
    if mult is not None and not mult.is_contiguous():
        mult = mult.contiguous()
    W1, b1, w2 = (t if t.is_contiguous() else t.contiguous() for t in (W1, b1, w2))
    if b is None:
        if a.dim() != 3 or a.shape[1] != 2:
            raise ValueError("the stacked form takes an (n, 2, F) tensor, got %s" % (tuple(a.shape),))
        _check_attention(a[:, 0], a[:, 1], W1, b1, w2, mult)
    else:
        _check_attention(a, b, W1, b1, w2, mult)
    return _AttentionFuse.apply(a, b, W1, b1, w2, mult)


def pair_mlp_rank_list(X: torch.Tensor, C: torch.Tensor, W2: torch.Tensor, b2: torch.Tensor, w3: torch.Tensor,
                       b3: torch.Tensor, pair_query: torch.Tensor, pair_cand: torch.Tensor,
                       known_query: Optional[torch.Tensor] = None,
                       known_cand: Optional[torch.Tensor] = None) -> Tuple[torch.Tensor, torch.Tensor, torch.Tensor]:
    _pair_list(pair_query, pair_cand)
    _require_device(X, C, W2, b2, w3, b3, pair_query, pair_cand, known_query, known_cand)
    logit, above, total, info = _T.pair_mlp_rank_list(X, C, W2, b2.reshape(-1), w3.reshape(-1), b3.reshape(-1), pair_query,
                                                      pair_cand, known_query, known_cand)
    bad_pair, bad_known = (int(v) for v in info.tolist())
    if bad_pair:
        raise RuntimeError("pair_mlp_rank_list: a listed (query, candidate) id is outside [0, %d) x [0, %d)"
                           % (X.shape[0], C.shape[0]))
    if bad_known:
        raise RuntimeError("pair_mlp_rank_list: a known (query, candidate) id is outside [0, %d) x [0, %d)"
                           % (X.shape[0], C.shape[0]))
    return logit, above, total


_CURVE_FLAGS = ("a score is NaN", "a label is neither 0 nor 1", "a segment id is out of range")


class CurveStats:

    def __init__(self, count: torch.Tensor, area: torch.Tensor, info: torch.Tensor):
        self.count, self.area, self.info = count, area, info
        self.P, self.N, self.tp, self.fp, self.groups, self.u2 = count.unbind(1)
        self.auroc, self.aupr = area.unbind(1)

    def accuracy(self) -> torch.Tensor:
        return (self.tp + (self.N - self.fp)).double() / (self.P + self.N).double()

    def f1(self) -> torch.Tensor:
        return (2 * self.tp).double() / (self.tp + self.fp + self.P).double()

    def macro(self) -> Tuple[torch.Tensor, torch.Tensor]:
        return torch.nanmean(self.auroc), torch.nanmean(self.aupr)


def curve_areas(score: torch.Tensor, label: torch.Tensor, segment: Optional[torch.Tensor] = None, n_segments: int = 0,
                threshold: float = 0.0, check: bool = True) -> CurveStats:
    _require_device(score, label, segment)
    n_segments = int(n_segments)
    if (segment is None) != (n_segments == 0):
        raise ValueError("segment ids and n_segments > 0 go together")
    stats = CurveStats(*_T.curve_areas(score.detach(), label, segment, n_segments, float(threshold)))
    if check:
        flags = int(stats.info[0])
        if flags:
            raise RuntimeError("curve_areas: " + "; ".join(m for b, m in enumerate(_CURVE_FLAGS) if flags >> b & 1))
    return stats

def random_subset_select(E: int, keep: int, seed: int, device, e_offset: int = 0) -> torch.Tensor:
    device = torch.device(device)
    if device.type != "cuda":
        raise RuntimeError("dream_gnn_amd ops run on the MI355X only: got device %s" % device)
    return _T.random_subset_select(torch.empty(0, device=device), E, keep, _signed64(seed), e_offset)


def _signed64(seed: int) -> int:
    seed &= 0xFFFFFFFFFFFFFFFF
    return seed - (1 << 64) if seed >= 1 << 63 else seed


def random_subset_select_batch(Es, keeps, seeds, device, e_offsets=None) -> torch.Tensor:
    device = torch.device(device)
    if device.type != "cuda":
        raise RuntimeError("dream_gnn_amd ops run on the MI355X only: got device %s" % device)
    n = len(Es)
    offs = [0] * n if e_offsets is None else list(e_offsets)
    if isinstance(seeds, torch.Tensor):
        _require_device(seeds)
        seeds = seeds.reshape(-1).to(torch.int64).contiguous()
        parts = [_T.random_subset_select_batch_dseed(seeds[i:i + 8], list(Es[i:i + 8]), list(keeps[i:i + 8]), offs[i:i + 8])
                 for i in range(0, n, 8)]
        return parts[0] if len(parts) == 1 else torch.cat(parts)
    like = torch.empty(0, device=device)
    parts = [_T.random_subset_select_batch(like, list(Es[i:i + 8]), list(keeps[i:i + 8]),
                                           [_signed64(s) for s in seeds[i:i + 8]], offs[i:i + 8])
             for i in range(0, n, 8)]
    return parts[0] if len(parts) == 1 else torch.cat(parts)


def keep_mask(desc: torch.Tensor, E: int) -> torch.Tensor:
    _require_device(desc)
    return _T.keep_mask(_prep_keep(desc), E)


def random_subset_mask(E: int, keep: int, seed: int, device) -> torch.Tensor:
    device = torch.device(device)
    if device.type != "cuda":
        raise RuntimeError("dream_gnn_amd ops run on the MI355X only: got device %s" % device)
    mask = torch.empty(E, dtype=torch.float32, device=device)
    nbytes = int(_L.dgmi_random_subset_workspace_bytes())
    ws = torch.empty(nbytes, dtype=torch.uint8, device=device)
    with _guard(device):
        _lib.check(_L.dgmi_random_subset_mask_f32(E, keep, seed & 0xFFFFFFFFFFFFFFFF, _ptr(mask), _ptr(ws), nbytes,
                                                  _stream(device)), "dgmi_random_subset_mask_f32")
    return mask
```

Before: 37.39 billion.

## Fuse gathered-side scale into owned SpMM via per-column code table in LDS

Adds a scaled variant of the owned SpMM kernel. Each column index carries an 11-bit code that points into a small table of distinct scale values held in LDS, so the kernel applies the source/degree scale inline instead of prescaling X in a separate pass. Code tables are built with torch.unique on the host side and cached per scale tensor version. The path only runs for certain plan/table-size classes and adds LDS pressure, plus a rebuild cost whenever the scale changes.

```diff
diff --git a/dream_gnn_amd/_lib.py b/dream_gnn_amd/_lib.py
--- a/dream_gnn_amd/_lib.py
+++ b/dream_gnn_amd/_lib.py
@@ -136,6 +136,13 @@
                                                                      ctypes.c_size_t, _vp]),
 }
 
+SCALE_SIGNATURES = {
+    "dgmi_spmm_owned_scaled_takes": (ctypes.c_int32, [_i64, _i64, _i64, _i64, ctypes.c_int32, ctypes.c_int32, ctypes.c_int32]),
+    "dgmi_spmm_owned_scaled_f32": (ctypes.c_int, [_vp, _vp, _vp, _i64, _vp, ctypes.c_int32, _vp, _vp, _i64, _i64, _i64, _i64,
+                                                  ctypes.c_int32, ctypes.c_int32] + _EPI + [ctypes.POINTER(ctypes.c_int32), _vp]),
+}
+SCALE_CODE_SHIFT, SCALE_CODE_BITS = 17, 11
+
 
 class DgmiError(RuntimeError):
     """A non-zero dgmi_status came back from the C ABI."""
@@ -151,7 +158,7 @@
                               + list(ABOVE_SIGNATURES.items()) + list(BF16_SIGNATURES.items())
                               + list(GIVEN_SIGNATURES.items()) + list(CURVE_SIGNATURES.items())
                               + list(LAYOUT_SIGNATURES.items()) + list(TRAIN_SIGNATURES.items())
-                              + list(ATTN_SIGNATURES.items())):
+                              + list(ATTN_SIGNATURES.items()) + list(SCALE_SIGNATURES.items())):
         fn = getattr(lib, name)
         fn.restype = res
         fn.argtypes = args
@@ -184,6 +191,24 @@
     return int(lib.dgmi_sliced_layout_slices(int(n_dst), int(n_src), int(F), 1 if id_mult else 0))
 
 
+def owned_scaled_takes(n_dst: int, n_src: int, F: int, ldx: int, n_slices: int, id_mult: bool, n_codes: int) -> bool:
+    return bool(lib.dgmi_spmm_owned_scaled_takes(int(n_dst), int(n_src), int(F), int(ldx), int(n_slices), 1 if id_mult else 0,
+                                                 int(n_codes)))
+
+
+def spmm_owned_scaled(segptr, words, X, table, dst_scale, out, n_src: int, n_slices: int, id_mult: bool, epi) -> bool:
+    act, slope, mask, mask_scale = epi
+    taken = ctypes.c_int32(0)
+    with torch.cuda.device(X.device):
+        check(lib.dgmi_spmm_owned_scaled_f32(
+            segptr.data_ptr(), words.data_ptr(), X.data_ptr(), X.stride(0), table.data_ptr(), table.numel(),
+            None if dst_scale is None else dst_scale.data_ptr(), out.data_ptr(), out.stride(0), out.shape[0], int(n_src),
+            X.shape[1], int(n_slices), 1 if id_mult else 0, int(act), float(slope), None if mask is None else mask.data_ptr(),
+            0 if mask is None else mask.stride(0), float(mask_scale), ctypes.byref(taken),
+            torch.cuda.current_stream(X.device).cuda_stream), "dgmi_spmm_owned_scaled_f32")
+    return taken.value == 1
+
+
 def check(status: int, what: str) -> None:
     if status != 0:
         raise DgmiError("%s failed: %s (status %d)" % (what, lib.dgmi_status_string(status).decode(), status))
diff --git a/dream_gnn_amd/csrc/dgmi_api.hip b/dream_gnn_amd/csrc/dgmi_api.hip
--- a/dream_gnn_amd/csrc/dgmi_api.hip
+++ b/dream_gnn_amd/csrc/dgmi_api.hip
@@ -7,6 +7,7 @@
 #include "dgmi_bf16.h"
 #include "dgmi_keep.h"
 #include "dgmi_layout.h"
+#include "dgmi_scale.h"
 #include "dgmi_kernels.h"
 #include "dgmi_tuning.h"
 
@@ -41,6 +42,7 @@
     v.sliced_owned_lds_rows = env_ll("DGMI_SLICED_OWNED_LDS_ROWS", 0);
     v.sliced_owned_workers = (int)env_ll("DGMI_SLICED_OWNED_WORKERS", 0);
     v.sliced_owned_slices = (int)env_ll("DGMI_SLICED_OWNED_SLICES", 0);
+    v.sliced_owned_scaled = (int)env_ll("DGMI_SLICED_OWNED_SCALED", -1);
     v.sliced_owned_lag = (int)env_ll("DGMI_SLICED_OWNED_LAG", -2);
     v.sliced_owned_spin_ticks = env_ll("DGMI_SLICED_OWNED_SPIN_TICKS", 0);
     v.select_window_min = env_ll("DGMI_SELECT_WINDOW_MIN", 0);
@@ -73,6 +75,7 @@
   else if (strcmp(name, "sliced_owned_lds_rows") == 0) t.sliced_owned_lds_rows = value;
   else if (strcmp(name, "sliced_owned_workers") == 0) t.sliced_owned_workers = (int)value;
   else if (strcmp(name, "sliced_owned_slices") == 0) t.sliced_owned_slices = (int)value;
+  else if (strcmp(name, "sliced_owned_scaled") == 0) t.sliced_owned_scaled = (int)value;
   else if (strcmp(name, "sliced_owned_lag") == 0) t.sliced_owned_lag = (int)value;
   else if (strcmp(name, "sliced_owned_spin_ticks") == 0) t.sliced_owned_spin_ticks = value;
   else if (strcmp(name, "select_window_min") == 0) t.select_window_min = value;
@@ -376,6 +379,53 @@
   return dgmi::sliced_layout_slices(n_dst, n_src, F, id_multiplicity == 1);
 }
 
+static dgmi::SlicedArgs scaled_args(const int32_t* segptr, const int32_t* coded, const float* X, int64_t ldx, const float* table,
+                                    int32_t n_codes, const float* dst_scale, float* Y, int64_t ldy, int64_t n_dst, int64_t n_src,
+                                    int64_t F, int32_t n_slices, int32_t id_multiplicity, const dgmi::Epilogue& ep) {
+  dgmi::SlicedArgs a{segptr, coded, nullptr, X, 4, ldx, nullptr, dst_scale, Y, ldy, n_dst, n_src, F, n_slices, nullptr, F, n_dst,
+                     nullptr, nullptr, 0, ep, false, id_multiplicity == 1};
+  a.scale_table = table;
+  a.n_codes = n_codes;
+  return a;
+}
+
+DGMI_API int32_t dgmi_spmm_owned_scaled_takes(int64_t n_dst, int64_t n_src, int64_t F, int64_t ldx, int32_t n_slices,
+                                              int32_t id_multiplicity, int32_t n_codes) {
+  if (n_dst < 1 || n_src < 1 || F < 1 || F % 4 != 0 || ldx < F || ldx % 4 != 0 || n_dst >= INT32_MAX || F > INT32_MAX ||
+      n_slices < 1 || n_slices > 64 || id_multiplicity < 0 || id_multiplicity > 1)
+    return 0;
+  static const float kSome = 0.f;
+  return dgmi::spmm_owned_scaled_takes(scaled_args(nullptr, nullptr, nullptr, ldx, &kSome, n_codes, nullptr, nullptr, F, n_dst,
+                                                   n_src, F, n_slices, id_multiplicity, {0, 0.f, nullptr, 0, 1.f}))
+             ? 1
+             : 0;
+}
+
+DGMI_API int dgmi_spmm_owned_scaled_f32(const int32_t* segptr, const int32_t* coded_indices, const float* X, int64_t ldx,
+                                        const float* table, int32_t n_codes, const float* dst_scale, float* Y, int64_t ldy,
+                                        int64_t n_dst, int64_t n_src, int64_t F, int32_t n_slices, int32_t id_multiplicity,
+                                        int32_t act, float act_slope, const float* out_mask, int64_t ld_mask,
+                                        float out_mask_scale, int32_t* taken, dgmi_stream_t stream) {
+  if (taken == nullptr) return DGMI_ERR_INVALID_ARG;
+  *taken = 0;
+  if (n_dst < 0 || n_src < 0 || F < 0 || n_slices < 1 || n_slices > 64 || !epilogue_ok(act, out_mask, ld_mask, F) ||
+      id_multiplicity < 0 || id_multiplicity > 1 || n_codes < 0)
+    return DGMI_ERR_INVALID_ARG;
+  if (out_mask != nullptr && (ld_mask % 4 != 0 || (reinterpret_cast<uintptr_t>(out_mask) & 15))) return DGMI_ERR_INVALID_ARG;
+  if (n_dst >= INT32_MAX || n_src >= INT32_MAX || F > INT32_MAX) return DGMI_ERR_TOO_LARGE;
+  if (n_dst == 0 || F == 0) return DGMI_OK;
+  if (segptr == nullptr || coded_indices == nullptr || Y == nullptr || table == nullptr || X == nullptr) return DGMI_ERR_INVALID_ARG;
+  if (ldx < F || ldy < F || F % 4 != 0 || ldx % 4 != 0 || ldy % 4 != 0) return DGMI_ERR_INVALID_ARG;
+  if ((reinterpret_cast<uintptr_t>(X) & 15) || (reinterpret_cast<uintptr_t>(Y) & 15)) return DGMI_ERR_INVALID_ARG;
+  if (static_cast<const void*>(X) == static_cast<const void*>(Y)) return DGMI_ERR_INVALID_ARG;
+  const dgmi::SlicedArgs a = scaled_args(segptr, coded_indices, X, ldx, table, n_codes, dst_scale, Y, ldy, n_dst, n_src, F,
+                                         n_slices, id_multiplicity, {act, act_slope, out_mask, ld_mask, out_mask_scale});
+  bool owned = false;
+  const hipError_t err = dgmi::spmm_owned_scaled(a, as_stream(stream), &owned);
+  *taken = err == hipSuccess && owned ? 1 : 0;
+  return from_hip(err);
+}
+
 DGMI_API int dgmi_gather_concat_f32(const int32_t* src, const int32_t* dst, int64_t E, const float* A,
                                     int64_t lda, int64_t Fa, const float* B, int64_t ldb, int64_t Fb,
                                     float* out, int64_t ldo, dgmi_stream_t stream) {
diff --git a/dream_gnn_amd/csrc/dgmi_kernels.h b/dream_gnn_amd/csrc/dgmi_kernels.h
--- a/dream_gnn_amd/csrc/dgmi_kernels.h
+++ b/dream_gnn_amd/csrc/dgmi_kernels.h
@@ -103,6 +103,9 @@
 constexpr int kMultShift = 28;
 constexpr int kMultMax = 7;
 constexpr uint32_t kMultIdMask = 0x0fffffffu;
+constexpr int kScaleShift = 17;
+constexpr int kScaleBits = 11;
+constexpr uint32_t kScaleIdMask = (1u << kScaleShift) - 1u;
 
 struct SlicedArgs {
   const int32_t* segptr;
@@ -126,7 +129,12 @@
   Epilogue ep;
   bool full_width;
   bool id_mult;
-};
+  const float* scale_table = nullptr;
+  int n_codes = 0;
+};
+
+bool spmm_owned_scaled_takes(const SlicedArgs& a);
+hipError_t spmm_owned_scaled(const SlicedArgs& a, hipStream_t s, bool* taken);
 
 hipError_t row_multiplicity_f32(const int32_t* indptr, const float* vals, int64_t n_rows, float rel_tol, float* row_scale,
                                 int32_t* mult, int32_t* fail, hipStream_t s);
diff --git a/dream_gnn_amd/csrc/dgmi_owned.hip b/dream_gnn_amd/csrc/dgmi_owned.hip
--- a/dream_gnn_amd/csrc/dgmi_owned.hip
+++ b/dream_gnn_amd/csrc/dgmi_owned.hip
@@ -36,6 +36,37 @@
     unsigned* __restrict__ arrive, int lag, int64_t spin_ticks, int workers, Epilogue ep) {
   owned_body<OwnedRowBf16, LPR, VALS, OFF32, kOwnedWaves, false>(segptr, indices, X, ldx, dst_scale, Y, ldy, n_dst, F, pl, arrive,
                                                                  lag, spin_ticks, workers, ep);
+}
+
+constexpr size_t kOwnedScaleLdsBytes = sizeof(float) << kScaleBits;
+template <int LPR, int VALS>
+__global__ __launch_bounds__(kWave* kOwnedWaves, 4) void spmm_owned_scaled_kernel(
+    const int32_t* __restrict__ segptr, const int32_t* __restrict__ indices, const float* __restrict__ X, int64_t ldx,
+    const float* __restrict__ dst_scale, float* __restrict__ Y, int64_t ldy, int64_t n_dst, int F, OwnedPlan pl, int workers,
+    Epilogue ep, const float* __restrict__ table, int n_codes) {
+  owned_body<OwnedRowF32, LPR, VALS, true, kOwnedWaves, false, true>(segptr, indices, X, ldx, dst_scale, Y, ldy, n_dst, F, pl, nullptr,
+                                                                     -1, 0, workers, ep, table, n_codes);
+}
+
+constexpr bool owned_scaled_built(int lpr) { return lpr == 16 || lpr == 32; }
+
+template <int LPR>
+hipError_t launch_owned_scaled(const SlicedArgs& a, const OwnedPlan& pl, int64_t grid, hipStream_t s) {
+  const int workers = tuning().sliced_owned_workers > 0 && tuning().sliced_owned_workers < kOwnedWorkers ? tuning().sliced_owned_workers : 0;
+  const size_t lds = pl.lds_bytes + kOwnedScaleLdsBytes;
+#define DGMI_OWNED_SCALED(V)                                                                                              \
+  do {                                                                                                                    \
+    auto kern = &spmm_owned_scaled_kernel<LPR, V>;                                                                        \
+    static const hipError_t attr =                                                                                        \
+        hipFuncSetAttribute(reinterpret_cast<const void*>(kern), hipFuncAttributeMaxDynamicSharedMemorySize, 160 << 10);  \
+    if (attr != hipSuccess) return attr;                                                                                  \
+    hipLaunchKernelGGL(kern, dim3((unsigned)grid), dim3(kWave* kOwnedWaves), lds, s, a.segptr, a.indices,                 \
+                       static_cast<const float*>(a.X), a.ldx, a.dst_scale, a.Y, a.ldy, a.n_dst, (int)a.F, pl, workers, a.ep, \
+                       a.scale_table, a.n_codes);                                                                         \
+  } while (0)
+  if (a.id_mult) DGMI_OWNED_SCALED(2); else DGMI_OWNED_SCALED(0);
+#undef DGMI_OWNED_SCALED
+  return hipGetLastError();
 }
 
 template <typename Row, int LPR, int VALS, bool OFF32, int WAVES>
@@ -156,9 +187,41 @@
   }
 }
 
+bool owned_class_scaled(const OwnedPlan& pl, bool id_mult, int64_t table_bytes) {
+  const auto mib = [&](int64_t lo, int64_t hi) { return table_bytes >= (lo << 20) && table_bytes <= (hi << 20); };
+  if (pl.slices == kOwnedSlices) {
+    if (pl.col_rounds == 1 && pl.row_rounds == 2 && !id_mult && mib(16, 32)) return true;
+    if (pl.col_rounds == 2 && pl.row_rounds == 1 && id_mult && mib(48, 64)) return true;
+    if (pl.col_rounds == 1 && pl.row_rounds == 1 && id_mult && mib(16, 32)) return true;
+  }
+  if (pl.slices == kOwnedWideSlices && pl.col_rounds == 1 && pl.row_rounds == 1 && !id_mult && mib(48, 64)) return true;
+  return false;
+}
+
+hipError_t owned_try(const SlicedArgs& a, hipStream_t s, bool* taken, bool launch);
+
 }
 
 hipError_t spmm_owned_try(const SlicedArgs& a, hipStream_t s, bool* taken) {
+  *taken = false;
+  if (a.scale_table != nullptr) return hipErrorInvalidValue;
+  return owned_try(a, s, taken, true);
+}
+
+bool spmm_owned_scaled_takes(const SlicedArgs& a) {
+  bool taken = false;
+  return a.scale_table != nullptr && owned_try(a, nullptr, &taken, false) == hipSuccess && taken;
+}
+
+hipError_t spmm_owned_scaled(const SlicedArgs& a, hipStream_t s, bool* taken) {
+  *taken = false;
+  if (a.scale_table == nullptr) return hipErrorInvalidValue;
+  return owned_try(a, s, taken, true);
+}
+
+namespace {
+
+hipError_t owned_try(const SlicedArgs& a, hipStream_t s, bool* taken, bool launch) {
   *taken = false;
   const Tuning& tune = tuning();
   if (tune.sliced_owned == 0) return hipSuccess;
@@ -181,6 +244,18 @@
   if (tune.sliced_owned != 1 && rule == 0) return hipSuccess;
   const bool off32 = !tune.sliced_no_off32 && (a.n_src * a.ldx + a.F) * a.x_bytes < ((int64_t)1 << 32);
   bool resident = true;
+  if (a.scale_table != nullptr) {
+    const bool wanted = tune.sliced_owned_scaled == 1 ||
+                        (tune.sliced_owned_scaled < 0 && (tune.sliced_owned == 1 || (rule == 1 && owned_class_scaled(pl, a.id_mult, table_bytes))));
+    if (!wanted || a.x_bytes != 4 || a.n_src > ((int64_t)1 << kScaleShift) || a.n_codes < 1 || a.n_codes > (1 << kScaleBits) ||
+        !off32 || !owned_scaled_built(lpr) || pl.lds_bytes + kOwnedScaleLdsBytes > (size_t)(160 << 10) || tune.sliced_owned_lag >= 0 ||
+        tune.sliced_owned_wgs == 2)
+      return hipSuccess;
+    *taken = true;
+    if (!launch) return hipSuccess;
+    return lpr == 16 ? launch_owned_scaled<16>(a, pl, grid, s) : launch_owned_scaled<32>(a, pl, grid, s);
+  }
+  if (!launch) return hipSuccess;
   if (a.x_bytes == 2) {
     *taken = true;
     return launch_owned_width<OwnedRowBf16, kOwnedWaves>(a, pl, lpr, grid, off32, -1, 0, s, &resident);
@@ -204,6 +279,8 @@
   return launch_owned_width<OwnedRowF32, kOwnedWaves>(a, pl, lpr, grid, off32, lag, spin, s, &resident);
 }
 
+}
+
 int sliced_layout_slices(int64_t n_dst, int64_t n_src, int64_t F, bool id_mult) {
   const Tuning& tune = tuning();
   if (n_dst < 1 || n_src < 1 || F < 1 || F % 4 != 0 || tune.sliced_owned == 0 || tune.sliced_chunk_rows > 0) return kOwnedSlices;
diff --git a/dream_gnn_amd/csrc/dgmi_owned_kernel.h b/dream_gnn_amd/csrc/dgmi_owned_kernel.h
--- a/dream_gnn_amd/csrc/dgmi_owned_kernel.h
+++ b/dream_gnn_amd/csrc/dgmi_owned_kernel.h
@@ -1,6 +1,8 @@
 #pragma once
 #include <hip/hip_runtime.h>
 #include <stdint.h>
+
+#include <type_traits>
 
 #include "dgmi_owned_common.h"
 #include "dgmi_sliced_common.h"
@@ -80,16 +82,24 @@
   }
 };
 
-template <typename Row, int LPR, int VALS, bool OFF32, int WAVES, bool GATE>
+__device__ __forceinline__ float owned_mul_rn(float a, float b) {
+  float r;
+  asm("v_mul_f32 %0, %1, %2" : "=v"(r) : "v"(a), "v"(b));
+  return r;
+}
+
+template <typename Row, int LPR, int VALS, bool OFF32, int WAVES, bool GATE, bool SCALED = false>
 __device__ __forceinline__ void owned_body(const int32_t* __restrict__ segptr, const int32_t* __restrict__ indices,
                                            const typename Row::Elem* __restrict__ X, int64_t ldx,
                                            const float* __restrict__ dst_scale, float* __restrict__ Y, int64_t ldy,
                                            int64_t n_dst, int F, OwnedPlan pl, unsigned* __restrict__ arrive, int lag,
-                                           int64_t spin_ticks, int workers, Epilogue ep) {
+                                           int64_t spin_ticks, int workers, Epilogue ep,
+                                           const float* __restrict__ table = nullptr, int n_codes = 0) {
   typedef typename Row::Elem Elem;
   typedef typename Row::Acc Acc;
   constexpr bool MULT = VALS == 2;
-  constexpr int kIdMask = MULT ? (int)kMultIdMask : 0x7fffffff;
+  constexpr int kIdMask = SCALED ? (int)kScaleIdMask : (MULT ? (int)kMultIdMask : 0x7fffffff);
+  static_assert(!SCALED || (std::is_same<Elem, float>::value && kScaleShift + kScaleBits <= kMultShift), "an fp32 table; the code lies below the multiplicity");
   constexpr int kRowSlots = Row::kLaneSlots * LPR;
   constexpr bool CARRY = WAVES == kOwnedWaves && MULT && Row::kCarry;
   extern __shared__ float4 lds_rows[];
@@ -104,6 +114,9 @@
   int* counter = phase_cnt + pl.phases;
   int* open = counter + 1;
   for (int i = threadIdx.x; i < pl.tasks + pl.phases + 2; i += blockDim.x) done[i] = 0;
+  float* lds_scale = reinterpret_cast<float*>(open + 1);
+  if (SCALED)
+    for (int i = threadIdx.x; i < (1 << kScaleBits); i += blockDim.x) lds_scale[i] = i < n_codes ? table[i] : 0.f;
   __syncthreads();
   const int total = pl.phases * T;
   const int label = (int)(blockIdx.x & 7u);
@@ -197,6 +210,7 @@
   constexpr int W = kOwnedWindow;
   static_assert(W <= 8 && kMultShift == 28 && LPR % W == 0, "at most eight 4-bit multiplicity fields, shifted down from bit 28");
   typename Row::Reg v[W];
+  float sc[SCALED ? W : 1];
   int idx[W];
   int nidx[W];
   uint32_t mults = 0, mults_in = 0, nmults = 0;
@@ -207,7 +221,7 @@
       int id = __shfl(batch_idx, gbase + u, kWave);
       if (MULT) {
         fields = (fields >> 4) | ((uint32_t)id & ((uint32_t)kMultMax << kMultShift));
-        id &= kIdMask;
+        if (!SCALED) id &= kIdMask;
       }
       out[u] = id;
     }
@@ -216,6 +230,13 @@
   auto read_ids = [&](int batch_idx) { read_batch(batch_idx, idx, mults_in); };
 
   const uint32_t row_bytes = (uint32_t)ldx * (uint32_t)sizeof(Elem);
+  auto issue = [&](int u, const Elem* Xcol, int word, uint32_t cbytes) {
+    if (SCALED) {
+      sc[u] = lds_scale[((uint32_t)word >> kScaleShift) & ((1u << kScaleBits) - 1u)];
+      word &= kIdMask;
+    }
+    v[u] = Row::template load<OFF32>(X, Xcol, word, ldx, row_bytes, cbytes);
+  };
   int k = grab();
   OwnedWork w = owned_decode(pl, wg, T, k, grp);
   int e_begin = 0, e_end = 0;
@@ -231,7 +252,7 @@
     if (L > 0 && !carried) {
       read_ids(nxt_idx);
 #pragma unroll
-      for (int u = 0; u < W; ++u) v[u] = Row::template load<OFF32>(X, Xc, idx[u], ldx, row_bytes, col_bytes);
+      for (int u = 0; u < W; ++u) issue(u, Xc, idx[u], col_bytes);
       mults = mults_in;
     }
     const int k_next = grab();
@@ -275,7 +296,13 @@
           m = (float)(((mults >> (32 - 4 * W)) & (uint32_t)kMultMax) + 1u);
           mults >>= 4;
         }
-        Row::template add<MULT>(acc, m, v[u]);
+        if constexpr (SCALED) {
+          const float s = sc[u];
+          const float4 t = make_float4(owned_mul_rn(s, v[u].x), owned_mul_rn(s, v[u].y), owned_mul_rn(s, v[u].z), owned_mul_rn(s, v[u].w));
+          Row::template add<MULT>(acc, m, t);
+        } else {
+          Row::template add<MULT>(acc, m, v[u]);
+        }
       };
       auto rows_before = [&](int p) {
         while (p >= row_end) {
@@ -297,7 +324,7 @@
         for (int u = 0; u < W; ++u) {
           rows_before(p0 + u);
           add(u);
-          v[u] = Row::template load<OFF32>(X, Xc, idx[u], ldx, row_bytes, col_bytes);
+          issue(u, Xc, idx[u], col_bytes);
           __builtin_amdgcn_sched_barrier(0);
         }
         mults = mults_in;
@@ -338,7 +365,7 @@
             rows_before(p0 + u);
             add(u);
           }
-          v[u] = Row::template load<OFF32>(X, Xn, nidx[u], ldx, row_bytes, ncol_bytes);
+          issue(u, Xn, nidx[u], ncol_bytes);
           __builtin_amdgcn_sched_barrier(0);
         }
         mults = nmults;
diff --git a/dream_gnn_amd/csrc/dgmi_sliced.hip b/dream_gnn_amd/csrc/dgmi_sliced.hip
--- a/dream_gnn_amd/csrc/dgmi_sliced.hip
+++ b/dream_gnn_amd/csrc/dgmi_sliced.hip
@@ -171,6 +171,7 @@
 hipError_t spmm_sliced(const SlicedArgs& a, hipStream_t s) {
   if (a.x_bytes != 4 && a.x_bytes != 2) return hipErrorInvalidValue;
   if (a.x_bytes == 2 && a.src_scale != nullptr) return hipErrorInvalidValue;
+  if (a.scale_table != nullptr) return hipErrorInvalidValue;
   bool owned = false;
   const hipError_t err = spmm_owned_try(a, s, &owned);
   if (err != hipSuccess || owned) return err;
diff --git a/dream_gnn_amd/csrc/dgmi_tuning.h b/dream_gnn_amd/csrc/dgmi_tuning.h
--- a/dream_gnn_amd/csrc/dgmi_tuning.h
+++ b/dream_gnn_amd/csrc/dgmi_tuning.h
@@ -17,6 +17,7 @@
   int64_t sliced_owned_lds_rows = 0;
   int sliced_owned_workers = 0;
   int sliced_owned_slices = 0;
+  int sliced_owned_scaled = -1;
   int sliced_owned_lag = -2;
   int64_t sliced_owned_spin_ticks = 0;
   int64_t select_window_min = 0;
diff --git a/dream_gnn_amd/ops.py b/dream_gnn_amd/ops.py
--- a/dream_gnn_amd/ops.py
+++ b/dream_gnn_amd/ops.py
@@ -279,6 +279,9 @@
 MULT_FORM = os.environ.get("DGMI_MULT_FORM", "1") != "0"
 MULT_REL_TOL = 2.4e-7
 MULT_SHIFT, MULT_MAX_IDS = 28, 1 << 28
+SCALE_CODES = os.environ.get("DGMI_SCALE_CODES", "1") != "0"
+SCALE_SHIFT, SCALE_BITS = _lib.SCALE_CODE_SHIFT, _lib.SCALE_CODE_BITS
+SCALE_MAX_IDS, SCALE_MAX_CODES = 1 << SCALE_SHIFT, 1 << SCALE_BITS
 COLUMN_PASS_MIN_ROWS, LONG_ROW_MIN_DEGREE = 32768, 384
 SPLIT_MIN_DEGREE, SPLIT_DENSE_DEGREE = 8, 300
 SPLIT_MAX_TABLE_BYTES, SPLIT_MAX_TABLE_BYTES_DENSE = 350_000_000, 900_000_000
@@ -310,7 +313,7 @@
 
 class _Structure:
 
-    __slots__ = ("n_dst", "n_src", "dst", "src", "nnz", "planned", "validated", "wide", "fwd", "bwd")
+    __slots__ = ("n_dst", "n_src", "dst", "src", "nnz", "planned", "validated", "wide", "fwd", "bwd", "scale_builds")
 
 
 for _side, _sfx, _fields in (("fwd", "", ("indptr", "indices", "eid", "plan", "max_deg", "regular", "sliced", "split")),
@@ -417,6 +420,7 @@
         S.planned = planned
         S.wide = {}
         S.validated = bool(check_range)
+        S.scale_builds = 0
         D = S.fwd = _Direction("", S.n_dst, S.n_src, S.src, bool(regular) if regular is not None else None, "src_scale", "dst_scale")
         S.bwd = _Direction("_t", S.n_src, S.n_dst, S.dst, regular_t, "dst_scale", "src_scale")
         D.indptr, D.indices, D.eid, flag = csr_from_coo(S.dst, S.src, S.n_dst, S.n_src, return_flag=True)
@@ -525,6 +529,36 @@
     def _fold(scale, other):
         return scale if other is None else scale * other.reshape(-1)
 
+    @staticmethod
+    def scale_codes(scale: torch.Tensor, ids: torch.Tensor):
+        if scale.dim() != 1 or scale.dtype != torch.float32 or scale.shape[0] > SCALE_MAX_IDS:
+            raise RuntimeError("scale_codes takes a 1-D float32 scale of at most %d entries" % SCALE_MAX_IDS)
+        bits, code = torch.unique(scale.contiguous().view(torch.int32), return_inverse=True)
+        if bits.shape[0] > SCALE_MAX_CODES:
+            return None, None
+        words = ids | (code.to(torch.int32)[(ids & (SCALE_MAX_IDS - 1)).long()] << SCALE_SHIFT)
+        return bits.view(torch.float32), words
+
+    def _scale_ids(self, name: str, scale: torch.Tensor, ids: torch.Tensor):
+        if self._capturing() or scale.dtype != torch.float32 or not scale.is_cuda or scale.dim() != 1 or scale.shape[0] > SCALE_MAX_IDS:
+            return None
+        slot = name + "/scale_ids"
+        entry = self._v.get(slot)
+        if entry is False:
+            return None
+        key = (scale.data_ptr(), scale.shape[0], scale.stride(0), scale._version)
+        if entry is not None and entry["key"] == key:
+            entry["misses"] = 0
+            return entry["coded"]
+        misses = 0 if entry is None else entry["misses"] + 1
+        if misses >= 2:
+            self._v[slot] = False
+            return None
+        table, words = self.scale_codes(scale, ids)
+        self._S.scale_builds += 1
+        self._v[slot] = {"key": key, "ref": scale, "misses": misses, "coded": None if table is None else (table, words)}
+        return self._v[slot]["coded"]
+
     def _combine_vals(self, name: str, split: "_SplitSliced"):
         if self._coo_vals is None or not split.has_light:
             return None
@@ -719,10 +753,12 @@
         if bf16 or (two_d and not long_rows and self._use_sliced(F, D.n_rows, D.n_cols, D.regular) and _sliced_ok(X, out)):
             name, layout = self._layout_of(D) if bf16 else self._plain_layout(D, F, gathered_scale)
             mult = self._mult_ids(name, layout)
+            stable = None if gathered_scale is None else gathered_scale.reshape(-1)
             if mult is not None:
                 if (mult[0] == "row") != D.transposed:
                     out_scale = self._fold(mult[1], out_scale)
                 else:
+                    stable = mult[1] if gathered_scale is None else None
                     gathered_scale = self._fold(mult[1], gathered_scale)
             gd = None
             if bf16:
@@ -735,6 +771,10 @@
             c = self._compacted(name, layout, mult)
             if c is not None:
                 return c.spmm(X, gathered_scale, out_scale, out, epi=epi, gather_dtype=gd)
+            if stable is not None and not bf16 and self._keep is None and (mult is not None or self._coo_vals is None):
+                y = self._scaled_product(name, layout, X, stable, mult, out_scale, out, epi)
+                if y is not None:
+                    return y
             if mult is not None:
                 return layout.spmm(X, gathered_scale, out_scale, out, vals=None, keep=self._keep, epi=epi, indices=mult[2],
                                    id_mult=True, gather_dtype=gd)
@@ -750,6 +790,36 @@
                               out, None if c is not None else self._vals_for(D.split_key, split.sliced.eid), keep=self._keep,
                               epi=epi, compacted=c, c_vals=self._combine_vals(D.split_key, split))
         return self._run(D, X, gathered_scale, out_scale, out, epi)
+
+    def _scaled_product(self, name, layout, X, scale, mult, out_scale, out, epi):
+        F = X.shape[1]
+        if not SCALE_CODES or layout.n_src > SCALE_MAX_IDS or scale.shape[0] != layout.n_src or X.shape[0] != layout.n_src:
+            return None
+        if not X.is_cuda or X.device != layout.segptr.device or scale.device != X.device:
+            return None
+        if self._v.get(name + "/scale_ids") is False or not layout._prescale_pays(layout.n_src * F * 4, False):
+            return None
+        takes = lambda n: _lib.owned_scaled_takes(layout.n_dst, layout.n_src, F, X.stride(0), layout.n_slices, mult is not None, n)
+        if not takes(1):
+            return None
+        act, slope, mask, mask_scale = epi or _NO_EPI
+        if mask is not None and not (mask.dtype == torch.float32 and mask.dim() == 2 and tuple(mask.shape) == (layout.n_dst, F)
+                                     and mask.device == X.device and mask.stride(1) == 1 and mask.stride(0) % 4 == 0
+                                     and mask.data_ptr() % 16 == 0):
+            return None
+        coded = self._scale_ids(name, scale, layout.indices if mult is None else mult[2])
+        if coded is None or not takes(coded[0].shape[0]):
+            return None
+        ds = _prep_scale(out_scale, layout.n_dst, "dst_scale")
+        if ds is not None and (not ds.is_cuda or ds.device != X.device):
+            return None
+        y = torch.empty((layout.n_dst, F), dtype=torch.float32, device=X.device) if out is None else out
+        if tuple(y.shape) != (layout.n_dst, F) or y.dtype != torch.float32 or y.device != X.device:
+            return None
+        if not _lib.spmm_owned_scaled(layout.segptr, coded[1], X, coded[0], ds, y, layout.n_src, layout.n_slices,
+                                      mult is not None, (act, slope, mask, mask_scale)):
+            return None
+        return y
 
     def spmm(self, X, src_scale=None, dst_scale=None, out=None, epi=None, gather_dtype=None):
         return self._product(self._S.fwd, X, src_scale, dst_scale, out, epi, gather_dtype)
diff --git a/include/dgmi_scale.h b/include/dgmi_scale.h
--- /dev/null
+++ b/include/dgmi_scale.h
@@ -0,0 +1,26 @@
+#ifndef DGMI_SCALE_H_
+#define DGMI_SCALE_H_
+
+#include "dgmi.h"
+
+#ifdef __cplusplus
+extern "C" {
+#endif
+
+#define DGMI_SCALE_CODE_SHIFT 17
+#define DGMI_SCALE_CODE_BITS 11
+
+DGMI_API int32_t dgmi_spmm_owned_scaled_takes(int64_t n_dst, int64_t n_src, int64_t F, int64_t ldx, int32_t n_slices,
+                                              int32_t id_multiplicity, int32_t n_codes);
+
+DGMI_API int dgmi_spmm_owned_scaled_f32(const int32_t* segptr, const int32_t* coded_indices, const float* X, int64_t ldx,
+                                        const float* table, int32_t n_codes, const float* dst_scale, float* Y, int64_t ldy,
+                                        int64_t n_dst, int64_t n_src, int64_t F, int32_t n_slices, int32_t id_multiplicity,
+                                        int32_t act, float act_slope, const float* out_mask, int64_t ld_mask,
+                                        float out_mask_scale, int32_t* taken, dgmi_stream_t stream);
+
+#ifdef __cplusplus
+}
+#endif
+
+#endif
```

Result: faster. 38.27 billion (median of 6 runs) (+2.3%).
